# ljubobratovicrelja/tensor-truth

Measured on AMD Instinct MI355X. Metric: queries/sec (embed+top-k+rerank) over 10M x 1024 corpus, higher is better.
Workload: dtype bf16

## Files before the change

### include/tt_hip.h

```cpp
#ifndef TT_HIP_H
#define TT_HIP_H

#include <stddef.h>
#include <stdint.h>

#ifdef __cplusplus
extern "C" {
#endif

#if defined(__GNUC__) || defined(__clang__)
#pragma GCC visibility push(default)
#endif

#define TT_OK 0
#define TT_E_INVALID (-1)
#define TT_E_UNSUPPORTED (-2)
#define TT_E_WORKSPACE (-3)
#define TT_E_HIP (-4)

int tt_version(void);
const char* tt_arch(void);
const char* tt_last_error(void);
int tt_device_cu_count(void);

// ... 48 lines not shown

typedef struct tt_layer_weights {
    const void* qkv_w;
    const float* qkv_b;
    const void* o_w;
    const float* o_b;
    const float* ln1_g;
    const float* ln1_b;
    const void* ffn1_w;
    const float* ffn1_b;
    const void* ffn2_w;
    const float* ffn2_b;
    const float* ln2_g;
    const float* ln2_b;
    const void* qkv_w8;
    const float* qkv_wscale;
    const void* ffn1_w8;
    const float* ffn1_wscale;
    const void* o_w8;
    const float* o_wscale;
    const void* ffn2_w8;
    const float* ffn2_wscale;
    float ffn_act_scale;
} tt_layer_weights;

typedef struct tt_encoder_weights {
    int32_t hidden, layers, heads, ffn, vocab, max_pos, type_vocab;
    float ln_eps;
    const void* word_emb;
    const void* pos_emb;
    const void* type_emb;
    const float* emb_ln_g;
    const float* emb_ln_b;
    const tt_layer_weights* layer;
    const void* cls_dense_w;
    const float* cls_dense_b;
    const void* cls_out_w;
    const float* cls_out_b;
    float* ffn_absmax_out;
} tt_encoder_weights;

size_t tt_encoder_workspace_bytes(const tt_encoder_weights* w, int n_rows);

int tt_encoder_forward(const tt_encoder_weights* w, const int32_t* ids, const int32_t* pos,
                       const int32_t* type_ids, const int32_t* seq_start, const int32_t* seq_len,
                       int n_seq, int n_rows, int max_len, void* hidden_out,
                       void* workspace, size_t workspace_bytes, void* stream);

size_t tt_encoder_cls_workspace_bytes(const tt_encoder_weights* w, int n_rows, int n_seq);
int tt_encoder_forward_cls(const tt_encoder_weights* w, const int32_t* ids, const int32_t* pos,
                           const int32_t* type_ids, const int32_t* seq_start, const int32_t* seq_len,
                           int n_seq, int n_rows, int max_len, void* cls_out,
                           void* workspace, size_t workspace_bytes, void* stream);

int tt_embed_pool(const void* hidden_bf16, int ld, const int32_t* rows, int n_seq, int hidden,
                  float* out_f32, void* out_bf16, void* stream);

int tt_embed_pool_mean(const void* hidden_bf16, int ld, const int32_t* seq_start, const int32_t* seq_len, int n_seq, int hidden,
                       float* out_f32, void* out_bf16, void* stream);
int tt_embed_pool_mean_f32(const float* hidden_f32, int ld, const int32_t* seq_start, const int32_t* seq_len, int n_seq, int hidden,
                           float* out_f32, void* out_bf16, void* stream);

int tt_rerank_head(const tt_encoder_weights* w, const void* hidden_bf16, const int32_t* rows, int n_seq,
                   float* scores, float* logits, void* workspace, size_t workspace_bytes, void* stream);

int tt_adjacent_cosine(const float* emb_f32, int n, int hidden, float* out_dist, void* stream);

int tt_gemm_bf16(const void* a, const void* w, const float* bias, const void* residual, void* c,
                 int m, int n, int k, int epilogue , void* stream);
int tt_layernorm_bf16(const void* in, void* out, const float* gamma, const float* beta, int rows, int hidden,
                      float eps, void* stream);
int tt_attention_varlen(const void* qk, int ld_qk, int q_col0, int k_col0, const void* vt, int ldvt, void* out,
                        int ld_out, const int32_t* seq_start, const int32_t* seq_len, int n_seq, int heads,
                        int head_dim, int max_len, void* stream);
int tt_attention_cls_varlen(const void* qk, int ld_qk, int q_col0, int k_col0, const void* vt, int ldvt, void* out,
                            int ld_out, const int32_t* seq_start, const int32_t* seq_len, int n_seq, int heads,
                            int head_dim, int max_len, void* stream);

int tt_quantize_rows_fp8(const void* in_bf16, int rows, int cols, void* out_fp8, float* out_scale, void* stream);
int tt_layernorm_bf16_fp8(const void* in, void* out, const float* gamma, const float* beta, int rows, int hidden,
                          float eps, void* out_fp8, float* out_scale, void* stream);
int tt_gemm_fp8(const void* a8, const float* a_scale, const void* w8, const float* w_scale, const float* bias, void* c,
                int m, int n, int k, int epilogue , void* stream);
int tt_gemm_fp8_ex(const void* a8, const float* a_scale, const void* w8, const float* w_scale, const float* bias,
                   const void* residual, void* c_bf16, void* c_fp8, float c_fp8_inv_scale, int m, int n, int k,
                   int epilogue, void* stream);

typedef struct tt_layer_weights_f32 {
    const float* qkv_w;
    const float* qkv_b;
    const float* o_w;
    const float* o_b;
    const float* ln1_g;
    const float* ln1_b;
    const float* ffn1_w;
    const float* ffn1_b;
    const float* ffn2_w;
    const float* ffn2_b;
    const float* ln2_g;
    const float* ln2_b;
} tt_layer_weights_f32;

typedef struct tt_encoder_weights_f32 {
    int32_t hidden, layers, heads, ffn, vocab, max_pos, type_vocab;
    float ln_eps;
    const float* word_emb;
    const float* pos_emb;
    const float* type_emb;
    const float* emb_ln_g;
    const float* emb_ln_b;
    const tt_layer_weights_f32* layer;
    const float* cls_dense_w;
    const float* cls_dense_b;
    const float* cls_out_w;
    const float* cls_out_b;
} tt_encoder_weights_f32;

size_t tt_encoder_f32_workspace_bytes(const tt_encoder_weights_f32* w, int n_rows);
int tt_encoder_forward_f32(const tt_encoder_weights_f32* w, const int32_t* ids, const int32_t* pos,
                           const int32_t* type_ids, const int32_t* seq_start, const int32_t* seq_len,
                           int n_seq, int n_rows, int max_len, float* hidden_out,
                           void* workspace, size_t workspace_bytes, void* stream);
int tt_embed_pool_f32(const float* hidden_f32, int ld, const int32_t* rows, int n_seq, int hidden,
                      float* out_f32, void* out_bf16, void* stream);
int tt_rerank_head_f32(const tt_encoder_weights_f32* w, const float* hidden_f32, const int32_t* rows, int n_seq,
                       float* scores, float* logits, void* workspace, size_t workspace_bytes, void* stream);
int tt_gemm_f32(const float* a, const float* w, const float* bias, const float* residual, float* c,
                int m, int n, int k, int epilogue, void* stream);

size_t tt_encoder_workspace_bytes_f16(const tt_encoder_weights* w, int n_rows);
size_t tt_encoder_cls_workspace_bytes_f16(const tt_encoder_weights* w, int n_rows, int n_seq);
int tt_encoder_forward_f16(const tt_encoder_weights* w, const int32_t* ids, const int32_t* pos,
                           const int32_t* type_ids, const int32_t* seq_start, const int32_t* seq_len,
                           int n_seq, int n_rows, int max_len, void* hidden_out,
                           void* workspace, size_t workspace_bytes, void* stream);
int tt_encoder_forward_cls_f16(const tt_encoder_weights* w, const int32_t* ids, const int32_t* pos,
                               const int32_t* type_ids, const int32_t* seq_start, const int32_t* seq_len,
                               int n_seq, int n_rows, int max_len, void* cls_out,
                               void* workspace, size_t workspace_bytes, void* stream);
int tt_embed_pool_f16(const void* hidden_f16, int ld, const int32_t* rows, int n_seq, int hidden, float* out_f32,
                      void* out_f16, void* stream);
int tt_embed_pool_mean_f16(const void* hidden_f16, int ld, const int32_t* seq_start, const int32_t* seq_len, int n_seq, int hidden,
                           float* out_f32, void* out_f16, void* stream);
int tt_rerank_head_f16(const tt_encoder_weights* w, const void* hidden_f16, const int32_t* rows, int n_seq,
                       float* scores, float* logits, void* workspace, size_t workspace_bytes, void* stream);
int tt_gemm_f16(const void* a, const void* w, const float* bias, const void* residual, void* c,
                int m, int n, int k, int epilogue, void* stream);
int tt_layernorm_f16(const void* in, void* out, const float* gamma, const float* beta, int rows, int hidden,
                     float eps, void* stream);
int tt_attention_varlen_f16(const void* qk, int ld_qk, int q_col0, int k_col0, const void* vt, int ldvt, void* out,
                            int ld_out, const int32_t* seq_start, const int32_t* seq_len, int n_seq, int heads,
                            int head_dim, int max_len, void* stream);
int tt_attention_cls_varlen_f16(const void* qk, int ld_qk, int q_col0, int k_col0, const void* vt, int ldvt, void* out,
                                int ld_out, const int32_t* seq_start, const int32_t* seq_len, int n_seq, int heads,
                                int head_dim, int max_len, void* stream);

typedef struct tt_layer_weights_x3 {
    const void* qkv_w;
    const float* qkv_b;
    const void* o_w;
    const float* o_b;
    const float* ln1_g;
    const float* ln1_b;
    const void* ffn1_w;
    const float* ffn1_b;
    const void* ffn2_w;
    const float* ffn2_b;
    const float* ln2_g;
    const float* ln2_b;
} tt_layer_weights_x3;

typedef struct tt_encoder_weights_x3 {
    int32_t hidden, layers, heads, ffn, vocab, max_pos, type_vocab;
    float ln_eps;
    const float* word_emb;
    const float* pos_emb;
    const float* type_emb;
    const float* emb_ln_g;
    const float* emb_ln_b;
    const tt_layer_weights_x3* layer;
    const float* cls_dense_w;
    const float* cls_dense_b;
    const float* cls_out_w;
    const float* cls_out_b;
} tt_encoder_weights_x3;

size_t tt_encoder_x3_workspace_bytes(const tt_encoder_weights_x3* w, int n_rows);
int tt_encoder_forward_x3(const tt_encoder_weights_x3* w, const int32_t* ids, const int32_t* pos,
                          const int32_t* type_ids, const int32_t* seq_start, const int32_t* seq_len,
                          int n_seq, int n_rows, int max_len, float* hidden_out,
                          void* workspace, size_t workspace_bytes, void* stream);
size_t tt_encoder_x3_cls_workspace_bytes(const tt_encoder_weights_x3* w, int n_rows, int n_seq);
int tt_encoder_forward_x3_cls(const tt_encoder_weights_x3* w, const int32_t* ids, const int32_t* pos, const int32_t* type_ids,
                              const int32_t* seq_start, const int32_t* seq_len, int n_seq, int n_rows, int max_len,
                              float* cls_out, void* workspace, size_t workspace_bytes, void* stream);
int tt_rerank_head_x3(const tt_encoder_weights_x3* w, const float* hidden_f32, const int32_t* rows, int n_seq,
                      float* scores, float* logits, void* workspace, size_t workspace_bytes, void* stream);
int tt_split_planes(const float* in_f32, int64_t rows, int cols, void* out_planes, void* stream);
int tt_gemm_x3(const void* a_planes, const void* w_planes, const float* bias, const float* residual_f32, void* c_planes,
               float* c_f32, int m, int n, int k, int epilogue, void* stream);
int tt_gemm_x3_ex(const void* a_planes, const void* w_planes, const float* bias, const float* residual_f32,
                  const void* residual_planes, int ldr, int res_lo_off, void* c_planes, int ldc, int c_lo_off, float* c_f32,
                  void* vt_hi, void* vt_lo, int ldvt, int m, int n, int k, int epilogue, void* stream);
int tt_attention_x3(const void* qk_planes, int ld_qk, int q_col0, int k_col0, int lo_off, const void* vt_hi,
                    const void* vt_lo, int ldvt, void* out_planes, int ld_out, int out_lo_off,
// ... 470 lines not shown
```

### tensor-truth_amd/_lib.py

```python
from __future__ import annotations

import ctypes
import os
import threading
from ctypes import c_char_p, c_float, c_int, c_int32, c_int64, c_size_t, c_void_p

_HERE = os.path.dirname(os.path.abspath(__file__))
_LIB_NAME = "libtt_hip.so"
_lock = threading.Lock()
_lib = None


class LibraryNotBuiltError(RuntimeError):
    pass


class TTError(RuntimeError):
    """A libtt_hip.so call returned a non-zero status."""


def lib_path() -> str:
    return os.path.join(_HERE, os.environ.get("TT_LIB_NAME") or _LIB_NAME)


# ... 9 lines not shown
    if _isa_ok is None:
        import hashlib

        ok = False
        try:
            with open(lib_path() + ".isa_ok") as fh:
                want = fh.read().strip()
            h = hashlib.sha256()
            with open(lib_path(), "rb") as fh:
                for blk in iter(lambda: fh.read(1 << 20), b""):
                    h.update(blk)
            ok = h.hexdigest() == want
        except OSError:
            ok = False
        _isa_ok = ok
    return _isa_ok


_F32P = ctypes.POINTER(c_float)
_I32P = ctypes.POINTER(c_int32)

SIGNATURES = {
    "tt_version": (c_int, []),
    "tt_arch": (c_char_p, []),
    "tt_last_error": (c_char_p, []),
    "tt_device_cu_count": (c_int, []),
    "tt_scan_workspace_bytes": (c_size_t, [c_int64, c_int, c_int, c_int]),
    "tt_scan_topk": (c_int, [c_void_p, c_int64, c_int, c_void_p, c_int, c_int, c_int32, c_void_p, c_void_p,
                             c_void_p, c_size_t, c_void_p, c_void_p]),
    "tt_scan_exact_workspace_bytes": (c_size_t, [c_int64, c_int, c_int, c_int]),
    "tt_scan_topk_exact": (c_int, [c_void_p, c_int64, c_int, c_void_p, c_int, c_int, c_int32, c_void_p, c_void_p,
                                   c_void_p, c_size_t, c_void_p]),
    "tt_scan_segmented_workspace_bytes": (c_size_t, [c_int64, c_int, c_int, c_int]),
    "tt_scan_topk_segmented": (c_int, [c_void_p, c_int64, c_int, c_void_p, c_int, c_int, c_void_p, c_int, c_void_p,
                                       c_void_p, c_void_p, c_size_t, c_void_p]),
    "tt_scan_shadow_bytes": (c_size_t, [c_int64, c_int]),
    "tt_scan_shadow_build": (c_int, [c_void_p, c_int, c_int64, c_int64, c_void_p, c_int64, c_void_p]),
    "tt_scan_shadow_workspace_bytes": (c_size_t, [c_int64, c_int, c_int, c_int]),
    "tt_scan_topk_shadow": (c_int, [c_void_p, c_void_p, c_int64, c_int64, c_int, c_void_p, c_int, c_int, c_int32, c_void_p, c_void_p,
                                    c_void_p, c_size_t, c_void_p, c_void_p]),
    "tt_filter_rows_workspace_bytes": (c_size_t, [c_int64]),
    "tt_filter_rows": (c_int, [c_int, c_void_p, c_void_p, c_void_p, c_int, c_int64, c_void_p, c_int, c_void_p, c_void_p,
                               c_void_p, c_size_t, c_void_p]),
    "tt_scan_topk_rows_workspace_bytes": (c_size_t, [c_int64, c_int, c_int, c_int]),
    "tt_scan_topk_rows": (c_int, [c_void_p, c_int64, c_int, c_void_p, c_int, c_int, c_void_p, c_void_p, c_int64, c_void_p, c_int,
                                  c_int32, c_void_p, c_void_p, c_void_p, c_size_t, c_void_p, c_void_p]),
    "tt_topk_merge": (c_int, [c_void_p, c_void_p, c_int, c_int, c_int, c_void_p, c_void_p, c_void_p]),
    "tt_encoder_workspace_bytes": (c_size_t, [c_void_p, c_int]),
    "tt_encoder_forward": (c_int, [c_void_p, c_void_p, c_void_p, c_void_p, c_void_p, c_void_p, c_int, c_int, c_int,
                                   c_void_p, c_void_p, c_size_t, c_void_p]),
    "tt_encoder_cls_workspace_bytes": (c_size_t, [c_void_p, c_int, c_int]),
    "tt_encoder_forward_cls": (c_int, [c_void_p, c_void_p, c_void_p, c_void_p, c_void_p, c_void_p, c_int, c_int, c_int,
                                       c_void_p, c_void_p, c_size_t, c_void_p]),
    "tt_embed_pool": (c_int, [c_void_p, c_int, c_void_p, c_int, c_int, c_void_p, c_void_p, c_void_p]),
    "tt_embed_pool_mean": (c_int, [c_void_p, c_int, c_void_p, c_void_p, c_int, c_int, c_void_p, c_void_p, c_void_p]),
    "tt_embed_pool_mean_f32": (c_int, [c_void_p, c_int, c_void_p, c_void_p, c_int, c_int, c_void_p, c_void_p, c_void_p]),
    "tt_encoder_workspace_bytes_f16": (c_size_t, [c_void_p, c_int]),
    "tt_encoder_cls_workspace_bytes_f16": (c_size_t, [c_void_p, c_int, c_int]),
    "tt_encoder_forward_f16": (c_int, [c_void_p, c_void_p, c_void_p, c_void_p, c_void_p, c_void_p, c_int, c_int, c_int,
                                   c_void_p, c_void_p, c_size_t, c_void_p]),
    "tt_encoder_forward_cls_f16": (c_int, [c_void_p, c_void_p, c_void_p, c_void_p, c_void_p, c_void_p, c_int, c_int, c_int,
                                       c_void_p, c_void_p, c_size_t, c_void_p]),
    "tt_embed_pool_f16": (c_int, [c_void_p, c_int, c_void_p, c_int, c_int, c_void_p, c_void_p, c_void_p]),
    "tt_embed_pool_mean_f16": (c_int, [c_void_p, c_int, c_void_p, c_void_p, c_int, c_int, c_void_p, c_void_p, c_void_p]),
    "tt_rerank_head_f16": (c_int, [c_void_p, c_void_p, c_void_p, c_int, c_void_p, c_void_p, c_void_p, c_size_t, c_void_p]),
    "tt_gemm_f16": (c_int, [c_void_p, c_void_p, c_void_p, c_void_p, c_void_p, c_int, c_int, c_int, c_int, c_void_p]),
    "tt_layernorm_f16": (c_int, [c_void_p, c_void_p, c_void_p, c_void_p, c_int, c_int, c_float, c_void_p]),
    "tt_attention_varlen_f16": (c_int, [c_void_p, c_int, c_int, c_int, c_void_p, c_int, c_void_p, c_int, c_void_p,
                                    c_void_p, c_int, c_int, c_int, c_int, c_void_p]),
    "tt_attention_cls_varlen_f16": (c_int, [c_void_p, c_int, c_int, c_int, c_void_p, c_int, c_void_p, c_int, c_void_p,
                                    c_void_p, c_int, c_int, c_int, c_int, c_void_p]),
    "tt_rerank_head": (c_int, [c_void_p, c_void_p, c_void_p, c_int, c_void_p, c_void_p, c_void_p, c_size_t, c_void_p]),
    "tt_adjacent_cosine": (c_int, [c_void_p, c_int, c_int, c_void_p, c_void_p]),
    "tt_gemm_bf16": (c_int, [c_void_p, c_void_p, c_void_p, c_void_p, c_void_p, c_int, c_int, c_int, c_int, c_void_p]),
    "tt_layernorm_bf16": (c_int, [c_void_p, c_void_p, c_void_p, c_void_p, c_int, c_int, c_float, c_void_p]),
    "tt_attention_varlen": (c_int, [c_void_p, c_int, c_int, c_int, c_void_p, c_int, c_void_p, c_int, c_void_p,
                                    c_void_p, c_int, c_int, c_int, c_int, c_void_p]),
    "tt_attention_cls_varlen": (c_int, [c_void_p, c_int, c_int, c_int, c_void_p, c_int, c_void_p, c_int, c_void_p,
                                    c_void_p, c_int, c_int, c_int, c_int, c_void_p]),
    "tt_quantize_rows_fp8": (c_int, [c_void_p, c_int, c_int, c_void_p, c_void_p, c_void_p]),
    "tt_layernorm_bf16_fp8": (c_int, [c_void_p, c_void_p, c_void_p, c_void_p, c_int, c_int, c_float, c_void_p, c_void_p,
                                      c_void_p]),
    "tt_gemm_fp8": (c_int, [c_void_p, c_void_p, c_void_p, c_void_p, c_void_p, c_void_p, c_int, c_int, c_int, c_int,
                            c_void_p]),
    "tt_gemm_fp8_ex": (c_int, [c_void_p, c_void_p, c_void_p, c_void_p, c_void_p, c_void_p, c_void_p, c_void_p, c_float,
                               c_int, c_int, c_int, c_int, c_void_p]),
    "tt_encoder_f32_workspace_bytes": (c_size_t, [c_void_p, c_int]),
    "tt_encoder_forward_f32": (c_int, [c_void_p, c_void_p, c_void_p, c_void_p, c_void_p, c_void_p, c_int, c_int, c_int,
                                       c_void_p, c_void_p, c_size_t, c_void_p]),
    "tt_embed_pool_f32": (c_int, [c_void_p, c_int, c_void_p, c_int, c_int, c_void_p, c_void_p, c_void_p]),
    "tt_rerank_head_f32": (c_int, [c_void_p, c_void_p, c_void_p, c_int, c_void_p, c_void_p, c_void_p, c_size_t, c_void_p]),
    "tt_gemm_f32": (c_int, [c_void_p, c_void_p, c_void_p, c_void_p, c_void_p, c_int, c_int, c_int, c_int, c_void_p]),
    "tt_encoder_x3_workspace_bytes": (c_size_t, [c_void_p, c_int]),
    "tt_encoder_x3_cls_workspace_bytes": (c_size_t, [c_void_p, c_int, c_int]),
    "tt_encoder_forward_x3": (c_int, [c_void_p, c_void_p, c_void_p, c_void_p, c_void_p, c_void_p, c_int, c_int, c_int,
                                      c_void_p, c_void_p, c_size_t, c_void_p]),
    "tt_encoder_forward_x3_cls": (c_int, [c_void_p, c_void_p, c_void_p, c_void_p, c_void_p, c_void_p, c_int, c_int, c_int,
                                      c_void_p, c_void_p, c_size_t, c_void_p]),
    "tt_rerank_head_x3": (c_int, [c_void_p, c_void_p, c_void_p, c_int, c_void_p, c_void_p, c_void_p, c_size_t, c_void_p]),
    "tt_split_planes": (c_int, [c_void_p, c_int64, c_int, c_void_p, c_void_p]),
    "tt_gemm_x3": (c_int, [c_void_p, c_void_p, c_void_p, c_void_p, c_void_p, c_void_p, c_int, c_int, c_int, c_int, c_void_p]),
    "tt_gemm_x3_ex": (c_int, [c_void_p, c_void_p, c_void_p, c_void_p, c_void_p, c_int, c_int, c_void_p, c_int, c_int, c_void_p,
                              c_void_p, c_void_p, c_int, c_int, c_int, c_int, c_int, c_void_p]),
    "tt_attention_x3": (c_int, [c_void_p, c_int, c_int, c_int, c_int, c_void_p, c_void_p, c_int, c_void_p, c_int, c_int,
                                c_void_p, c_void_p, c_int, c_int, c_int, c_void_p]),
    "tt_attention_x3_hd": (c_int, [c_void_p, c_int, c_int, c_int, c_int, c_void_p, c_void_p, c_int, c_void_p, c_int, c_int,
# ... 117 lines not shown
                                       c_int, c_int, c_int, c_int, c_int, c_void_p, c_void_p]),
    "tt_maxsim": (c_int, [c_void_p, c_void_p, c_void_p, c_int, c_void_p, c_void_p, c_void_p, c_void_p, c_int, c_int, c_void_p,
                          c_void_p]),
    "tt_colbert_project": (c_int, [c_void_p, c_int, c_int, c_void_p, c_int, c_void_p, c_int, c_void_p, c_void_p]),
    "tt_attention_keylimit": (c_int, [c_void_p, c_int, c_int, c_int, c_void_p, c_int, c_void_p, c_int, c_void_p, c_void_p, c_void_p,
                                      c_int, c_int, c_int, c_int, c_void_p]),
    "tt_encoder_forward_keylen": (c_int, [c_void_p, c_void_p, c_void_p, c_void_p, c_void_p, c_void_p, c_void_p, c_int, c_int, c_int,
                                          c_void_p, c_void_p, c_size_t, c_void_p]),
    "tt_maxsim_f16": (c_int, [c_void_p, c_void_p, c_void_p, c_int, c_void_p, c_void_p, c_void_p, c_void_p, c_int, c_int, c_void_p,
                              c_void_p]),
    "tt_colbert_project_f16": (c_int, [c_void_p, c_int, c_int, c_void_p, c_int, c_void_p, c_int, c_void_p, c_void_p]),
    "tt_attention_keylimit_f16": (c_int, [c_void_p, c_int, c_int, c_int, c_void_p, c_int, c_void_p, c_int, c_void_p, c_void_p,
                                          c_void_p, c_int, c_int, c_int, c_int, c_void_p]),
    "tt_encoder_forward_keylen_f16": (c_int, [c_void_p, c_void_p, c_void_p, c_void_p, c_void_p, c_void_p, c_void_p, c_int, c_int,
                                              c_int, c_void_p, c_void_p, c_size_t, c_void_p]),
    "tt_lexical_weights": (c_int, [c_void_p, c_int, c_int, c_int, c_void_p, c_float, c_void_p, c_void_p, c_void_p, c_int, c_int,
                                   c_int, c_int, c_int, c_int, c_void_p, c_void_p, c_void_p, c_void_p]),
    "tt_lexical_weights_f16": (c_int, [c_void_p, c_int, c_int, c_int, c_void_p, c_float, c_void_p, c_void_p, c_void_p, c_int, c_int,
                                       c_int, c_int, c_int, c_int, c_void_p, c_void_p, c_void_p, c_void_p]),
    "tt_lexical_weights_f32": (c_int, [c_void_p, c_int, c_int, c_int, c_void_p, c_float, c_void_p, c_void_p, c_void_p, c_int, c_int,
                                       c_int, c_int, c_int, c_int, c_void_p, c_void_p, c_void_p, c_void_p]),
    "tt_lexical_score": (c_int, [c_void_p, c_void_p, c_void_p, c_void_p, c_int, c_void_p, c_void_p, c_void_p, c_void_p, c_void_p,
                                 c_int, c_void_p, c_void_p, c_int, c_float, c_float, c_void_p, c_void_p, c_void_p, c_void_p]),
    "tt_lexical_scan_workspace_bytes": (c_size_t, [c_int64, c_int]),
    "tt_lexical_scan_topk": (c_int, [c_void_p, c_void_p, c_void_p, c_void_p, c_int, c_void_p, c_void_p, c_void_p, c_void_p, c_int64,
                                     c_int, c_void_p, c_void_p, c_void_p, c_size_t, c_void_p]),
    "tt_postings_build_workspace_bytes": (c_size_t, [c_int]),
    "tt_postings_build": (c_int, [c_void_p, c_void_p, c_void_p, c_void_p, c_int64, c_int, c_void_p, c_void_p, c_int64, c_void_p,
                                  c_void_p, c_void_p, c_size_t, c_void_p]),
    "tt_lexical_topk_postings_workspace_bytes": (c_size_t, [c_int64, c_int64, c_int]),
    "tt_lexical_topk_postings": (c_int, [c_void_p, c_void_p, c_void_p, c_void_p, c_int, c_void_p, c_void_p, c_void_p, c_void_p, c_int64,
                                         c_void_p, c_int64, c_int64, c_void_p, c_void_p, c_void_p, c_int64, c_int, c_void_p, c_void_p,
                                         c_void_p, c_void_p, c_void_p, c_void_p, c_size_t, c_void_p]),
    "tt_multivec_project": (c_int, [c_void_p, c_int, c_int, c_int, c_void_p, c_void_p, c_int, c_void_p, c_int, c_void_p, c_void_p]),
    "tt_multivec_project_f16": (c_int, [c_void_p, c_int, c_int, c_int, c_void_p, c_void_p, c_int, c_void_p, c_int, c_void_p,
                                        c_void_p]),
    "tt_multivec_project_f32": (c_int, [c_void_p, c_int, c_int, c_int, c_void_p, c_void_p, c_int, c_void_p, c_int, c_void_p,
                                        c_void_p]),
    "tt_maxsim_wide": (c_int, [c_void_p, c_void_p, c_void_p, c_int, c_void_p, c_void_p, c_void_p, c_void_p, c_int, c_int, c_int,
                               c_void_p, c_void_p]),
    "tt_maxsim_wide_f16": (c_int, [c_void_p, c_void_p, c_void_p, c_int, c_void_p, c_void_p, c_void_p, c_void_p, c_int, c_int, c_int,
                                   c_void_p, c_void_p]),
    "tt_m3_mix": (c_int, [c_void_p, c_void_p, c_void_p, c_int64, c_float, c_float, c_float, c_void_p, c_void_p]),
    "tt_splade_pool": (c_int, [c_void_p, c_int, c_int, c_int, c_void_p, c_void_p, c_int, c_void_p, c_void_p, c_int, c_int, c_int,
                               c_void_p, c_int, c_void_p]),
    "tt_splade_pool_f16": (c_int, [c_void_p, c_int, c_int, c_int, c_void_p, c_void_p, c_int, c_void_p, c_void_p, c_int, c_int, c_int,
                                   c_void_p, c_int, c_void_p]),
    "tt_sparse_compact": (c_int, [c_void_p, c_int, c_int, c_int, c_int, c_void_p, c_void_p, c_void_p, c_void_p]),
    "tt_prof_enable": (c_int, [c_int]),
    "tt_prof_read": (c_int, [c_int, ctypes.POINTER(ctypes.c_double), ctypes.POINTER(c_int)]),
}


def load_library():
    global _lib
    if _lib is not None:
        return _lib
    with _lock:
        if _lib is not None:
            return _lib
        path = lib_path()
        if not os.path.exists(path):
            raise LibraryNotBuiltError(
                f"{path} not found. Build it first: `python -c 'import __graft_entry__ as g; g.build()'` "
                f"or `make -C {os.path.join(_HERE, 'csrc')}` (needs hipcc, --offload-arch=gfx950). "
                "tensor_truth_amd has no CPU fallback."
            )
        import torch

        lib = ctypes.CDLL(path)
        for name, (res, args) in SIGNATURES.items():
            fn = getattr(lib, name)
            fn.restype = res
            fn.argtypes = args
        _lib = lib
        return _lib


def check(status: int, what: str) -> None:
    if status != 0:
        msg = load_library().tt_last_error().decode("utf-8", "replace")
        raise TTError(f"{what} failed with status {status}: {msg}")
```

### tensor-truth_amd/csrc/attention.hip

```cpp
#include "common.h"
#include "encoder.h"
#include "f16c.h"

namespace {

#ifndef TT_ATT_RESIDENT_DEFAULT
#define TT_ATT_RESIDENT_DEFAULT 0
#endif
#ifndef TT_ATT_RESIDENT_MIN_LEN
#define TT_ATT_RESIDENT_MIN_LEN 1
#endif
constexpr int kKTile = 64;
constexpr int kWaves = 4;

typedef unsigned int u32x4 __attribute__((ext_vector_type(4)));
template <int OFF>
__device__ __forceinline__ u32x4 lds_read128_async(uint32_t addr) {
    u32x4 r;
    asm volatile("ds_read_b128 %0, %1 offset:%2" : "=v"(r) : "v"(addr), "n"(OFF));
    return r;
}
template <int N>
__device__ __forceinline__ void lds_wait4n(u32x4& a, u32x4& b, u32x4& c, u32x4& d) {
    asm volatile("s_waitcnt lgkmcnt(%4)" : "+v"(a), "+v"(b), "+v"(c), "+v"(d) : "n"(N));
}
template <int N>
__device__ __forceinline__ void lds_wait2n(u32x4& a, u32x4& b) {
    asm volatile("s_waitcnt lgkmcnt(%2)" : "+v"(a), "+v"(b) : "n"(N));
}
typedef unsigned int u32x2 __attribute__((ext_vector_type(2)));
__device__ __forceinline__ void lds_write64_async(uint32_t addr, uint2 v) {
    const u32x2 d = u32x2{v.x, v.y};
    asm volatile("ds_write_b64 %0, %1" :: "v"(addr), "v"(d) : "memory");
}

constexpr int kIoLineStores = 1, kIoShapeStores = 4, kIoShapeQ = 8;

template <int DH, bool STAMP = false, int ABL = 0, int NW = kWaves, int IO = kIoLineStores>
__global__ __launch_bounds__(64 * NW, 4) void attention_kernel(AttnParams p) {
    constexpr int RB = DH * 2;
    constexpr int CH = RB / 16;
    constexpr int RPB = 256 / RB;
    constexpr int KS = DH / 16;
    constexpr int DT = DH / 32;
    constexpr int NPK = kKTile * RB / 1024;
    constexpr int NPV = 8 * DH * 16 / 1024;
    constexpr bool kEvenPieces = NPK % NW == 0 && NPV % NW == 0;
    constexpr int KPW = kEvenPieces ? NPK / NW : 1, VPW = kEvenPieces ? NPV / NW : 1;
    static_assert(kEvenPieces || (DH == 64 && NPK == 8 && NPV == 8), "the uneven piece map is written for head_dim 64");
    constexpr int BUF = (NPK + NPV) * 1024;
    __shared__ __attribute__((aligned(1024))) char lds[2 * BUF];

    int st_i = 0;
    auto stamp = [&]() {
        if constexpr (STAMP) {
            if (p.dbg && blockIdx.x == gridDim.x / 2 && (threadIdx.x & 63) == 0 && st_i < 60) {
                __builtin_amdgcn_sched_barrier(0);
                p.dbg[(threadIdx.x >> 6) * 64 + st_i] = __builtin_amdgcn_s_memtime();
                __builtin_amdgcn_sched_barrier(0);
            }
            ++st_i;
        }
    };
    stamp();
    const int nqt = p.n_qt > 0 ? p.n_qt : -p.n_qt;
    const int L = blockIdx.x, t = L >> 3;
    const int qt = p.n_qt > 0 ? t % nqt : L % nqt;
    const int pair = p.n_qt > 0 ? (t / nqt) * 8 + (L & 7) : L / nqt;
    if (pair >= p.heads * p.n_seq) return;
    const int head = pair % p.heads, seq = pair / p.heads;
    const int len = p.seq_len[seq];
    if (qt * 32 * NW >= len) return;
    const int t0 = p.seq_start[seq];
    const int t0a = t0 & ~7, off = t0 - t0a, alen = off + len;
    const int tid = threadIdx.x, lane = tid & 63;
    const int wave = __builtin_amdgcn_readfirstlane(tid >> 6);
    const int ql = lane & 31, hh = lane >> 5;
    const uint32_t lds0 = (uint32_t)(uintptr_t)(__attribute__((address_space(3))) char*)lds;

    int wslot = wave;
    if (p.rotate && NW == kWaves) {
        const int left = len - qt * 32 * kWaves;
        const int n_live = left >= 32 * kWaves ? kWaves : (left + 31) >> 5;
        if (n_live < kWaves) wslot = (wave + ((pair * n_live) & (kWaves - 1))) & (kWaves - 1);
    }
    const int q_row = (qt * NW + wslot) * 32 + ql;
    const int q_row_c = q_row < len ? q_row : len - 1;
    const uint16_t* qp = p.qk + (size_t)(t0 + q_row_c) * p.ld_qk + p.q_col0 + head * DH + hh * 8;
    ex8 qf[KS];
    if constexpr ((IO & kIoShapeQ) != 0) {
#pragma unroll
        for (int s = 0; s < KS; ++s) {
            const int r = (qt * NW + wslot) * 32 + s * (64 / CH) + lane / CH;
            const int rc = r < len ? r : len - 1;
            qf[s] = *reinterpret_cast<const ex8*>(p.qk + (size_t)(t0 + rc) * p.ld_qk + p.q_col0 + head * DH + (lane % CH) * 8);
        }
    } else {
#pragma unroll
        for (int s = 0; s < KS; ++s) qf[s] = *reinterpret_cast<const ex8*>(qp + s * 16);
    }

    const int n_kt = (alen + kKTile - 1) / kKTile;
    const int n_g8 = (alen + 7) >> 3;
    const int t0kv = (ABL == 4) ? (p.seq_start[0] & ~7) : t0a;
    const uint16_t* kbase = p.qk + (size_t)t0kv * p.ld_qk + p.k_col0 + head * DH;
    const uint16_t* vbase = p.vt + (size_t)(t0kv >> 3) * p.ldvt + (size_t)head * DH * 8;
    constexpr int kRowsPerPiece = 64 / CH, kGroupsPerPiece = 64 / DH > 0 ? 64 / DH : 1;
    static_assert(KPW == 1 || CH == 8, "piece-to-piece swizzle step is written for 128-byte K rows");
    static_assert(VPW == 1 || DH == 64, "one token group per V piece");
    const uint32_t lds_base = (uint32_t)(uintptr_t)(__attribute__((address_space(3))) char*)lds;
    uint32_t kvoff0, vvoff0;
    {
        const int e = (kEvenPieces ? wave * KPW * 64 : 0) + lane, r = e / CH, pos = e % CH;
        kvoff0 = ((uint32_t)r * (uint32_t)p.ld_qk + (uint32_t)((pos ^ ((r / RPB) & (CH - 1))) << 3)) * 2u;
        const int ev = (kEvenPieces ? wave * VPW * 64 : 0) + lane;
        vvoff0 = ((uint32_t)(ev / DH) * (uint32_t)p.ldvt + (uint32_t)((ev % DH) * 8)) * 2u;
    }
    auto sbase = [](const void* ptr) {
        const unsigned long long b = reinterpret_cast<unsigned long long>(ptr);
        const unsigned lo = __builtin_amdgcn_readfirstlane((unsigned)b), hi = __builtin_amdgcn_readfirstlane((unsigned)(b >> 32));
        return reinterpret_cast<const char*>(((unsigned long long)hi << 32) | lo);
    };
    auto glds16 = [](const char* base, uint32_t voff, uint32_t lds_addr) {
        asm volatile("s_mov_b32 m0, %2\n\ts_nop 0\n\tglobal_load_lds_dwordx4 %0, %1" ::"v"(voff), "s"(base), "s"(lds_addr) : "memory", "m0");
    };
    auto issue_tile = [&](int kt) {
        const uint32_t buf = lds_base + (uint32_t)(kt & 1) * BUF;
        const bool clamp = (kt + 1) * kKTile > alen || (kt == 0 && off != 0);
        if (!clamp) {
            if constexpr (kEvenPieces) {
#pragma unroll
                for (int i = 0; i < KPW; ++i)
                    glds16(sbase(kbase + ((size_t)kt * kKTile + i * kRowsPerPiece) * p.ld_qk), (i & 1) ? (kvoff0 ^ 64u) : kvoff0,
                           buf + (uint32_t)(wave * KPW + i) * 1024u);
#pragma unroll
                for (int i = 0; i < VPW; ++i)
                    glds16(sbase(vbase + ((size_t)kt * 8 + i * kGroupsPerPiece) * p.ldvt), vvoff0, buf + (uint32_t)(NPK + wave * VPW + i) * 1024u);
            } else {
                for (int j = wave; j < NPK + NPV; j += NW) {
                    if (j < NPK)
                        glds16(sbase(kbase + ((size_t)kt * kKTile + j * kRowsPerPiece) * p.ld_qk), (j & 1) ? (kvoff0 ^ 64u) : kvoff0,
                               buf + (uint32_t)j * 1024u);
                    else
                        glds16(sbase(vbase + ((size_t)kt * 8 + (j - NPK) * kGroupsPerPiece) * p.ldvt), vvoff0, buf + (uint32_t)j * 1024u);
                }
            }
            return;
        }
        const char* kb = sbase(kbase);
        const char* vb = sbase(vbase);
        int lane_c = lane;
        asm volatile("" : "+v"(lane_c));
        auto clamped_k = [&](int piece) {
            const int e = piece * 64 + lane_c, r = e / CH, pos = e % CH;
            int row = kt * kKTile + r;
            row = row < off ? off : (row < alen ? row : alen - 1);
            glds16(kb, ((uint32_t)row * (uint32_t)p.ld_qk + (uint32_t)((pos ^ ((r / RPB) & (CH - 1))) << 3)) * 2u,
                   buf + (uint32_t)piece * 1024u);
// ... 246 lines not shown
            __builtin_amdgcn_sched_barrier(0);
            if (!wave_active) return;
            const uint32_t slice = lds0 + (uint32_t)wave * (32 * RB);
            const uint32_t wbase = slice + ql * RB + (((ql / RPL) & (CH - 1)) << 4) + 8 * hh;
#pragma unroll
            for (int d = 0; d < DT; ++d)
#pragma unroll
                for (int g = 0; g < 4; ++g) {
                    uint2 o;
                    o.x = pack_e2(acc_o[d][4 * g + 0] * inv, acc_o[d][4 * g + 1] * inv);
                    o.y = pack_e2(acc_o[d][4 * g + 2] * inv, acc_o[d][4 * g + 3] * inv);
                    lds_write64_async(wbase ^ (uint32_t)((4 * d + g) << 4), o);
                }
            asm volatile("s_waitcnt lgkmcnt(0)" ::: "memory");
            const int r0 = lane / CH;
            const uint32_t raddr = slice + r0 * RB + (((lane % CH) ^ ((r0 / RPL) & (CH - 1))) << 4);
            t[0] = lds_read128_async<0>(raddr);
            t[1] = lds_read128_async<RPI * RB>(raddr);
            if constexpr (NI == 4) {
                t[2] = lds_read128_async<2 * RPI * RB>(raddr);
                t[3] = lds_read128_async<3 * RPI * RB>(raddr);
                lds_wait4n<0>(t[0], t[1], t[2], t[3]);
            } else {
                lds_wait2n<0>(t[0], t[1]);
            }
        }
        const int row0 = (qt * NW + wslot) * 32 + lane / CH;
        uint16_t* op = p.out + (size_t)(t0 + row0) * p.ld_out + head * DH + (lane % CH) * 8;
#pragma unroll
        for (int i = 0; i < NI; ++i)
            if (row0 + i * RPI < len) *reinterpret_cast<u32x4*>(op + (size_t)(i * RPI) * p.ld_out) = t[i];
    }
}


#if TT_DIAG
constexpr int kResMaxTiles = 5;

template <int DH, bool PIPE = false, bool EARLY = false>
__global__ __launch_bounds__(64 * kWaves, 2) void attention_resident_kernel(AttnParams p) {
    constexpr int RB = DH * 2, CH = RB / 16, RPB = 256 / RB, KS = DH / 16, DT = DH / 32;
    constexpr int NPK = kKTile * RB / 1024, NPV = 8 * DH * 16 / 1024, NW = kWaves;
    constexpr int KPW = NPK / NW, VPW = NPV / NW;
    static_assert(DH == 64 && NPK % NW == 0 && NPV % NW == 0, "written for head_dim 64");
    constexpr int BUF = (NPK + NPV) * 1024;
    extern __shared__ __attribute__((aligned(1024))) char lds_dyn[];

    const int pair = blockIdx.x;
    if (pair >= p.heads * p.n_seq) return;
    const int head = pair % p.heads, seq = pair / p.heads;
    const int len = p.seq_len[seq];
    if (len <= 0) return;
    const int t0 = p.seq_start[seq];
    const int t0a = t0 & ~7, off = t0 - t0a, alen = off + len;
    const int tid = threadIdx.x, lane = tid & 63;
    const int wave = __builtin_amdgcn_readfirstlane(tid >> 6);
    const int ql = lane & 31, hh = lane >> 5;
    const uint32_t lds0 = (uint32_t)(uintptr_t)(__attribute__((address_space(3))) char*)lds_dyn;
    const int n_kt = (alen + kKTile - 1) / kKTile;
    const int n_g8 = (alen + 7) >> 3;
    const int n_blk = (len + 31) >> 5;
    const int rot = (int)((blockIdx.x >> 8) * 2 + (blockIdx.x & 1)) & 3;
    const int first = (wave - rot) & 3;

    auto q_ptr = [&](int b) {
        const int q_row = b * 32 + ql;
        const int q_row_c = q_row < len ? q_row : len - 1;
        return p.qk + (size_t)(t0 + q_row_c) * p.ld_qk + p.q_col0 + head * DH + hh * 8;
    };
    const int abl = p.rotate;
    ex8 qf[KS] = {};
    if (first < n_blk && !(abl & 2)) {
        const uint16_t* qp = q_ptr(first);
#pragma unroll
        for (int s = 0; s < KS; ++s) qf[s] = *reinterpret_cast<const ex8*>(qp + s * 16);
    }

    const uint16_t* kbase = p.qk + (size_t)t0a * p.ld_qk + p.k_col0 + head * DH;
    const uint16_t* vbase = p.vt + (size_t)(t0a >> 3) * p.ldvt + (size_t)head * DH * 8;
    constexpr int kRowsPerPiece = 64 / CH, kGroupsPerPiece = 1;
    uint32_t kvoff0, vvoff0;
    {
        const int e = wave * KPW * 64 + lane, r = e / CH, pos = e % CH;
        kvoff0 = ((uint32_t)r * (uint32_t)p.ld_qk + (uint32_t)((pos ^ ((r / RPB) & (CH - 1))) << 3)) * 2u;
        const int ev = wave * VPW * 64 + lane;
        vvoff0 = ((uint32_t)(ev / DH) * (uint32_t)p.ldvt + (uint32_t)((ev % DH) * 8)) * 2u;
    }
    auto sbase = [](const void* ptr) {
        const unsigned long long b = reinterpret_cast<unsigned long long>(ptr);
        const unsigned lo = __builtin_amdgcn_readfirstlane((unsigned)b), hi = __builtin_amdgcn_readfirstlane((unsigned)(b >> 32));
        return reinterpret_cast<const char*>(((unsigned long long)hi << 32) | lo);
    };
    auto glds16 = [](const char* base, uint32_t voff, uint32_t lds_addr) {
        asm volatile("s_mov_b32 m0, %2\n\ts_nop 0\n\tglobal_load_lds_dwordx4 %0, %1" ::"v"(voff), "s"(base), "s"(lds_addr) : "memory", "m0");
    };
    for (int kt = 0; kt < ((abl & 4) ? 0 : n_kt); ++kt) {
        const uint32_t buf = lds0 + (uint32_t)kt * BUF;
        const bool clamp = (kt + 1) * kKTile > alen || (kt == 0 && off != 0);
        if (!clamp) {
#pragma unroll
            for (int i = 0; i < KPW; ++i)
                glds16(sbase(kbase + ((size_t)kt * kKTile + i * kRowsPerPiece) * p.ld_qk), (i & 1) ? (kvoff0 ^ 64u) : kvoff0,
                       buf + (uint32_t)(wave * KPW + i) * 1024u);
#pragma unroll
            for (int i = 0; i < VPW; ++i)
                glds16(sbase(vbase + ((size_t)kt * 8 + i * kGroupsPerPiece) * p.ldvt), vvoff0, buf + (uint32_t)(NPK + wave * VPW + i) * 1024u);
        } else {
            const char* kb = sbase(kbase);
            const char* vb = sbase(vbase);
#pragma unroll
            for (int i = 0; i < KPW; ++i) {
                const int piece = wave * KPW + i;
                const int e = piece * 64 + lane, r = e / CH, pos = e % CH;
                int row = kt * kKTile + r;
                row = row < off ? off : (row < alen ? row : alen - 1);
                glds16(kb, ((uint32_t)row * (uint32_t)p.ld_qk + (uint32_t)((pos ^ ((r / RPB) & (CH - 1))) << 3)) * 2u, buf + (uint32_t)piece * 1024u);
            }
#pragma unroll
            for (int i = 0; i < VPW; ++i) {
                const int piece = wave * VPW + i;
                const int e = piece * 64 + lane;
                int g8 = kt * 8 + e / DH;
                g8 = g8 < n_g8 ? g8 : n_g8 - 1;
                glds16(vb, ((uint32_t)g8 * (uint32_t)p.ldvt + (uint32_t)((e % DH) * 8)) * 2u, buf + (uint32_t)(NPK + piece) * 1024u);
            }
        }
    }
    if constexpr (!EARLY) {
        __builtin_amdgcn_s_waitcnt(0x0F70);
        asm volatile("" ::: "memory");
        __builtin_amdgcn_sched_barrier(0);
// ... 284 lines not shown
                    vf[1][1] = lds_read128_async<6 * DH * 16 + 512>(vaddr);
                }
#pragma unroll
                for (int s2 = 0; s2 < 2; ++s2) {
                    uint4 pb;
                    pb.x = pack_e2_inrange(acc_s[j][8 * s2 + 0], acc_s[j][8 * s2 + 1]);
                    pb.y = pack_e2_inrange(acc_s[j][8 * s2 + 2], acc_s[j][8 * s2 + 3]);
                    pb.z = pack_e2_inrange(acc_s[j][8 * s2 + 4], acc_s[j][8 * s2 + 5]);
                    pb.w = pack_e2_inrange(acc_s[j][8 * s2 + 6], acc_s[j][8 * s2 + 7]);
                    const ex8 pf = __builtin_bit_cast(ex8, pb);
#pragma unroll
                    for (int d = 0; d < DT; ++d)
                        acc_o[d] = TT_MFMA_32x32x16(va[s2][d], pf, acc_o[d]);
                }
            }
        }
        const float l_tot = l_run + __shfl_xor(l_run, 32, 64);
        const float inv = 1.0f / l_tot;
        const int q_row = b * 32 + ql;
        if (q_row < len && !(abl & 1)) {
            uint16_t* op = p.out + (size_t)(t0 + q_row) * p.ld_out + head * DH;
#pragma unroll
            for (int d = 0; d < DT; ++d)
#pragma unroll
                for (int g = 0; g < 4; ++g) {
                    uint2 o;
                    o.x = pack_e2(acc_o[d][4 * g + 0] * inv, acc_o[d][4 * g + 1] * inv);
                    o.y = pack_e2(acc_o[d][4 * g + 2] * inv, acc_o[d][4 * g + 3] * inv);
                    *reinterpret_cast<uint2*>(op + 32 * d + 8 * g + 4 * hh) = o;
                }
        }
        if (EARLY && first_walk) {
            first_walk = false;
            if (more && !(abl & 2)) {
                const uint16_t* qp = q_ptr(b + NW);
#pragma unroll
                for (int s = 0; s < KS; ++s) qn[s] = *reinterpret_cast<const ex8*>(qp + s * 16);
            }
        }
        if (more) {
#pragma unroll
            for (int s = 0; s < KS; ++s) qf[s] = qn[s];
        }
    }
}


#endif
template <int DH>
__global__ __launch_bounds__(64) void attention_cls_kernel(AttnParams p) {
    extern __shared__ __attribute__((aligned(16))) float probs[];
    const int seq = blockIdx.x, head = blockIdx.y, lane = threadIdx.x;
    const int len = p.seq_len[seq], t0 = p.seq_start[seq];
    const int t0a = t0 & ~7, off = t0 - t0a, alen = off + len;
    float q[DH];
    {
        const uint16_t* qp = p.q_rows ? p.q_rows + (size_t)seq * p.ld_q_rows + head * DH : p.qk + (size_t)t0 * p.ld_qk + p.q_col0 + head * DH;
#pragma unroll
        for (int c = 0; c < DH / 8; ++c) {
            const uint4 u = *reinterpret_cast<const uint4*>(qp + c * 8);
            q[c * 8 + 0] = elo(u.x); q[c * 8 + 1] = ehi(u.x);
            q[c * 8 + 2] = elo(u.y); q[c * 8 + 3] = ehi(u.y);
            q[c * 8 + 4] = elo(u.z); q[c * 8 + 5] = ehi(u.z);
            q[c * 8 + 6] = elo(u.w); q[c * 8 + 7] = ehi(u.w);
            if (p.qk_lo_off) {
                const uint4 l = *reinterpret_cast<const uint4*>(qp + p.qk_lo_off + c * 8);
                q[c * 8 + 0] += elo(l.x); q[c * 8 + 1] += ehi(l.x);
                q[c * 8 + 2] += elo(l.y); q[c * 8 + 3] += ehi(l.y);
                q[c * 8 + 4] += elo(l.z); q[c * 8 + 5] += ehi(l.z);
                q[c * 8 + 6] += elo(l.w); q[c * 8 + 7] += ehi(l.w);
            }
        }
    }
    const float sc = p.scale * 1.4426950408889634f;
    float mx = -__builtin_inff();
    for (int j = off + lane; j < alen; j += 64) {
        const uint16_t* kp = p.qk + (size_t)(t0a + j) * p.ld_qk + p.k_col0 + head * DH;
        float acc = 0.f;
#pragma unroll
        for (int c = 0; c < DH / 8; ++c) {
            const uint4 u = *reinterpret_cast<const uint4*>(kp + c * 8);
            float kf[8] = {elo(u.x), ehi(u.x), elo(u.y), ehi(u.y), elo(u.z), ehi(u.z), elo(u.w), ehi(u.w)};
            if (p.qk_lo_off) {
                const uint4 l = *reinterpret_cast<const uint4*>(kp + p.qk_lo_off + c * 8);
                kf[0] += elo(l.x); kf[1] += ehi(l.x); kf[2] += elo(l.y); kf[3] += ehi(l.y);
                kf[4] += elo(l.z); kf[5] += ehi(l.z); kf[6] += elo(l.w); kf[7] += ehi(l.w);
            }
#pragma unroll
            for (int i = 0; i < 8; ++i) acc = fmaf(q[c * 8 + i], kf[i], acc);
        }
        acc *= sc;
        probs[j] = acc;
        mx = fmaxf(mx, acc);
    }
#pragma unroll
    for (int off = 32; off > 0; off >>= 1) mx = fmaxf(mx, __shfl_xor(mx, off, 64));
    float sum = 0.f;
    const int len8 = (alen + 7) & ~7;
    for (int j = lane; j < len8; j += 64) {
        float e = 0.f;
        if (j >= off && j < alen) e = __builtin_amdgcn_exp2f(probs[j] - mx);
        probs[j] = e;
        sum += e;
    }
#pragma unroll
    for (int off = 32; off > 0; off >>= 1) sum += __shfl_xor(sum, off, 64);
    __syncthreads();
    constexpr int PARTS = 64 / DH;
    const int d = lane % DH, part = lane / DH;
    float o = 0.f;
    for (int g8 = part; g8 * 8 < alen; g8 += PARTS) {
        const uint4 u = *reinterpret_cast<const uint4*>(p.vt + (size_t)(t0a / 8 + g8) * p.ldvt + (size_t)(head * DH + d) * 8);
        const float4 pa = *reinterpret_cast<const float4*>(probs + g8 * 8);
        const float4 pb = *reinterpret_cast<const float4*>(probs + g8 * 8 + 4);
        o = fmaf(pa.x, elo(u.x), o); o = fmaf(pa.y, ehi(u.x), o);
        o = fmaf(pa.z, elo(u.y), o); o = fmaf(pa.w, ehi(u.y), o);
        o = fmaf(pb.x, elo(u.z), o); o = fmaf(pb.y, ehi(u.z), o);
        o = fmaf(pb.z, elo(u.w), o); o = fmaf(pb.w, ehi(u.w), o);
    }
    if constexpr (PARTS == 2) o += __shfl_xor(o, 32, 64);
    if (p.out_scales) {
        float y = o / sum;
        asm("" : "+v"(y));
        float amax = fabsf(y);
#pragma unroll
        for (int off = 16; off > 0; off >>= 1) amax = fmaxf(amax, __shfl_xor(amax, off, 64));
        int sbyte, sh;
        xc_block_scale(amax, sbyte, sh);
        if (part == 0) {
            const int W = p.out_width, col = head * DH + d;
// ... 140 lines not shown
```

### tensor-truth_amd/csrc/encoder.h

```cpp
#pragma once
#include "common.h"
#include "gemm_plan.h"

struct GemmParams {
    const uint16_t* A;
    const uint16_t* W;
    const float* bias;
    const uint16_t* residual;
    uint16_t* C;
    uint16_t* vt;
    int M, N, K, lda, ldc, ldr, ldvt, vt_col0;
    const float* a_scale;
    const float* w_scale;
    int fp8;
    uint8_t* C8;
    float c8_inv_scale;
    int nt_store;
    int sn;
    int scan_wave_lists;
    int32_t* scan_cnt;
    float* scan_scores;
    int32_t* scan_idx;
    int scan_cap;
    int32_t scan_idx_base;
    float* scan_dense;
    int scan_dense_stride;
    int scan_tile_stride;
    int scan_rows;
    int x3;
    int ldw;
    int c_lo_off;
    float* C32;
    const float* res32;
    const uint16_t* res_planes;
    int res_lo_off;
    uint16_t* vt_lo;
    int x3_zero_lo;
    int xc;
    const uint8_t* a_scales;
    const uint8_t* w_scales;
    uint8_t* c_scales;
};
int tt_scan_gemm_launch(const uint16_t* corpus, int64_t rows, int dim, const uint16_t* queries256, const float* thr256,
                        int32_t* cnt, float* cand_scores, int32_t* cand_idx, int cap, int32_t idx_base, hipStream_t st);
int tt_scan_gemm_sample_launch(const uint16_t* corpus, int tiles, int tile_stride, int dim, const uint16_t* queries256, const float* thr256,
                               float* dense, int dense_stride, hipStream_t st);
int tt_gemm_launch(const GemmParams& p, int epilogue, hipStream_t st);
bool tt_gemm_skinny_enabled();

struct AttnParams {
    const uint16_t* qk;
    const uint16_t* vt;
    uint16_t* out;
    const int32_t* seq_start;
    const int32_t* seq_len;
    int n_seq, heads, head_dim, max_len;
    int total_rows;
    int ld_qk, q_col0, k_col0, ldvt, ld_out;
    float scale;
    float lazy;
    int n_qt;
    int rotate;
    unsigned long long* dbg;
    const uint16_t* q_rows;
    int ld_q_rows;
    uint8_t* out_scales;
    int out_width;
    int qk_lo_off;
};
int tt_attention_launch(const AttnParams& p, hipStream_t st);
int tt_attention_keylimit_launch(const AttnParams& p, const int32_t* key_len, hipStream_t st);
int tt_attention_cls_launch(const AttnParams& p, hipStream_t st);

struct EmbedParams {
    const int32_t* ids;
    const int32_t* pos;
    const int32_t* type;
    const uint16_t* word;
    const uint16_t* posemb;
    const uint16_t* typeemb;
    const float* gamma;
    const float* beta;
    uint16_t* out;
    int T, H, vocab, max_pos, type_vocab;
    float eps;
    uint8_t* q8;
    float* q8_scale;
};
int tt_embed_ln_launch(const EmbedParams& p, hipStream_t st);

int tt_layernorm_launch(const uint16_t* in, uint16_t* out, const float* gamma, const float* beta, int rows, int H,
                        float eps, hipStream_t st, uint8_t* q8 = nullptr, float* q8_scale = nullptr);
int tt_absmax_launch(const uint16_t* x, size_t n, float* out, hipStream_t st);
int tt_quantize_rows_launch(const uint16_t* in, int ld, int rows, int cols, uint8_t* q8, float* scale, hipStream_t st);

int tt_cls_pool_l2norm_launch(const uint16_t* hidden, int ld, const int32_t* rows, int n, int H, float* out_f32,
                              uint16_t* out_bf16, hipStream_t st);

int tt_mean_pool_l2norm_launch(const void* hidden, int is_f32, int ld, const int32_t* seq_start, const int32_t* seq_len, int n, int H,
                               float* out_f32, uint16_t* out_bf16, hipStream_t st);
int tt_gather_rows_launch(const uint16_t* src, int ld, const int32_t* rows, int n, int n_pad, int H, uint16_t* dst,
                          hipStream_t st);

int tt_head_out_sigmoid_launch(const uint16_t* t, int ld, const uint16_t* w, const float* bias, int n, int H,
                               float* scores, float* logits, hipStream_t st);

int tt_adjacent_cosine_launch(const float* e, int n, int H, float* dist, hipStream_t st);

int tt_gather_rows_f32_launch(const float* src, const int32_t* rows, int n, int n_pad, int H, float* dst, hipStream_t st);

struct WsPlanner {
    size_t off = 0;
    size_t take(size_t bytes) { const size_t o = off; off += tt_align_up(bytes, 256); return o; }
};

inline int tt_check_workspace(const char* what, const void* workspace, size_t workspace_bytes, size_t need) {
    if (!workspace || workspace_bytes < need) {
        tt_set_error("%s: workspace %zu < required %zu bytes", what, workspace_bytes, need);
        return TT_E_WORKSPACE;
    }
    TT_CHECK_ARG(((uintptr_t)workspace % 256) == 0, "workspace must be 256-byte aligned");
    return TT_OK;
}

inline int pooled_rows_pad(int n_seq, bool skinny_allowed) {
    return (n_seq <= 256 && skinny_allowed) ? (n_seq + 63) / 64 * 64 : (n_seq + 255) / 256 * 256;
}

template <class Weights>
inline tt_encoder_weights_f32 head_weights_f32(const Weights* w) {
    tt_encoder_weights_f32 h{};
    h.hidden = w->hidden; h.layers = 0; h.heads = w->heads; h.ffn = w->ffn; h.vocab = w->vocab; h.max_pos = w->max_pos;
    h.type_vocab = w->type_vocab; h.ln_eps = w->ln_eps;
    h.word_emb = w->word_emb; h.pos_emb = w->pos_emb; h.type_emb = w->type_emb; h.emb_ln_g = w->emb_ln_g; h.emb_ln_b = w->emb_ln_b;
    h.cls_dense_w = w->cls_dense_w; h.cls_dense_b = w->cls_dense_b; h.cls_out_w = w->cls_out_w; h.cls_out_b = w->cls_out_b;
    return h;
}

inline GemmParams gemm_16(const uint16_t* a, const void* w, const float* bias, int M, int N, int K) {
    GemmParams g{};
// ... 4 lines not shown
```

### tensor-truth_amd/csrc/encoder_api.hip

```cpp
#include "common.h"
#include "encoder.h"

namespace {

struct EncWs {
    size_t off_xa, off_xb, off_y, off_qk, off_vt, off_ctx, off_ffn, total;
    size_t off_cctx, off_cx, off_cy, off_cx1, off_cffn, off_rows;
    int n_cls_pad;
    size_t off_q8, off_q8s, off_q8c;
    bool fp8;
};

bool fp8_ready(const tt_encoder_weights* w, int n_rows) {
    if constexpr (kF16) return false;
    if (w->layers <= 0 || w->hidden % 256 || w->ffn % 256 || n_rows % 256) return false;
    for (int l = 0; l < w->layers; ++l) {
        const tt_layer_weights& lw = w->layer[l];
        if (!lw.qkv_w8 || !lw.qkv_wscale || !lw.ffn1_w8 || !lw.ffn1_wscale) return false;
    }
    return true;
}

EncWs enc_plan(const tt_encoder_weights* w, int n_rows, int n_seq = 0) {
    EncWs e{};
    const size_t H = (size_t)w->hidden, F = (size_t)w->ffn, T = ((size_t)n_rows + 255) / 256 * 256;
    WsPlanner ws;
    e.off_xa = ws.take(T * H * 2);
    e.off_xb = ws.take(T * H * 2);
    e.off_y = ws.take(T * H * 2);
    e.off_qk = ws.take(T * 2 * H * 2);
    e.off_vt = ws.take(H * T * 2);
    e.off_ctx = ws.take(T * H * 2);
    e.off_ffn = ws.take(T * F * 2);
    e.n_cls_pad = pooled_rows_pad(n_seq, tt_gemm_skinny_enabled());
    if (n_seq > 0) {
        const size_t B = (size_t)e.n_cls_pad;
        e.off_cctx = ws.take(B * H * 2);
        e.off_cx = ws.take(B * H * 2);
        e.off_cy = ws.take(B * H * 2);
        e.off_cx1 = ws.take(B * H * 2);
        e.off_cffn = ws.take(B * F * 2);
    }
    e.fp8 = fp8_ready(w, n_rows);
    if (e.fp8) {
        e.off_q8 = ws.take(T * H);
        e.off_q8s = ws.take(T * 4);
        e.off_q8c = ws.take(T * 4);
    }
    e.total = ws.off;
    return e;
}

int check_weights(const tt_encoder_weights* w) {
    TT_CHECK_ARG(w != nullptr, "null weights");
    TT_CHECK_ARG(w->hidden > 0 && w->hidden % 128 == 0 && w->hidden <= 1024, "hidden=%d unsupported", w->hidden);
    TT_CHECK_ARG(w->heads > 0 && w->hidden % w->heads == 0, "heads=%d", w->heads);
    const int dh = w->hidden / w->heads;
    TT_CHECK_ARG(dh == 64 || dh == 32, "head_dim=%d not in {32,64}", dh);
    TT_CHECK_ARG(w->ffn > 0 && w->ffn % 128 == 0, "ffn=%d must be a multiple of 128", w->ffn);
    TT_CHECK_ARG(w->layers >= 0 && (w->layers == 0 || w->layer != nullptr), "layer array missing");
    TT_CHECK_ARG(w->word_emb && w->pos_emb && w->type_emb && w->emb_ln_g && w->emb_ln_b, "embedding tables missing");
    return TT_OK;
}

}

extern "C" {

size_t tt_encoder_workspace_bytes(const tt_encoder_weights* w, int n_rows) {
    if (!w || n_rows <= 0) return 0;
    return enc_plan(w, n_rows).total;
}

static int forward_impl(const tt_encoder_weights* w, const int32_t* ids, const int32_t* pos,
                        const int32_t* type_ids, const int32_t* seq_start, const int32_t* seq_len, int n_seq,
                        int n_rows, int max_len, void* hidden_out, void* cls_out, void* workspace,
                        size_t workspace_bytes, void* stream, const int32_t* key_len = nullptr) {
    if (int rc = check_weights(w)) return rc;
    TT_CHECK_ARG(key_len == nullptr || cls_out == nullptr, "key_len: the full forward only");
    TT_CHECK_ARG(n_rows > 0 && (n_rows % 128 == 0 || (n_rows < 256 && n_rows % 64 == 0)),
                 "n_rows=%d must be a positive multiple of 128 (or 64 / 192)", n_rows);
    TT_CHECK_ARG(n_seq > 0 && max_len > 0, "n_seq=%d max_len=%d", n_seq, max_len);
    TT_CHECK_ARG(ids && pos && seq_start && seq_len && (hidden_out || cls_out), "null pointer");
    const bool cls_tail = cls_out != nullptr && w->layers > 0;
    const EncWs e = enc_plan(w, n_rows, cls_tail ? n_seq : 0);
    if (int rc = tt_check_workspace("tt_encoder_forward", workspace, workspace_bytes, e.total)) return rc;
    hipStream_t st = (hipStream_t)stream;
    char* ws = (char*)workspace;
    const int H = w->hidden, F = w->ffn, T = n_rows;
    uint16_t* xa = (uint16_t*)(ws + e.off_xa);
    uint16_t* xb = (uint16_t*)(ws + e.off_xb);
    uint16_t* y = (uint16_t*)(ws + e.off_y);
    uint16_t* qk = (uint16_t*)(ws + e.off_qk);
    uint16_t* vt = (uint16_t*)(ws + e.off_vt);
    uint16_t* ctx = (uint16_t*)(ws + e.off_ctx);
    uint16_t* ffn = (uint16_t*)(ws + e.off_ffn);
    TT_CHECK_HIP(hipMemsetAsync(ctx, 0, (size_t)T * H * 2, st));

    EmbedParams ep{};
    ep.ids = ids; ep.pos = pos; ep.type = type_ids;
    ep.word = (const uint16_t*)w->word_emb; ep.posemb = (const uint16_t*)w->pos_emb;
    ep.typeemb = (const uint16_t*)w->type_emb;
    ep.gamma = w->emb_ln_g; ep.beta = w->emb_ln_b;
    ep.T = T; ep.H = H; ep.vocab = w->vocab; ep.max_pos = w->max_pos; ep.type_vocab = w->type_vocab;
    ep.eps = w->ln_eps;
    uint16_t* x = (w->layers == 0 && hidden_out) ? (uint16_t*)hidden_out : xa;
    ep.out = x;
    uint8_t* q8 = e.fp8 ? (uint8_t*)(ws + e.off_q8) : nullptr;
    float* q8s = e.fp8 ? (float*)(ws + e.off_q8s) : nullptr;
    ep.q8 = q8; ep.q8_scale = q8s;
    {
        TtProfScope prof(TT_K_ROWOPS, st);
        if (int rc = tt_embed_ln_launch(ep, st)) return rc;
    }

    const int dh = H / w->heads;
    const int f8mask_all = TT_DIAG_ENV_INT("TT_FP8_MASK", 0xF), f8first = TT_DIAG_ENV_INT("TT_FP8_SKIP_FIRST", 0),
              f8last = TT_DIAG_ENV_INT("TT_FP8_SKIP_LAST", 0);
    struct Fp8Ops {
        uint8_t* q8;
        float* q8s;
        float* q8c;
        int mask;
        float* absmax;
    };
    auto half_layer = [&](const tt_layer_weights& lw, int M, uint16_t* c, const uint16_t* res, uint16_t* y, uint16_t* x1, uint16_t* f,
                          uint16_t* out, const Fp8Ops& f8) -> int {
        GemmParams go = gemm_16(c, lw.o_w, lw.o_b, M, H, H);
        go.residual = res; go.ldr = H; go.C = y; go.ldc = H;
        if ((f8.mask & 2) && lw.o_w8 && lw.o_wscale) {
            {
                TtProfScope prof(TT_K_ROWOPS, st);
                if (int rc = tt_quantize_rows_launch(c, H, M, H, f8.q8, f8.q8s, st)) return rc;
            }
            go.A = (const uint16_t*)f8.q8; go.W = (const uint16_t*)lw.o_w8; go.a_scale = f8.q8s; go.w_scale = lw.o_wscale; go.fp8 = 1;
        }
        if (int rc = tt_gemm_launch(go, TT_EPI_RESIDUAL, st)) return rc;
        {
            TtProfScope prof(TT_K_ROWOPS, st);
            if (int rc = tt_layernorm_launch(y, x1, lw.ln1_g, lw.ln1_b, M, H, w->ln_eps, st, f8.q8, f8.q8s)) return rc;
        }
        GemmParams g1 = gemm_16(x1, lw.ffn1_w, lw.ffn1_b, M, F, H);
        g1.C = f; g1.ldc = F;
        const bool f8down = (f8.mask & 12) == 12 && lw.ffn2_w8 && lw.ffn2_wscale && lw.ffn_act_scale > 0.f;
        if (f8.mask & 4) {
            g1.A = (const uint16_t*)f8.q8; g1.W = (const uint16_t*)lw.ffn1_w8; g1.a_scale = f8.q8s; g1.w_scale = lw.ffn1_wscale; g1.fp8 = 1;
            if (f8down) {
                g1.C8 = (uint8_t*)f; g1.c8_inv_scale = 1.0f / lw.ffn_act_scale;
            }
        }
        if (int rc = tt_gemm_launch(g1, TT_EPI_GELU, st)) return rc;
        if (f8.absmax && !f8down) {
            TtProfScope prof(TT_K_ROWOPS, st);
            if (int rc = tt_absmax_launch(f, (size_t)M * F, f8.absmax, st)) return rc;
        }
        GemmParams g2 = gemm_16(f, lw.ffn2_w, lw.ffn2_b, M, H, F);
        g2.residual = x1; g2.ldr = H; g2.C = y; g2.ldc = H;
        if (f8down) {
            const unsigned bits = __builtin_bit_cast(unsigned, lw.ffn_act_scale);
            TT_CHECK_HIP(hipMemsetD32Async(f8.q8c, (int)bits, (size_t)M, st));
            g2.W = (const uint16_t*)lw.ffn2_w8; g2.a_scale = f8.q8c; g2.w_scale = lw.ffn2_wscale; g2.fp8 = 1;
        }
        if (int rc = tt_gemm_launch(g2, TT_EPI_RESIDUAL, st)) return rc;
        TtProfScope prof(TT_K_ROWOPS, st);
        return tt_layernorm_launch(y, out, lw.ln2_g, lw.ln2_b, M, H, w->ln_eps, st, f8.q8, f8.q8s);
    };
    for (int l = 0; l < w->layers; ++l) {
        const tt_layer_weights& lw = w->layer[l];
        TT_CHECK_ARG(lw.qkv_w && lw.qkv_b && lw.o_w && lw.o_b && lw.ln1_g && lw.ln1_b && lw.ffn1_w && lw.ffn1_b &&
                         lw.ffn2_w && lw.ffn2_b && lw.ln2_g && lw.ln2_b,
                     "layer %d has a null weight pointer", l);
        GemmParams g = gemm_16(x, lw.qkv_w, lw.qkv_b, T, 3 * H, H);
        g.C = qk; g.ldc = 2 * H; g.vt = vt; g.ldvt = 8 * H; g.vt_col0 = 2 * H;
        const int f8mask = (!e.fp8 || l < f8first || l >= w->layers - f8last) ? 0 : f8mask_all;
        if (f8mask & 1) {
            g.A = (const uint16_t*)q8; g.W = (const uint16_t*)lw.qkv_w8; g.a_scale = q8s; g.w_scale = lw.qkv_wscale; g.fp8 = 1;
        }
        static const bool kv_only_on = TT_DIAG_ENV_INT("TT_CLS_KV_ONLY", 1) != 0;
        const bool kv_only = cls_tail && l == w->layers - 1 && !g.fp8 && kv_only_on;
        if (kv_only) {
            g.W = (const uint16_t*)lw.qkv_w + (size_t)H * H; g.bias = lw.qkv_b + H;
            g.C = qk + H; g.N = 2 * H; g.vt_col0 = H;
        }
        if (int rc = tt_gemm_launch(g, TT_EPI_QKV, st)) return rc;
        AttnParams a{};
        a.qk = qk; a.ld_qk = 2 * H; a.q_col0 = 0; a.k_col0 = H; a.vt = vt; a.ldvt = 8 * H;
        a.ld_out = H; a.seq_start = seq_start; a.seq_len = seq_len;
        a.n_seq = n_seq; a.heads = w->heads; a.head_dim = dh; a.max_len = max_len;
        a.scale = 1.0f / sqrtf((float)dh);
        if (cls_tail && l == w->layers - 1) {
            const int Bp = e.n_cls_pad;
            uint16_t* cctx = (uint16_t*)(ws + e.off_cctx);
            uint16_t* cx = (uint16_t*)(ws + e.off_cx);
            uint16_t* cy = (uint16_t*)(ws + e.off_cy);
            uint16_t* cx1 = (uint16_t*)(ws + e.off_cx1);
            uint16_t* cffn = (uint16_t*)(ws + e.off_cffn);
            TT_CHECK_HIP(hipMemsetAsync(cctx, 0, (size_t)Bp * H * 2, st));
            {
                TtProfScope prof(TT_K_ROWOPS, st);
                if (int rc = tt_gather_rows_launch(x, H, seq_start, n_seq, Bp, H, cx, st)) return rc;
            }
            if (kv_only) {
                GemmParams gq = gemm_16(cx, lw.qkv_w, lw.qkv_b, Bp, H, H);
                gq.C = cy; gq.ldc = H;
                if (int rc = tt_gemm_launch(gq, TT_EPI_BIAS, st)) return rc;
                a.q_rows = cy; a.ld_q_rows = H;
            }
            a.out = cctx;
            if (int rc = tt_attention_cls_launch(a, st)) return rc;
            return half_layer(lw, Bp, cctx, cx, cy, cx1, cffn, (uint16_t*)cls_out, Fp8Ops{});
        }
        a.out = ctx; a.total_rows = n_rows;
        if (int rc = key_len ? tt_attention_keylimit_launch(a, key_len, st) : tt_attention_launch(a, st)) return rc;
        uint16_t* x1 = (x == xa) ? xb : xa;
        uint16_t* dst = (l == w->layers - 1) ? (uint16_t*)hidden_out : x;
        const Fp8Ops f8{q8, q8s, e.fp8 ? (float*)(ws + e.off_q8c) : nullptr, f8mask, w->ffn_absmax_out ? w->ffn_absmax_out + l : nullptr};
        if (int rc = half_layer(lw, T, ctx, x, y, x1, ffn, dst, f8)) return rc;
        x = dst;
    }
    return TT_OK;
}

int tt_encoder_forward(const tt_encoder_weights* w, const int32_t* ids, const int32_t* pos,
                       const int32_t* type_ids, const int32_t* seq_start, const int32_t* seq_len, int n_seq,
                       int n_rows, int max_len, void* hidden_out, void* workspace, size_t workspace_bytes,
                       void* stream) {
    TT_CHECK_ARG(hidden_out != nullptr, "null hidden_out");
    return forward_impl(w, ids, pos, type_ids, seq_start, seq_len, n_seq, n_rows, max_len, hidden_out, nullptr, workspace,
                        workspace_bytes, stream);
}

int tt_encoder_forward_keylen(const tt_encoder_weights* w, const int32_t* ids, const int32_t* pos, const int32_t* type_ids,
                              const int32_t* seq_start, const int32_t* seq_len, const int32_t* key_len, int n_seq, int n_rows,
                              int max_len, void* hidden_out, void* workspace, size_t workspace_bytes, void* stream) {
    TT_CHECK_ARG(hidden_out != nullptr, "null hidden_out");
    TT_CHECK_ARG(key_len != nullptr, "null key_len");
    return forward_impl(w, ids, pos, type_ids, seq_start, seq_len, n_seq, n_rows, max_len, hidden_out, nullptr, workspace,
                        workspace_bytes, stream, key_len);
}

size_t tt_encoder_cls_workspace_bytes(const tt_encoder_weights* w, int n_rows, int n_seq) {
    if (!w || n_rows <= 0 || n_seq <= 0) return 0;
    return enc_plan(w, n_rows, n_seq).total;
}

int tt_encoder_forward_cls(const tt_encoder_weights* w, const int32_t* ids, const int32_t* pos,
                           const int32_t* type_ids, const int32_t* seq_start, const int32_t* seq_len, int n_seq,
                           int n_rows, int max_len, void* cls_out, void* workspace, size_t workspace_bytes,
                           void* stream) {
    TT_CHECK_ARG(cls_out != nullptr, "null cls_out");
    TT_CHECK_ARG(w && w->layers > 0, "tt_encoder_forward_cls needs at least one layer");
    return forward_impl(w, ids, pos, type_ids, seq_start, seq_len, n_seq, n_rows, max_len, nullptr, cls_out, workspace,
                        workspace_bytes, stream);
}

int tt_embed_pool(const void* hidden_bf16, int ld, const int32_t* rows, int n_seq, int hidden, float* out_f32,
                  void* out_bf16, void* stream) {
    TT_CHECK_ARG(n_seq >= 0, "n_seq=%d", n_seq);
    if (n_seq == 0) return TT_OK;
    TT_CHECK_ARG(hidden_bf16 && rows && out_f32 && ld >= hidden && ld % 8 == 0, "bad argument");
    TtProfScope prof(TT_K_ROWOPS, (hipStream_t)stream);
    return tt_cls_pool_l2norm_launch((const uint16_t*)hidden_bf16, ld, rows, n_seq, hidden, out_f32,
                                     (uint16_t*)out_bf16, (hipStream_t)stream);
}

int tt_embed_pool_mean(const void* hidden_bf16, int ld, const int32_t* seq_start, const int32_t* seq_len, int n_seq, int hidden,
                       float* out_f32, void* out_bf16, void* stream) {
    TT_CHECK_ARG(n_seq >= 0, "n_seq=%d", n_seq);
    if (n_seq == 0) return TT_OK;
    TT_CHECK_ARG(hidden_bf16 && seq_start && seq_len && out_f32 && ld >= hidden && ld % 8 == 0, "bad argument");
    TtProfScope prof(TT_K_ROWOPS, (hipStream_t)stream);
    return tt_mean_pool_l2norm_launch(hidden_bf16, 0, ld, seq_start, seq_len, n_seq, hidden, out_f32, (uint16_t*)out_bf16,
                                      (hipStream_t)stream);
}

#if !TT_F16
int tt_embed_pool_mean_f32(const float* hidden_f32, int ld, const int32_t* seq_start, const int32_t* seq_len, int n_seq, int hidden,
                           float* out_f32, void* out_bf16, void* stream) {
    TT_CHECK_ARG(n_seq >= 0, "n_seq=%d", n_seq);
    if (n_seq == 0) return TT_OK;
    TT_CHECK_ARG(hidden_f32 && seq_start && seq_len && out_f32 && ld >= hidden && ld % 4 == 0, "bad argument");
    TtProfScope prof(TT_K_ROWOPS, (hipStream_t)stream);
    return tt_mean_pool_l2norm_launch(hidden_f32, 1, ld, seq_start, seq_len, n_seq, hidden, out_f32, (uint16_t*)out_bf16,
                                      (hipStream_t)stream);
}

#endif
int tt_rerank_head(const tt_encoder_weights* w, const void* hidden_bf16, const int32_t* rows, int n_seq,
                   float* scores, float* logits, void* workspace, size_t workspace_bytes, void* stream) {
    if (int rc = check_weights(w)) return rc;
    TT_CHECK_ARG(w->cls_dense_w && w->cls_dense_b && w->cls_out_w && w->cls_out_b, "weights carry no classification head");
    TT_CHECK_ARG(n_seq >= 0, "n_seq=%d", n_seq);
    if (n_seq == 0) return TT_OK;
    TT_CHECK_ARG(hidden_bf16 && rows && scores, "null pointer");
    const int H = w->hidden;
    const int n_pad = (n_seq + 127) / 128 * 128;
    const size_t need = 2 * tt_align_up((size_t)n_pad * H * 2, 256);
    if (!workspace || workspace_bytes < need) {
        tt_set_error("tt_rerank_head: workspace %zu < required %zu bytes", workspace_bytes, need);
        return TT_E_WORKSPACE;
    }
    hipStream_t st = (hipStream_t)stream;
    uint16_t* cls = (uint16_t*)workspace;
    uint16_t* t = (uint16_t*)((char*)workspace + tt_align_up((size_t)n_pad * H * 2, 256));
    {
        TtProfScope prof(TT_K_ROWOPS, st);
        if (int rc = tt_gather_rows_launch((const uint16_t*)hidden_bf16, H, rows, n_seq, n_pad, H, cls, st)) return rc;
    }
// ... 46 lines not shown
    g.A = (const uint16_t*)a8; g.lda = k; g.W = (const uint16_t*)w8; g.bias = bias; g.C = (uint16_t*)c; g.ldc = n;
    g.M = m; g.N = n; g.K = k; g.a_scale = a_scale; g.w_scale = w_scale; g.fp8 = 1;
    return tt_gemm_launch(g, epilogue, (hipStream_t)stream);
}

int tt_gemm_fp8_ex(const void* a8, const float* a_scale, const void* w8, const float* w_scale, const float* bias,
                   const void* residual, void* c_bf16, void* c_fp8, float c_fp8_inv_scale, int m, int n, int k,
                   int epilogue, void* stream) {
    TT_CHECK_ARG(epilogue == TT_EPI_BIAS || epilogue == TT_EPI_GELU || epilogue == TT_EPI_RESIDUAL, "epilogue %d", epilogue);
    TT_CHECK_ARG(a8 && a_scale && w8 && w_scale && bias && (c_bf16 || c_fp8), "null pointer");
    TT_CHECK_ARG(epilogue != TT_EPI_RESIDUAL || (residual && c_bf16 && !c_fp8), "residual epilogue: bf16 result only");
    GemmParams g{};
    g.A = (const uint16_t*)a8; g.lda = k; g.W = (const uint16_t*)w8; g.bias = bias; g.ldc = n;
    g.C = c_bf16 ? (uint16_t*)c_bf16 : (uint16_t*)c_fp8;
    g.residual = (const uint16_t*)residual; g.ldr = n;
    g.M = m; g.N = n; g.K = k; g.a_scale = a_scale; g.w_scale = w_scale; g.fp8 = 1;
    if (c_fp8) { g.C8 = (uint8_t*)c_fp8; g.c8_inv_scale = c_fp8_inv_scale; }
    return tt_gemm_launch(g, epilogue, (hipStream_t)stream);
}

#endif
#if !TT_F16 && TT_DIAG
__attribute__((visibility("default"))) int tt_attention_debug_stamps(const void* qk, int ld_qk, int q_col0, int k_col0, const void* vt, int ldvt, void* out,
                              int ld_out, const int32_t* seq_start, const int32_t* seq_len, int n_seq, int heads,
                              int head_dim, int max_len, void* stamps, void* stream) {
    AttnParams a{};
    a.qk = (const uint16_t*)qk; a.ld_qk = ld_qk; a.q_col0 = q_col0; a.k_col0 = k_col0;
    a.vt = (const uint16_t*)vt; a.ldvt = ldvt; a.out = (uint16_t*)out; a.ld_out = ld_out;
    a.seq_start = seq_start; a.seq_len = seq_len; a.n_seq = n_seq; a.heads = heads; a.head_dim = head_dim;
    a.max_len = max_len; a.scale = 1.0f / sqrtf((float)head_dim);
    a.dbg = (unsigned long long*)stamps;
    return tt_attention_launch(a, (hipStream_t)stream);
}

#endif
int tt_layernorm_bf16(const void* in, void* out, const float* gamma, const float* beta, int rows, int hidden,
                      float eps, void* stream) {
    TT_CHECK_ARG(in && out && gamma && beta, "null pointer");
    return tt_layernorm_launch((const uint16_t*)in, (uint16_t*)out, gamma, beta, rows, hidden, eps, (hipStream_t)stream);
}

int tt_attention_varlen(const void* qk, int ld_qk, int q_col0, int k_col0, const void* vt, int ldvt, void* out,
                        int ld_out, const int32_t* seq_start, const int32_t* seq_len, int n_seq, int heads,
                        int head_dim, int max_len, void* stream) {
    TT_CHECK_ARG(qk && vt && out && seq_start && seq_len, "null pointer");
    AttnParams a{};
    a.qk = (const uint16_t*)qk; a.ld_qk = ld_qk; a.q_col0 = q_col0; a.k_col0 = k_col0;
    a.vt = (const uint16_t*)vt; a.ldvt = ldvt; a.out = (uint16_t*)out; a.ld_out = ld_out;
    a.seq_start = seq_start; a.seq_len = seq_len; a.n_seq = n_seq; a.heads = heads; a.head_dim = head_dim;
    a.max_len = max_len; a.scale = 1.0f / sqrtf((float)head_dim);
    return tt_attention_launch(a, (hipStream_t)stream);
}

int tt_attention_cls_varlen(const void* qk, int ld_qk, int q_col0, int k_col0, const void* vt, int ldvt, void* out,
                            int ld_out, const int32_t* seq_start, const int32_t* seq_len, int n_seq, int heads,
                            int head_dim, int max_len, void* stream) {
    TT_CHECK_ARG(qk && vt && out && seq_start && seq_len, "null pointer");
    TT_CHECK_ARG(head_dim == 64 || head_dim == 32, "head_dim=%d: the attention takes 64- or 32-wide heads", head_dim);
    AttnParams a{};
    a.qk = (const uint16_t*)qk; a.ld_qk = ld_qk; a.q_col0 = q_col0; a.k_col0 = k_col0;
    a.vt = (const uint16_t*)vt; a.ldvt = ldvt; a.out = (uint16_t*)out; a.ld_out = ld_out;
    a.seq_start = seq_start; a.seq_len = seq_len; a.n_seq = n_seq; a.heads = heads; a.head_dim = head_dim;
    a.max_len = max_len; a.scale = 1.0f / sqrtf((float)head_dim);
    return tt_attention_cls_launch(a, (hipStream_t)stream);
}

}
```

### tensor-truth_amd/csrc/f16_names.h

```cpp
#pragma once
#define tt_gemm_launch tt_gemm_launch_f16
#define tt_scan_gemm_launch tt_scan_gemm_launch_f16
#define tt_scan_gemm_sample_launch tt_scan_gemm_sample_launch_f16
#define tt_gemm_skinny_enabled tt_gemm_skinny_enabled_f16
#define tt_attention_launch tt_attention_launch_f16
#define tt_attention_cls_launch tt_attention_cls_launch_f16
#define tt_attention_keylimit_launch tt_attention_keylimit_launch_f16
#define tt_absmax_launch tt_absmax_launch_f16
#define tt_embed_ln_launch tt_embed_ln_launch_f16
#define tt_layernorm_launch tt_layernorm_launch_f16
#define tt_gather_rows_launch tt_gather_rows_launch_f16
#define tt_quantize_rows_launch tt_quantize_rows_launch_f16
#define tt_adjacent_cosine_launch tt_adjacent_cosine_launch_f16
#define tt_cls_pool_l2norm_launch tt_cls_pool_l2norm_launch_f16
#define tt_head_out_sigmoid_launch tt_head_out_sigmoid_launch_f16
#define tt_mean_pool_l2norm_launch tt_mean_pool_l2norm_launch_f16
#define tt_encoder_workspace_bytes tt_encoder_workspace_bytes_f16
#define tt_encoder_cls_workspace_bytes tt_encoder_cls_workspace_bytes_f16
#define tt_encoder_forward tt_encoder_forward_f16
#define tt_encoder_forward_cls tt_encoder_forward_cls_f16
#define tt_encoder_forward_keylen tt_encoder_forward_keylen_f16
#define tt_embed_pool tt_embed_pool_f16
#define tt_embed_pool_mean tt_embed_pool_mean_f16
#define tt_rerank_head tt_rerank_head_f16
#define tt_gemm_bf16 tt_gemm_f16
#define tt_layernorm_bf16 tt_layernorm_f16
#define tt_attention_varlen tt_attention_varlen_f16
#define tt_encoder_x3_workspace_bytes tt_encoder_x3_workspace_bytes_f16
#define tt_encoder_x3_cls_workspace_bytes tt_encoder_x3_cls_workspace_bytes_f16
#define tt_encoder_forward_x3 tt_encoder_forward_x3_f16
#define tt_encoder_forward_x3_cls tt_encoder_forward_x3_cls_f16
#define tt_rerank_head_x3 tt_rerank_head_x3_f16
#define tt_split_planes tt_split_planes_f16
#define tt_gemm_x3 tt_gemm_x3_f16
#define tt_gemm_x3_ex tt_gemm_x3_ex_f16
#define tt_attention_x3 tt_attention_x3_f16
#define tt_attention_x3_hd tt_attention_x3_hd_f16
#define tt_attention_cls_varlen tt_attention_cls_varlen_f16
#define tt_decoder_workspace_bytes tt_decoder_workspace_bytes_f16
#define tt_decoder_forward tt_decoder_forward_f16
#define tt_decoder_rows_workspace_bytes tt_decoder_rows_workspace_bytes_f16
#define tt_decoder_forward_rows tt_decoder_forward_rows_f16
#define tt_decoder_score tt_decoder_score_f16
#define tt_embed_pool_last tt_embed_pool_last_f16
#define tt_attention_causal_gqa tt_attention_causal_gqa_f16
#define tt_qk_norm_rope tt_qk_norm_rope_f16
#define tt_modernbert_workspace_bytes tt_modernbert_workspace_bytes_f16
#define tt_modernbert_forward tt_modernbert_forward_f16
#define tt_modernbert_head tt_modernbert_head_f16
#define tt_rope_v8 tt_rope_v8_f16
#define tt_attention_window tt_attention_window_f16
#define tt_mpnet_workspace_bytes tt_mpnet_workspace_bytes_f16
#define tt_mpnet_forward tt_mpnet_forward_f16
#define tt_attention_relbias tt_attention_relbias_f16
#define tt_deberta_workspace_bytes tt_deberta_workspace_bytes_f16
#define tt_deberta_forward tt_deberta_forward_f16
#define tt_deberta_head tt_deberta_head_f16
#define tt_attention_disentangled tt_attention_disentangled_f16
#define tt_ropebert_workspace_bytes tt_ropebert_workspace_bytes_f16
#define tt_ropebert_forward tt_ropebert_forward_f16
#define tt_jinabert_workspace_bytes tt_jinabert_workspace_bytes_f16
#define tt_jinabert_forward tt_jinabert_forward_f16
#define tt_attention_alibi tt_attention_alibi_f16
#define tt_maxsim tt_maxsim_f16
#define tt_colbert_project tt_colbert_project_f16
#define tt_attention_keylimit tt_attention_keylimit_f16
#define tt_lexical_weights tt_lexical_weights_f16
#define tt_multivec_project tt_multivec_project_f16
#define tt_maxsim_wide tt_maxsim_wide_f16
#define tt_splade_pool tt_splade_pool_f16
```

### tensor-truth_amd/csrc/gemm.hip

```cpp
#include "common.h"
#include <type_traits>

#include "encoder.h"
#include "gemm_plan.h"
#include "f16c.h"

namespace {

constexpr int BM = 128, BN = 128, BK = 64;
constexpr int kGemmThreads = 256;
constexpr int kTileBytes = BM * BK * 2;
constexpr int kStageBytes = 2 * kTileBytes;
constexpr int kGemmLds = 2 * kStageBytes;

__device__ __forceinline__ f32x2 gelu_erf2(f32x2 x) {
    const f32x2 u = f32x2{fabsf(x.x), fabsf(x.y)};
    f32x2 q = u * -9.697845371e-07f + 4.016999810e-05f;
    q = q * u + -7.211678312e-04f;
    q = q * u + 7.490924560e-03f;
    q = q * u + -5.142170191e-02f;
    q = q * u + -4.614778757e-01f;
    q = q * u + -1.149914980e+00f;
    q = q * u + -1.000091195e+00f;
    const f32x2 e = f32x2{__builtin_amdgcn_exp2f(q.x), __builtin_amdgcn_exp2f(q.y)};
// ... 70 lines not shown
                    const int n = nw + i * 16 + g * 4;
                    const int m = mw + j * 16 + (lane & 15);
                    const float4 b4 = *reinterpret_cast<const float4*>(p.bias + n);
                    uint16_t* vt = p.vt + (size_t)(m >> 3) * p.ldvt + (size_t)(n - p.vt_col0) * 8 + (m & 7);
                    vt[0] = f32_to_ebits(acc[i][j][0] + b4.x);
                    vt[8] = f32_to_ebits(acc[i][j][1] + b4.y);
                    vt[16] = f32_to_ebits(acc[i][j][2] + b4.z);
                    vt[24] = f32_to_ebits(acc[i][j][3] + b4.w);
                }
                continue;
            }
        }
        const int n = nw + i * 16 + (g & ~1) * 4;
        const float4 ba = *reinterpret_cast<const float4*>(p.bias + n);
        const float4 bb = *reinterpret_cast<const float4*>(p.bias + n + 4);
        const float bias8[8] = {ba.x, ba.y, ba.z, ba.w, bb.x, bb.y, bb.z, bb.w};
#pragma unroll
        for (int j = 0; j < MT; j += 2) {
            float v[8];
#pragma unroll
            for (int k = 0; k < 4; ++k) {
                const auto r = __builtin_amdgcn_permlane16_swap(__float_as_uint(acc[i][j][k]),
                                                                __float_as_uint(acc[i][j + 1][k]), false, false);
                v[k] = __uint_as_float(r[0]);
                v[4 + k] = __uint_as_float(r[1]);
            }
            const int m = mw + (odd ? j + 1 : j) * 16 + (lane & 15);
#pragma unroll
            for (int k = 0; k < 8; ++k) v[k] += bias8[k];
            if constexpr (EPI == TT_EPI_GELU) {
#pragma unroll
                for (int k = 0; k < 8; ++k) v[k] = gelu_erf(v[k]);
            } else if constexpr (EPI == TT_EPI_TANH) {
#pragma unroll
                for (int k = 0; k < 8; ++k) v[k] = tanhf(v[k]);
            } else if constexpr (EPI == TT_EPI_RELU) {
#pragma unroll
                for (int k = 0; k < 8; ++k) v[k] = fmaxf(v[k], 0.f);
            } else if constexpr (EPI == TT_EPI_RESIDUAL) {
                const uint4 r = *reinterpret_cast<const uint4*>(p.residual + (size_t)m * p.ldr + n);
                v[0] += elo(r.x); v[1] += ehi(r.x);
                v[2] += elo(r.y); v[3] += ehi(r.y);
                v[4] += elo(r.z); v[5] += ehi(r.z);
                v[6] += elo(r.w); v[7] += ehi(r.w);
            }
            uint4 o;
            o.x = pack_e2(v[0], v[1]); o.y = pack_e2(v[2], v[3]);
            o.z = pack_e2(v[4], v[5]); o.w = pack_e2(v[6], v[7]);
            *reinterpret_cast<uint4*>(p.C + (size_t)m * p.ldc + n) = o;
        }
    }
}

template <int NT, int MT, bool FP8 = false, bool X3 = false>
__device__ __forceinline__ void gemm_epilogue_vt(const GemmParams& p, f32x4 (&acc)[NT][MT], int mw, int nw, int lane) {
    static_assert(NT % 2 == 0, "n-tiles are processed in pairs");
    const int g = lane >> 4;
    const bool odd = (g & 1) != 0;
#pragma unroll
    for (int i = 0; i < NT; i += 2) {
        const int n = nw + (odd ? i + 1 : i) * 16 + (lane & 15);
        const float b = p.bias[n];
        float sw = 1.f;
        if constexpr (FP8) sw = p.w_scale[n];
        uint16_t* col = p.vt + (size_t)(n - p.vt_col0) * 8;
#pragma unroll
        for (int j = 0; j < MT; ++j) {
            float v[8];
            const int m = mw + j * 16 + (g & ~1) * 4;
#pragma unroll
            for (int k = 0; k < 4; ++k) {
                const auto r = __builtin_amdgcn_permlane16_swap(__float_as_uint(acc[i][j][k]),
                                                                __float_as_uint(acc[i + 1][j][k]), false, false);
                v[k] = __uint_as_float(r[0]);
                v[4 + k] = __uint_as_float(r[1]);
            }
            if constexpr (FP8) {
                const float4 a0 = *reinterpret_cast<const float4*>(p.a_scale + m);
                const float4 a1 = *reinterpret_cast<const float4*>(p.a_scale + m + 4);
                v[0] *= a0.x * sw; v[1] *= a0.y * sw; v[2] *= a0.z * sw; v[3] *= a0.w * sw;
                v[4] *= a1.x * sw; v[5] *= a1.y * sw; v[6] *= a1.z * sw; v[7] *= a1.w * sw;
            }
#pragma unroll
            for (int k = 0; k < 8; ++k) v[k] += b;
            uint4 o;
            o.x = pack_sel<X3>(v[0], v[1]); o.y = pack_sel<X3>(v[2], v[3]);
            o.z = pack_sel<X3>(v[4], v[5]); o.w = pack_sel<X3>(v[6], v[7]);
            *reinterpret_cast<uint4*>(col + (size_t)(m >> 3) * p.ldvt) = o;
            if constexpr (X3) {
                uint4 l;
                l.x = pack_e2(v[0] - elo(o.x), v[1] - ehi(o.x));
                l.y = pack_e2(v[2] - elo(o.y), v[3] - ehi(o.y));
                l.z = pack_e2(v[4] - elo(o.z), v[5] - ehi(o.z));
                l.w = pack_e2(v[6] - elo(o.w), v[7] - ehi(o.w));
                if (p.x3_zero_lo) l = uint4{0u, 0u, 0u, 0u};
                *reinterpret_cast<uint4*>(p.vt_lo + (size_t)(n - p.vt_col0) * 8 + (size_t)(m >> 3) * p.ldvt) = l;
            }
        }
    }
}

__device__ __forceinline__ void stage_tile(const GemmParams& p, char* stage, int wave, int lane, int m0, int n0, int k0) {
    const int lrow = lane >> 3;
    const int slot = lane & 7;
#pragma unroll
    for (int j = 0; j < 4; ++j) {
        const int row = 32 * wave + 8 * j + lrow;
        const int chunk = slot ^ ((row >> 1) & 7);
        const uint16_t* src = p.A + (size_t)(m0 + row) * p.lda + k0 + chunk * 8;
        __builtin_amdgcn_global_load_lds((const __attribute__((address_space(1))) void*)src,
                                         (__attribute__((address_space(3))) void*)(stage + (32 * wave + 8 * j) * 128),
                                         16, 0, 0);
    }
#pragma unroll
    for (int j = 0; j < 4; ++j) {
        const int row = 32 * wave + 8 * j + lrow;
        const int chunk = slot ^ ((row >> 1) & 7);
        const uint16_t* src = p.W + (size_t)(n0 + row) * p.K + k0 + chunk * 8;
        __builtin_amdgcn_global_load_lds((const __attribute__((address_space(1))) void*)src,
                                         (__attribute__((address_space(3))) void*)(stage + kTileBytes + (32 * wave + 8 * j) * 128),
                                         16, 0, 0);
    }
}

template <int EPI>
__global__ __launch_bounds__(kGemmThreads, 2) void gemm_kernel(GemmParams p) {
    extern __shared__ __attribute__((aligned(16))) char smem[];
    const int tid = threadIdx.x;
    const int lane = tid & 63;
    const int wave = __builtin_amdgcn_readfirstlane(tid >> 6);
    const int wm = wave >> 1, wn = wave & 1;

    const int mt_n = p.M / BM, nt_n = p.N / BN;
    int L = blockIdx.x;
    {
        const int nwg = gridDim.x;
        if ((nwg & 7) == 0) L = (L & 7) * (nwg >> 3) + (L >> 3);
    }
    const int SN = nt_n < 8 ? nt_n : 8;
    const int SM = 8;
// ... 634 lines not shown
#pragma unroll
            for (int qm = 0; qm < 2; ++qm)
#pragma unroll
                for (int half = 0; half < 2; ++half) {
                    const f32x4 a = acc[qm][qn][nt][2 * half], b = acc[qm][qn][nt][2 * half + 1];
                    float m[4];
#pragma unroll
                    for (int r = 0; r < 4; ++r) m[r] = dpp_max16(fmaxf(a[r], b[r]));
                    if (l15 == 0) {
                        const int grp = tile * 8 + qm * 4 + wm * 2 + half;
#pragma unroll
                        for (int r = 0; r < 4; ++r) p.scan_dense[(size_t)(q0 + r) * p.scan_dense_stride + grp] = m[r];
                    }
                }
        }
}

#define TT_SLOT_END()                                         \
    do {                                                      \
        __builtin_amdgcn_sched_barrier(0);                    \
        __builtin_amdgcn_s_barrier();                         \
        __builtin_amdgcn_sched_barrier(0);                    \
    } while (0)

typedef int v8i __attribute__((ext_vector_type(8)));
struct Frag2 { ex8 lo, hi; };
__device__ __forceinline__ f32x4 mfma_fp8(const ex8& a0, const ex8& a1, const ex8& b0, const ex8& b1, f32x4 c) {
    const v8i a = __builtin_bit_cast(v8i, Frag2{a0, a1});
    const v8i b = __builtin_bit_cast(v8i, Frag2{b0, b1});
    return __builtin_amdgcn_mfma_scale_f32_16x16x128_f8f6f4(a, b, c, 0, 0, 0, 0x7F7F7F7F, 0, 0x7F7F7F7F);
}

constexpr int kXcScaleOff = kLds3;
constexpr int kLdsXc = kLds3 + 2 * 8192;
__device__ __forceinline__ void glds4(const void* base, uint32_t voff, uint32_t lds_addr) {
    asm volatile("s_mov_b32 m0, %2\n\ts_nop 0\n\tglobal_load_lds_dword %0, %1"
                 :: "v"(voff), "s"(base), "s"(lds_addr) : "memory", "m0");
}
template <int OA, int OB>
__device__ __forceinline__ f32x4 mfma_fp8_scaled(const ex8& a0, const ex8& a1, const ex8& b0, const ex8& b1, f32x4 c, uint32_t scale_a,
                                                 uint32_t scale_b) {
    const v8i a = __builtin_bit_cast(v8i, Frag2{a0, a1});
    const v8i b = __builtin_bit_cast(v8i, Frag2{b0, b1});
    return __builtin_amdgcn_mfma_scale_f32_16x16x128_f8f6f4(a, b, c, 0, 0, OA, (int)scale_a, OB, (int)scale_b);
}
template <int N, class F>
__device__ __forceinline__ void static_for(F&& f) {
    if constexpr (N > 0) {
        static_for<N - 1>(f);
        f(std::integral_constant<int, N - 1>{});
    }
}

template <int EPI, bool FP8 = false, bool X3 = false, bool XC = false, bool RP = false>
__global__ __launch_bounds__(kThreads3, 2) void gemm_kernel_v3(GemmParams p) {
    static_assert(!(FP8 && X3), "split-bf16 operands are bf16");
    static_assert(!XC || (!FP8 && !X3 && kF16), "f16c operands: the fp16 instantiation, no other operand mode");
    constexpr int ES = FP8 ? 1 : 2;
    extern __shared__ __attribute__((aligned(16))) char smem[];
    const int tid = threadIdx.x;
    const int lane = tid & 63;
    const int wave = __builtin_amdgcn_readfirstlane(tid >> 6);
    const int wm = wave >> 2, wn = wave & 3;

    const int mt_n = p.M / BM3, nt_n = (p.N + BN3 - 1) / BN3;
    int L = blockIdx.x;
    {
        const int nwg = gridDim.x;
        if ((nwg & 7) == 0) L = (L & 7) * (nwg >> 3) + (L >> 3);
    }
    const int SN = p.sn > 0 ? p.sn : (nt_n < 4 ? nt_n : 4);
    const int SM = 32 / SN > 0 ? 32 / SN : 1;
    const int per_super = SM * SN;
    const int supers_n = (nt_n + SN - 1) / SN;
    const int sidx = L / per_super, widx = L % per_super;
    const int tm = (sidx / supers_n) * SM + widx / SN;
    const int tn = (sidx % supers_n) * SN + widx % SN;
    if (tm >= mt_n || tn >= nt_n) return;
    int m0_nominal = tm * BM3;
    if constexpr (EPI == TT_EPI_SCAN) {
        if (p.scan_tile_stride > 1) m0_nominal *= p.scan_tile_stride;
        if (p.scan_rows && m0_nominal + BM3 > p.scan_rows) m0_nominal = p.scan_rows - BM3;
    }
    const int m0 = m0_nominal, n0 = tn * BN3;
    const int nk1 = p.K * ES / 128;
    constexpr int TB = X3 ? 64 : 128;
    const int nk = X3 ? 2 * nk1 : (XC ? 2 * nk1 : nk1);
    auto tile_a = [&](int t) { return t; };
    auto tile_w = [&](int t) { return t; };

    f32x4 acc[2][2][2][4];
#pragma unroll
    for (int a = 0; a < 2; ++a)
#pragma unroll
        for (int b = 0; b < 2; ++b)
#pragma unroll
            for (int c = 0; c < 2; ++c)
#pragma unroll
                for (int d = 0; d < 4; ++d) acc[a][b][c][d] = f32x4{0.f, 0.f, 0.f, 0.f};

    const int frow = lane & 15, fchk = lane >> 4, sw = (frow >> 1) & 7;
    const int off0 = frow * 128 + ((fchk ^ sw) << 4);
    const int off1 = frow * 128 + (((4 + fchk) ^ sw) << 4);
    const int a_row0 = wm * 64 * 128;
    const int w_row0 = wn * 32 * 128;

    uint32_t voffA[2], voffW[2];
#pragma unroll
    for (int j = 0; j < 2; ++j) {
// ... 187 lines not shown
            mma8(acc[0][0], wf0, sa_reg[0], sw_reg, std::integral_constant<int, 0>{});
            mma8(acc[0][1], wf1, sa_reg[0], sw_reg, std::integral_constant<int, 1>{});
        } else {
            mma(acc[0][0], wf0);
            mma(acc[0][1], wf1);
        }
        TT_SLOT_END();
        if (more2) {
            stage_half<0, ES, true>(p, smem, 0, B, tile_a(t + 2), wave, voffA, m0, n0, TB);
            stage_half<1, ES>(p, smem, 0, B, tile_w(t + 2), wave, voffW, m0, n0, TB);
            if (sc_lb) stage_scales(t + 2);
        } else if (kResLds) {
            stage_res(B == 0 ? 0 : 2);
        }
        read_a(smem + slot_off(0, 1, B));
        if constexpr (F8T) sa_reg[1] = *reinterpret_cast<const uint32_t*>(sbuf + 512 + sa_off);
        wait_n((t + 2 < nk || kResLds) ? 6 + sc_lb : 0);
        if constexpr (F8T) {
            mma8(acc[1][1], wf1, sa_reg[1], sw_reg, std::integral_constant<int, 1>{});
            mma8(acc[1][0], wf0, sa_reg[1], sw_reg, std::integral_constant<int, 0>{});
        } else {
            mma(acc[1][1], wf1);
            mma(acc[1][0], wf0);
        }
        TT_SLOT_END();
    };

    if constexpr (XC) {
        for (int t = 0; t < nk1; t += 2) {
            tile4(t, std::integral_constant<int, 0>{}, std::false_type{});
            tile4(t + 1, std::integral_constant<int, 1>{}, std::false_type{});
        }
        for (int t = nk1; t < nk; t += 2) {
            tile4(t, std::integral_constant<int, 0>{}, std::true_type{});
            tile4(t + 1, std::integral_constant<int, 1>{}, std::true_type{});
        }
    } else {
        for (int t = 0; t < nk; t += 2) {
            tile4(t, std::integral_constant<int, 0>{}, std::false_type{});
            if (t + 1 < nk) tile4(t + 1, std::integral_constant<int, 1>{}, std::false_type{});
        }
    }
    if (!late) TT_SLOT_END();
    stage_res(3);

    if constexpr (X3) {
        if (n0 + wn * 64 >= p.N) return;
    }
    if constexpr (vblk) {
#pragma unroll
        for (int qm = 0; qm < 2; ++qm)
#pragma unroll
            for (int qn = 0; qn < 2; ++qn)
                gemm_epilogue_vt<2, 4, FP8, X3>(p, acc[qm][qn], m0 + qm * 128 + wm * 64, n0 + wn * 64 + qn * 32, lane);
    } else if constexpr (X3) {
        epilogue_x3<EPI, RP>(p, acc, smem, kBiasOff, m0, n0, wm, wn, lane);
    } else if constexpr (XC && EPI == TT_EPI_RESIDUAL) {
        epilogue_x3<EPI>(p, acc, smem, kBiasOff, m0, n0, wm, wn, lane);
    } else if constexpr (XC && EPI == TT_EPI_GELU) {
        epilogue_xc<EPI>(p, acc, smem, kBiasOff, m0, n0, wm, wn, lane);
    } else if constexpr (XC && EPI == TT_EPI_BIAS) {
        if (p.c_lo_off) epilogue_h2(p, acc, smem, kBiasOff, m0, n0, wm, wn, lane);
        else epilogue_all<EPI, true, false>(p, acc, smem, kBiasOff, kScaleOff, m0, n0, wm, wn, wave, lane, false, NoNext{});
    } else if constexpr (EPI == TT_EPI_QKV) {
#pragma unroll
        for (int qm = 0; qm < 2; ++qm)
#pragma unroll
            for (int qn = 0; qn < 2; ++qn)
                gemm_epilogue_wide<EPI, 2, 4>(p, acc[qm][qn], m0 + qm * 128 + wm * 64, n0 + wn * 64 + qn * 32, lane);
    } else if constexpr (EPI == TT_EPI_SCAN) {
        if (p.scan_dense) scan_sample_epilogue(p, acc, tm, wm, wn, lane);
        else if (p.scan_wave_lists) scan_filter_epilogue<2>(p, acc, smem, kBiasOff, m0, wm, wn, lane);
        else scan_filter_epilogue<1>(p, acc, smem, kBiasOff, m0, wm, wn, lane);
    } else {
        epilogue_all<EPI, true, FP8>(p, acc, smem, kBiasOff, kScaleOff, m0, n0, wm, wn, wave, lane, false, NoNext{});
    }
}

template <int EPI, bool FP8 = false>
__global__ __launch_bounds__(kThreads3, 2) void gemm_kernel_p(GemmParams p, int nwg) {
    constexpr int ES = FP8 ? 1 : 2;
    extern __shared__ __attribute__((aligned(16))) char smem[];
    const int tid = threadIdx.x;
    const int lane = tid & 63;
    const int wave = __builtin_amdgcn_readfirstlane(tid >> 6);
    const int wm = wave >> 2, wn = wave & 3;

    const int mt_n = p.M / BM3, nt_n = p.N / BN3;
    const int SN = p.sn > 0 ? p.sn : (nt_n < 4 ? nt_n : 4);
    const int SM = 32 / SN > 0 ? 32 / SN : 1;
    const int per_super = SM * SN;
    const int supers_n = (nt_n + SN - 1) / SN;
    const int nk = p.K * ES / 128;
    auto decode = [&](int v, int& m0, int& n0) {
        const int L = (v & 7) * (nwg >> 3) + (v >> 3);
        const int sidx = L / per_super, widx = L % per_super;
        const int tm = (sidx / supers_n) * SM + widx / SN;
        const int tn = (sidx % supers_n) * SN + widx % SN;
        int mm = tm * BM3;
        if constexpr (EPI == TT_EPI_SCAN) {
            if (p.scan_rows && mm + BM3 > p.scan_rows) mm = p.scan_rows - BM3;
        }
        m0 = __builtin_amdgcn_readfirstlane(mm);
        n0 = __builtin_amdgcn_readfirstlane(tn * BN3);
        return tm < mt_n && tn < nt_n;
    };
    auto next_valid = [&](int v, int& m0, int& n0) {
// ... 607 lines not shown
        const int ldw = p.ldw ? p.ldw : 2 * p.K;
        if (p.M % v3::BM3 || p.N % v3::BN3 || p.K % 256 || p.K < 256 || p.lda < 2 * p.K || ldw < 2 * p.K || p.lda % 8 || ldw % 8 || !p.A ||
            !p.W || !p.bias || !p.a_scales || !p.w_scales) {
            tt_set_error("gemm f16c: M=%d N=%d K=%d lda=%d ldw=%d: M, N, K multiples of 256, c-planes [.][>= 2K uint16] with tiled scales",
                         p.M, p.N, p.K, p.lda, ldw);
            return TT_E_UNSUPPORTED;
        }
        if constexpr (EPI == TT_EPI_RESIDUAL) {
            if (!p.C32 || !p.res32 || p.ldc % 4 || p.ldr % 4) { tt_set_error("gemm f16c: residual epilogue needs fp32 C32 / res32"); return TT_E_INVALID; }
        } else if constexpr (EPI == TT_EPI_VT) {
            if (!p.vt || p.ldvt % 8) { tt_set_error("gemm f16c: V^T epilogue needs vt"); return TT_E_INVALID; }
        } else if constexpr (EPI == TT_EPI_GELU) {
            if (!p.C || !p.c_scales || p.ldc != 2 * p.N) { tt_set_error("gemm f16c: c-planes output needs C, c_scales, ldc = 2 N"); return TT_E_INVALID; }
        } else {
            if (!p.C || p.ldc % 8 || p.c_lo_off % 8 || (p.c_lo_off && p.c_lo_off < p.N)) {
                tt_set_error("gemm f16c: fp16 output needs C, ldc %% 8 == 0 (two planes: c_lo_off >= N, a multiple of 8)");
                return TT_E_INVALID;
            }
        }
        const GemmPlan pl = plan_of(GemmForm::Xc, EPI, p);
        GemmParams q = p;
        q.sn = pl.grid.sn;
        q.ldw = ldw;
        q.nt_store = 1;
        return run_kernel<v3::gemm_kernel_v3<EPI, false, false, true>>(TT_K_GEMM, dim3(pl.gx), v3::kThreads3, v3::kLdsXc, st, q);
    } else {
        tt_set_error("gemm f16c: epilogue %d has no f16c form (fp16 instantiation: bias, GELU, residual, V^T)", EPI);
        return TT_E_UNSUPPORTED;
    }
}

template <int EPI>
int launch_16(const GemmParams& p, const GemmPlan& pl, hipStream_t st) {
    if constexpr (!kF16) if (p.fp8) return launch_fp8<EPI>(p, st);
    const GemmSwitches& sw = gemm_switches();
    GemmParams q = p;
    if constexpr (EPI != TT_EPI_VT) {
        if (pl.kernel == GemmKernel::Skinny) return run_kernel<gemm_skinny_kernel<EPI, false>>(TT_K_GEMM, dim3(pl.gx, pl.gy), 64, 0, st, q);
    }
    if (sw.trace) fprintf(stderr, "gemm launch<%d> M=%d N=%d K=%d lda=%d ldc=%d ldr=%d\n", EPI, p.M, p.N, p.K, p.lda, p.ldc, p.ldr);
    const bool tile128 = pl.kernel == GemmKernel::Staged128 || pl.kernel == GemmKernel::TwoStage128;
    if (EPI == TT_EPI_VT && tile128) {
        tt_set_error("gemm: internal V^T epilogue needs the 256x256 kernel");
        return TT_E_UNSUPPORTED;
    }
    if (!tile128) q.sn = pl.grid.sn;
    switch (pl.kernel) {
        case GemmKernel::Persistent256:
            if constexpr (EPI == TT_EPI_GELU)
                return run_kernel<v3::gemm_kernel_p<EPI>>(TT_K_GEMM, dim3(pl.gx), v3::kThreads3, v3::kLds3, st, q, pl.grid.blocks);
            break;
        case GemmKernel::OneTile256:
            q.nt_store = sw.nt_store;
            return run_kernel<v3::gemm_kernel_v3<EPI>>(TT_K_GEMM, dim3(pl.gx), v3::kThreads3, v3::kLds3, st, q);
        case GemmKernel::Staged128:
            if constexpr (EPI != TT_EPI_VT) return run_kernel<gemm_staged_kernel<EPI, false>>(TT_K_GEMM, dim3(pl.gx), kStagedThreads, kStagedLds, st, q);
            break;
        case GemmKernel::TwoStage128:
            if constexpr (EPI != TT_EPI_VT) return run_kernel<gemm_kernel<EPI>>(TT_K_GEMM, dim3(pl.gx), kGemmThreads, kGemmLds, st, q);
            break;
        default: break;
    }
    tt_set_error("gemm: internal: the plan names kernel %d, which epilogue %d of 16-bit operands has not", (int)pl.kernel, EPI);
    return TT_E_UNSUPPORTED;
}

}

bool tt_gemm_skinny_enabled() { return gemm_switches().skinny; }

int tt_gemm_launch(const GemmParams& p, int epilogue, hipStream_t st) {
    if (p.M <= 0 || p.N <= 0) return TT_OK;
    if constexpr (kF16) {
        if (p.fp8) { tt_set_error("gemm (fp16 build): fp8 operands belong to the bf16 instantiation"); return TT_E_UNSUPPORTED; }
        if (p.xc) {
            switch (epilogue) {
                case TT_EPI_BIAS: return launch_xc<TT_EPI_BIAS>(p, st);
                case TT_EPI_GELU: return launch_xc<TT_EPI_GELU>(p, st);
                case TT_EPI_RESIDUAL: return launch_xc<TT_EPI_RESIDUAL>(p, st);
                case TT_EPI_VT: return launch_xc<TT_EPI_VT>(p, st);
                default: tt_set_error("gemm f16c: epilogue %d has no f16c form", epilogue); return TT_E_UNSUPPORTED;
            }
        }
    } else if (p.xc) {
        tt_set_error("gemm (bf16 build): f16c operands belong to the fp16 instantiation");
        return TT_E_UNSUPPORTED;
    }
    if (p.x3) {
        switch (epilogue) {
            case TT_EPI_BIAS: return launch_x3<TT_EPI_BIAS>(p, st);
            case TT_EPI_GELU: return launch_x3<TT_EPI_GELU>(p, st);
            case TT_EPI_RESIDUAL: return launch_x3<TT_EPI_RESIDUAL>(p, st);
            case TT_EPI_VT: return launch_x3<TT_EPI_VT>(p, st);
            default: tt_set_error("gemm x3: epilogue %d has no split-bf16 form", epilogue); return TT_E_UNSUPPORTED;
        }
    }
    if constexpr (!kF16) if (p.fp8 && epilogue == TT_EPI_QKV) {
        if (!p.vt || p.vt_col0 % v3::BN3 || (p.N - p.vt_col0) % v3::BN3 || p.ldvt % 8) {
            tt_set_error("gemm fp8: bad qkv split");
            return TT_E_INVALID;
        }
        GemmParams a = p;
        a.N = p.vt_col0;
        if (int rc = launch_fp8<TT_EPI_BIAS>(a, st)) return rc;
        GemmParams b = p;
        b.W = reinterpret_cast<const uint16_t*>(reinterpret_cast<const char*>(p.W) + (size_t)p.vt_col0 * p.K);
        b.bias = p.bias + p.vt_col0;
        b.w_scale = p.w_scale + p.vt_col0;
        b.N = p.N - p.vt_col0;
        b.vt_col0 = 0;
        return launch_fp8<TT_EPI_VT>(b, st);
    }
    if ((p.lda % 8) || (p.ldc % 4) || !p.A || !p.W || !p.C || !p.bias) {
        tt_set_error("gemm: bad leading dimension / null pointer");
        return TT_E_INVALID;
    }
    const GemmPlan pl = plan_of(p.fp8 ? GemmForm::Fp8 : GemmForm::Bits16, epilogue, p);
    const bool skinny = pl.kernel == GemmKernel::Skinny;
    if (!skinny && (p.M % BM || p.N % BN || p.K % BK || p.K <= 0)) {
        tt_set_error("gemm: M=%d N=%d K=%d must be multiples of %d/%d/%d (or M a multiple of 64 up to 256)", p.M, p.N, p.K, BM, BN, BK);
        return TT_E_UNSUPPORTED;
    }
    switch (epilogue) {
        case TT_EPI_BIAS: return launch_16<TT_EPI_BIAS>(p, pl, st);
        case TT_EPI_GELU: return launch_16<TT_EPI_GELU>(p, pl, st);
        case TT_EPI_RESIDUAL:
            if (!p.residual || (skinny && p.ldr % 4)) { tt_set_error("gemm: residual epilogue without residual"); return TT_E_INVALID; }
            return launch_16<TT_EPI_RESIDUAL>(p, pl, st);
        case TT_EPI_TANH: return launch_16<TT_EPI_TANH>(p, pl, st);
        case TT_EPI_RELU: return launch_16<TT_EPI_RELU>(p, pl, st);
        case TT_EPI_QKV: {
            if (!p.vt || (skinny && p.vt_col0 % 16)) { tt_set_error("gemm: qkv epilogue without vt"); return TT_E_INVALID; }
            if (!skinny && gemm_qkv_splits(p.M, p.N, p.vt_col0, p.ldc, p.ldvt, gemm_switches())) {
                GemmParams a = p;
                a.N = p.vt_col0;
                if (int rc = launch_16<TT_EPI_BIAS>(a, plan_of(GemmForm::Bits16, TT_EPI_BIAS, a), st)) return rc;
                GemmParams b = p;
                b.W = p.W + (size_t)p.vt_col0 * p.K;
                b.bias = p.bias + p.vt_col0;
                b.N = p.N - p.vt_col0;
                b.vt_col0 = 0;
                return launch_16<TT_EPI_VT>(b, plan_of(GemmForm::Bits16, TT_EPI_VT, b), st);
            }
            return launch_16<TT_EPI_QKV>(p, pl, st);
        }
        default: tt_set_error("gemm: unknown epilogue %d", epilogue); return TT_E_INVALID;
    }
}

constexpr int kLdsScanOne = v3::kLdsScan > v3::kLdsScanW ? v3::kLdsScan : v3::kLdsScanW;
#ifndef TT_SCAN_PERSIST_DEFAULT
#define TT_SCAN_PERSIST_DEFAULT 1
#endif
int tt_scan_gemm_sample_launch(const uint16_t* corpus, int tiles, int tile_stride, int dim, const uint16_t* queries256, const float* thr256,
                               float* dense, int dense_stride, hipStream_t st) {
    if (tiles <= 0) return TT_OK;
    if constexpr (kF16) { tt_set_error("scan gemm: the corpus is bf16 (bf16 instantiation only)"); return TT_E_UNSUPPORTED; }
    else
    if (dim % 128 || dim <= 0 || tile_stride < 1 || !dense || dense_stride < tiles * 8 || (int64_t)tiles * tile_stride * v3::BM3 > INT32_MAX) {
        tt_set_error("scan gemm sample: tiles=%d stride=%d dim=%d dense_stride=%d", tiles, tile_stride, dim, dense_stride);
        return TT_E_UNSUPPORTED;
    }
    GemmParams p{};
    p.A = corpus;
    p.W = queries256;
    p.bias = thr256;
    p.M = tiles * v3::BM3;
    p.N = v3::BN3;
    p.K = dim;
    p.lda = dim;
    p.ldc = 8;
    p.scan_dense = dense;
    p.scan_dense_stride = dense_stride;
    p.scan_tile_stride = tile_stride;
    p.sn = 1;
    const int blocks = tile_grid_256(tiles, 1, 0).blocks;
    return run_kernel<v3::gemm_kernel_v3<TT_EPI_SCAN>>(TT_K_SCAN_SAMPLE, dim3(blocks), v3::kThreads3, kLdsScanOne, st, p);
}

int tt_scan_gemm_launch(const uint16_t* corpus, int64_t rows, int dim, const uint16_t* queries256, const float* thr256,
                        int32_t* cnt, float* cand_scores, int32_t* cand_idx, int cap, int32_t idx_base, hipStream_t st) {
    if (rows <= 0) return TT_OK;
    if constexpr (kF16) { tt_set_error("scan gemm: the corpus is bf16 (bf16 instantiation only)"); return TT_E_UNSUPPORTED; }
// ... 30 lines not shown
```

### tensor-truth_amd/csrc/rowops.hip

```cpp
#include "common.h"
#include "encoder.h"

namespace {

constexpr int kRowThreads = 256;
constexpr int kMaxChunks = 2;

__device__ __forceinline__ void unpack8(const uint4& u, float (&f)[8]) {
    f[0] = elo(u.x); f[1] = ehi(u.x);
    f[2] = elo(u.y); f[3] = ehi(u.y);
    f[4] = elo(u.z); f[5] = ehi(u.z);
    f[6] = elo(u.w); f[7] = ehi(u.w);
}

__device__ __forceinline__ uint4 pack8(const float (&f)[8]) {
    uint4 u;
    u.x = pack_e2(f[0], f[1]); u.y = pack_e2(f[2], f[3]);
    u.z = pack_e2(f[4], f[5]); u.w = pack_e2(f[6], f[7]);
    return u;
}

__device__ __forceinline__ float wave_max(float v) {
#pragma unroll
    for (int off = 32; off > 0; off >>= 1) v = fmaxf(v, __shfl_xor(v, off, 64));
// ... 74 lines not shown
            const int ch = lane + 64 * c;
            if (ch < nchunk_total) {
                float q[8];
#pragma unroll
                for (int i = 0; i < 8; ++i) q[i] = x[c][i] * inv;
                *reinterpret_cast<uint2*>(q8_row + ch * 8) = pack_fp8x8(q);
            }
        }
    }
}

template <int NT>
__global__ __launch_bounds__(kRowThreads) void layernorm_kernel(const uint16_t* in, uint16_t* out, const float* gamma,
                                                               const float* beta, int rows, int H, float eps, uint8_t* q8,
                                                               float* q8_scale) {
    constexpr int RPW = (NT & 2) ? 2 : 1;
    const int lane = threadIdx.x & 63;
    const int row0 = (blockIdx.x * (kRowThreads / 64) + (threadIdx.x >> 6)) * RPW;
    if (row0 >= rows) return;
    const int nch = H / 8;
    float x[RPW][kMaxChunks][8];
#pragma unroll
    for (int r = 0; r < RPW; ++r) {
        const int row = row0 + r < rows ? row0 + r : rows - 1;
#pragma unroll
        for (int c = 0; c < kMaxChunks; ++c) {
            const int ch = lane + 64 * c;
            if (ch < nch) {
                uint4 u;
                if constexpr (NT & 1) {
                    typedef unsigned int u4v __attribute__((ext_vector_type(4)));
                    const u4v t = __builtin_nontemporal_load(reinterpret_cast<const u4v*>(in + (size_t)row * H + ch * 8));
                    u = make_uint4(t.x, t.y, t.z, t.w);
                } else {
                    u = *reinterpret_cast<const uint4*>(in + (size_t)row * H + ch * 8);
                }
                unpack8(u, x[r][c]);
            }
        }
    }
#pragma unroll
    for (int r = 0; r < RPW; ++r) {
        const int row = row0 + r;
        if (row < rows)
            ln_finish<(NT & 4) != 0>(x[r], nch, lane, H, eps, gamma, beta, out + (size_t)row * H,
                                     q8 ? q8 + (size_t)row * H : nullptr, q8 ? q8_scale + row : nullptr);
    }
}

__global__ __launch_bounds__(kRowThreads) void embed_ln_kernel(EmbedParams p) {
    const int lane = threadIdx.x & 63;
    const int row = blockIdx.x * (kRowThreads / 64) + (threadIdx.x >> 6);
    if (row >= p.T) return;
    int id = p.ids[row], ps = p.pos[row], ty = p.type ? p.type[row] : 0;
    id = id < 0 ? 0 : (id >= p.vocab ? p.vocab - 1 : id);
    ps = ps < 0 ? 0 : (ps >= p.max_pos ? p.max_pos - 1 : ps);
    ty = ty < 0 ? 0 : (ty >= p.type_vocab ? p.type_vocab - 1 : ty);
    const int nch = p.H / 8;
    float x[kMaxChunks][8];
#pragma unroll
    for (int c = 0; c < kMaxChunks; ++c) {
        const int ch = lane + 64 * c;
        if (ch < nch) {
            float a[8], b[8], t[8];
            unpack8(*reinterpret_cast<const uint4*>(p.word + (size_t)id * p.H + ch * 8), a);
            unpack8(*reinterpret_cast<const uint4*>(p.posemb + (size_t)ps * p.H + ch * 8), b);
            unpack8(*reinterpret_cast<const uint4*>(p.typeemb + (size_t)ty * p.H + ch * 8), t);
#pragma unroll
            for (int i = 0; i < 8; ++i) x[c][i] = a[i] + b[i] + t[i];
        }
    }
    ln_finish(x, nch, lane, p.H, p.eps, p.gamma, p.beta, p.out + (size_t)row * p.H, p.q8 ? p.q8 + (size_t)row * p.H : nullptr,
              p.q8 ? p.q8_scale + row : nullptr);
}

__global__ __launch_bounds__(kRowThreads) void cls_pool_kernel(const uint16_t* hidden, int ld, const int32_t* rows, int n,
                                                              int H, float* out_f32, uint16_t* out_bf16) {
    const int lane = threadIdx.x & 63;
    const int b = blockIdx.x * (kRowThreads / 64) + (threadIdx.x >> 6);
    if (b >= n) return;
    const int nch = H / 8;
    const uint16_t* src = hidden + (size_t)rows[b] * ld;
    float x[kMaxChunks][8];
    float ss = 0.f;
#pragma unroll
    for (int c = 0; c < kMaxChunks; ++c) {
        const int ch = lane + 64 * c;
        if (ch < nch) {
            unpack8(*reinterpret_cast<const uint4*>(src + ch * 8), x[c]);
#pragma unroll
            for (int i = 0; i < 8; ++i) ss = mul_then_add(x[c][i], x[c][i], ss);
        }
    }
    const float nrm = fmaxf(sqrtf(wave_sum(ss)), 1e-12f);
    const float inv = 1.0f / nrm;
#pragma unroll
    for (int c = 0; c < kMaxChunks; ++c) {
        const int ch = lane + 64 * c;
        if (ch < nch) {
            float y[8];
#pragma unroll
            for (int i = 0; i < 8; ++i) y[i] = x[c][i] * inv;
            float* o = out_f32 + (size_t)b * H + ch * 8;
            *reinterpret_cast<float4*>(o) = make_float4(y[0], y[1], y[2], y[3]);
            *reinterpret_cast<float4*>(o + 4) = make_float4(y[4], y[5], y[6], y[7]);
            if (out_bf16) *reinterpret_cast<uint4*>(out_bf16 + (size_t)b * H + ch * 8) = pack8(y);
        }
// ... 258 lines not shown
```

### tensor-truth_amd/encoder.py

```python
from __future__ import annotations

import ctypes
import dataclasses
import itertools
import os
import threading
from ctypes import POINTER, Structure, c_float, c_int32, c_void_p
from dataclasses import dataclass
from typing import Dict, Iterable, List, Optional, Sequence, Tuple

import numpy as np
import torch

from . import _lib


@dataclass(frozen=True)
class EncoderConfig:

    arch: str = "xlmr"
    vocab_size: int = 250002
    hidden: int = 1024
    layers: int = 24
    heads: int = 16
# ... 22 lines not shown
    "BAAI/bge-m3": BGE_M3,
    "BAAI/bge-reranker-v2-m3": BGE_RERANKER_V2_M3,
    "BAAI/bge-small-en-v1.5": BGE_SMALL_EN_V15,
    "BAAI/bge-reranker-base": BGE_RERANKER_BASE,
    "cross-encoder/ms-marco-MiniLM-L-6-v2": MS_MARCO_MINILM_L6_V2,
}


_LAYER_FIELDS = ("qkv_w", "qkv_b", "o_w", "o_b", "ln1_g", "ln1_b", "ffn1_w", "ffn1_b", "ffn2_w", "ffn2_b", "ln2_g", "ln2_b")


class _LayerW(Structure):
    _fields_ = [(n, c_void_p) for n in _LAYER_FIELDS + ("qkv_w8", "qkv_wscale", "ffn1_w8", "ffn1_wscale",
                                                         "o_w8", "o_wscale", "ffn2_w8", "ffn2_wscale")] + [("ffn_act_scale", c_float)]


class _PlainLayerW(Structure):
    _fields_ = [(n, c_void_p) for n in _LAYER_FIELDS]


def _weights_struct(name: str, layer: type, *extra) -> type:
    fields = ([(n, c_int32) for n in ("hidden", "layers", "heads", "ffn", "vocab", "max_pos", "type_vocab")] + [("ln_eps", c_float)]
              + [(n, c_void_p) for n in ("word_emb", "pos_emb", "type_emb", "emb_ln_g", "emb_ln_b")] + [("layer", POINTER(layer))]
              + [(n, c_void_p) for n in ("cls_dense_w", "cls_dense_b", "cls_out_w", "cls_out_b")] + list(extra))
    return type(name, (Structure,), {"_fields_": fields, "layer_type": layer})


_EncW = _weights_struct("_EncW", _LayerW, ("ffn_absmax_out", c_void_p))


@dataclass(frozen=True, kw_only=True)
class EncoderPath:

    forward: str
    workspace: str
    cls_forward: Optional[str]
    cls_workspace: Optional[str]
    pool: str
    pool_mean: str
    head: Optional[str]
    scratch: str
    head_scratch: str
    hidden: torch.dtype
    row_tile: int = 0
    skinny: bool = False
    pool_writes_bf16: bool = True
    no_fp8: Optional[str] = None
    pool_last: Optional[str] = None
    rows_forward: Optional[str] = None
    rows_workspace: Optional[str] = None
    score: Optional[str] = None
    pooled_head: Optional[str] = None
    pool_dense: Optional[str] = None


BF16_PATH = EncoderPath(forward="tt_encoder_forward", workspace="tt_encoder_workspace_bytes",
                        cls_forward="tt_encoder_forward_cls", cls_workspace="tt_encoder_cls_workspace_bytes",
                        pool="tt_embed_pool", pool_mean="tt_embed_pool_mean", head="tt_rerank_head",
                        scratch="enc", head_scratch="head", hidden=torch.bfloat16)
FP16_PATH = EncoderPath(forward="tt_encoder_forward_f16", workspace="tt_encoder_workspace_bytes_f16",
                        cls_forward="tt_encoder_forward_cls_f16", cls_workspace="tt_encoder_cls_workspace_bytes_f16",
                        pool="tt_embed_pool_f16", pool_mean="tt_embed_pool_mean_f16", head="tt_rerank_head_f16",
                        scratch="enc", head_scratch="head", hidden=torch.float16, pool_writes_bf16=False)
DECODER_BF16_PATH = EncoderPath(forward="tt_decoder_forward", workspace="tt_decoder_workspace_bytes", cls_forward=None,
                                cls_workspace=None, pool="tt_embed_pool", pool_mean="tt_embed_pool_mean", head=None,
                                scratch="enc", head_scratch="head", hidden=torch.bfloat16, pool_last="tt_embed_pool_last",
                                rows_forward="tt_decoder_forward_rows", rows_workspace="tt_decoder_rows_workspace_bytes",
                                score="tt_decoder_score", no_fp8="the decoder embedder has no fp8 projections")
DECODER_FP16_PATH = EncoderPath(forward="tt_decoder_forward_f16", workspace="tt_decoder_workspace_bytes_f16", cls_forward=None,
                                cls_workspace=None, pool="tt_embed_pool_f16", pool_mean="tt_embed_pool_mean_f16", head=None,
                                scratch="enc", head_scratch="head", hidden=torch.float16, pool_writes_bf16=False,
                                pool_last="tt_embed_pool_last_f16", rows_forward="tt_decoder_forward_rows_f16",
                                rows_workspace="tt_decoder_rows_workspace_bytes_f16", score="tt_decoder_score_f16",
                                no_fp8="the decoder embedder has no fp8 projections")
MODERNBERT_BF16_PATH = EncoderPath(forward="tt_modernbert_forward", workspace="tt_modernbert_workspace_bytes", cls_forward=None,
                                   cls_workspace=None, pool="tt_embed_pool", pool_mean="tt_embed_pool_mean", head=None,
                                   scratch="enc", head_scratch="head", hidden=torch.bfloat16, pooled_head="tt_modernbert_head",
                                   no_fp8="the ModernBERT path has no fp8 projections")
MODERNBERT_FP16_PATH = EncoderPath(forward="tt_modernbert_forward_f16", workspace="tt_modernbert_workspace_bytes_f16",
                                   cls_forward=None, cls_workspace=None, pool="tt_embed_pool_f16",
                                   pool_mean="tt_embed_pool_mean_f16", head=None, scratch="enc", head_scratch="head",
                                   hidden=torch.float16, pool_writes_bf16=False, pooled_head="tt_modernbert_head_f16",
                                   no_fp8="the ModernBERT path has no fp8 projections")
GEMMA_BF16_PATH = EncoderPath(forward="tt_gemma_forward", workspace="tt_gemma_workspace_bytes", cls_forward=None, cls_workspace=None,
                              pool="tt_embed_pool", pool_mean="tt_embed_pool_mean", head=None, scratch="enc", head_scratch="head",
                              hidden=torch.bfloat16, pool_dense="tt_gemma_pool_dense",
                              no_fp8="the EmbeddingGemma path has no fp8 projections")
MPNET_BF16_PATH = EncoderPath(forward="tt_mpnet_forward", workspace="tt_mpnet_workspace_bytes", cls_forward=None, cls_workspace=None,
                              pool="tt_embed_pool", pool_mean="tt_embed_pool_mean", head=None, scratch="enc", head_scratch="head",
                              hidden=torch.bfloat16, no_fp8="the MPNet path has no fp8 projections")
MPNET_FP16_PATH = EncoderPath(forward="tt_mpnet_forward_f16", workspace="tt_mpnet_workspace_bytes_f16", cls_forward=None,
                              cls_workspace=None, pool="tt_embed_pool_f16", pool_mean="tt_embed_pool_mean_f16", head=None,
                              scratch="enc", head_scratch="head", hidden=torch.float16, pool_writes_bf16=False,
                              no_fp8="the MPNet path has no fp8 projections")

DEBERTA_BF16_PATH = EncoderPath(forward="tt_deberta_forward", workspace="tt_deberta_workspace_bytes", cls_forward=None,
                                cls_workspace=None, pool="tt_embed_pool", pool_mean="tt_embed_pool_mean", head=None, scratch="enc",
                                head_scratch="head", hidden=torch.bfloat16, pooled_head="tt_deberta_head",
                                no_fp8="the DeBERTa path has no fp8 projections")
DEBERTA_FP16_PATH = EncoderPath(forward="tt_deberta_forward_f16", workspace="tt_deberta_workspace_bytes_f16", cls_forward=None,
                                cls_workspace=None, pool="tt_embed_pool_f16", pool_mean="tt_embed_pool_mean_f16", head=None,
                                scratch="enc", head_scratch="head", hidden=torch.float16, pool_writes_bf16=False,
                                pooled_head="tt_deberta_head_f16", no_fp8="the DeBERTa path has no fp8 projections")

ROPEBERT_BF16_PATH = EncoderPath(forward="tt_ropebert_forward", workspace="tt_ropebert_workspace_bytes", cls_forward=None,
                                 cls_workspace=None, pool="tt_embed_pool", pool_mean="tt_embed_pool_mean", head=None, scratch="enc",
                                 head_scratch="head", hidden=torch.bfloat16, no_fp8="the NomicBERT / Jina-v3 path has no fp8 projections")
ROPEBERT_FP16_PATH = EncoderPath(forward="tt_ropebert_forward_f16", workspace="tt_ropebert_workspace_bytes_f16", cls_forward=None,
                                 cls_workspace=None, pool="tt_embed_pool_f16", pool_mean="tt_embed_pool_mean_f16", head=None,
                                 scratch="enc", head_scratch="head", hidden=torch.float16, pool_writes_bf16=False,
                                 no_fp8="the NomicBERT / Jina-v3 path has no fp8 projections")

JINABERT_BF16_PATH = EncoderPath(forward="tt_jinabert_forward", workspace="tt_jinabert_workspace_bytes", cls_forward=None,
                                 cls_workspace=None, pool="tt_embed_pool", pool_mean="tt_embed_pool_mean", head=None, scratch="enc",
                                 head_scratch="head", hidden=torch.bfloat16, no_fp8="the JinaBERT path has no fp8 projections")
JINABERT_FP16_PATH = EncoderPath(forward="tt_jinabert_forward_f16", workspace="tt_jinabert_workspace_bytes_f16", cls_forward=None,
# ... 225 lines not shown
        W[p + "attention.output.LayerNorm.bias"] = n(H, std=0.05)
        W[p + "intermediate.dense.weight"] = n(F, H)
        W[p + "intermediate.dense.bias"] = n(F)
        W[p + "output.dense.weight"] = n(H, F)
        W[p + "output.dense.bias"] = n(H)
        W[p + "output.LayerNorm.weight"] = 1.0 + n(H, std=0.1)
        W[p + "output.LayerNorm.bias"] = n(H, std=0.05)
    if cfg.num_labels:
        W["classifier.dense.weight"] = n(H, H)
        W["classifier.dense.bias"] = n(H)
        W["classifier.out_proj.weight"] = n(cfg.num_labels, H, std=0.2)
        W["classifier.out_proj.bias"] = n(cfg.num_labels)
    return W


def synthetic_state_device(cfg: EncoderConfig, device: torch.device, seed: int = 0,
                           dtype: torch.dtype = torch.bfloat16) -> Dict[str, torch.Tensor]:
    g = torch.Generator(device=device).manual_seed(seed)
    n = lambda *s, std=0.02: (torch.randn(*s, generator=g, device=device) * std).to(dtype)
    H, F = cfg.hidden, cfg.ffn
    W = {
        "embeddings.word_embeddings.weight": n(cfg.vocab_size, H),
        "embeddings.position_embeddings.weight": n(cfg.max_pos, H),
        "embeddings.token_type_embeddings.weight": n(cfg.type_vocab, H),
        "embeddings.LayerNorm.weight": 1.0 + n(H, std=0.1).float(),
        "embeddings.LayerNorm.bias": n(H, std=0.05).float(),
    }
    for i in range(cfg.layers):
        p = f"encoder.layer.{i}."
        for nm in ("query", "key", "value"):
            W[p + f"attention.self.{nm}.weight"] = n(H, H)
            W[p + f"attention.self.{nm}.bias"] = n(H).float()
        W[p + "attention.output.dense.weight"] = n(H, H)
        W[p + "attention.output.dense.bias"] = n(H).float()
        W[p + "attention.output.LayerNorm.weight"] = 1.0 + n(H, std=0.1).float()
        W[p + "attention.output.LayerNorm.bias"] = n(H, std=0.05).float()
        W[p + "intermediate.dense.weight"] = n(F, H)
        W[p + "intermediate.dense.bias"] = n(F).float()
        W[p + "output.dense.weight"] = n(H, F)
        W[p + "output.dense.bias"] = n(H).float()
        W[p + "output.LayerNorm.weight"] = 1.0 + n(H, std=0.1).float()
        W[p + "output.LayerNorm.bias"] = n(H, std=0.05).float()
    if cfg.num_labels:
        W["classifier.dense.weight"] = n(H, H)
        W["classifier.dense.bias"] = n(H).float()
        W["classifier.out_proj.weight"] = n(cfg.num_labels, H, std=0.2)
        W["classifier.out_proj.bias"] = n(cfg.num_labels).float()
    return W


_PACK_ALIGN = max(1, int(os.environ.get("TT_PACK_ALIGN", "8")))


@dataclass
class PackedBatch:

    ids: np.ndarray
    pos: np.ndarray
    types: Optional[np.ndarray]
    seq_start: np.ndarray
    seq_len: np.ndarray
    n_rows: int
    max_len: int
    n_tokens: int


def _round_rows(used: int) -> int:
    if used <= 256 and not (_lib.is_diag() and os.environ.get("TT_GEMM_SKINNY", "1") == "0"):
        return max(64, (used + 63) // 64 * 64)
    return (used + 255) // 256 * 256


def pack_tokens(seqs: Sequence[Sequence[int]], cfg: EncoderConfig,
                type_ids: Optional[Sequence[Sequence[int]]] = None, max_len: Optional[int] = None) -> PackedBatch:
    limit = cfg.max_seq_len if max_len is None else min(max_len, cfg.max_seq_len)
    n_seq = len(seqs)
    lens = np.fromiter((min(len(s), limit) for s in seqs), dtype=np.int64, count=n_seq)
    if n_seq == 0 or (lens <= 0).any():
        raise ValueError("empty token sequence")
    aligned = (lens + _PACK_ALIGN - 1) // _PACK_ALIGN * _PACK_ALIGN
    starts = np.zeros(n_seq, dtype=np.int64)
    np.cumsum(aligned[:-1], out=starts[1:])
    n_rows = _round_rows(int(aligned.sum()))
    total = int(lens.sum())

    def flat_of(rows) -> np.ndarray:
        if all(isinstance(r, np.ndarray) for r in rows):
            return np.concatenate([np.asarray(r[:n], dtype=np.int32) for r, n in zip(rows, lens)]) if n_seq > 1 else \
                np.asarray(rows[0][: lens[0]], dtype=np.int32)
        return np.fromiter(itertools.chain.from_iterable(r if len(r) == n else r[:n] for r, n in zip(rows, lens)),
                           dtype=np.int32, count=total)

    first = np.zeros(n_seq, dtype=np.int64)
    np.cumsum(lens[:-1], out=first[1:])
    within = np.arange(total, dtype=np.int64) - np.repeat(first, lens)
    dest = np.repeat(starts, lens) + within
    flat = flat_of(seqs)
    if flat.min() < 0 or flat.max() >= cfg.vocab_size:
        raise ValueError("token id outside the vocabulary")
    ids = np.full(n_rows, cfg.pad_id, dtype=np.int32)
    pos = np.zeros(n_rows, dtype=np.int32)
    pos_off = cfg.pad_id + 1 if cfg.arch in ("xlmr", "mpnet") else 0
    ids[dest] = flat
    pos[dest] = within + pos_off
    types = None
    if type_ids is not None:
# ... 9 lines not shown
    sel = np.asarray(sel, dtype=np.int64)
    n_seq = len(sel)
    ln = np.minimum(lens[sel].astype(np.int64), limit)
    if n_seq == 0 or (ln <= 0).any():
        raise ValueError("empty token sequence")
    aligned = (ln + _PACK_ALIGN - 1) // _PACK_ALIGN * _PACK_ALIGN
    starts = np.zeros(n_seq, dtype=np.int64)
    np.cumsum(aligned[:-1], out=starts[1:])
    n_rows = _round_rows(int(aligned.sum()))
    total = int(ln.sum())
    local_first = np.zeros(n_seq, dtype=np.int64)
    np.cumsum(ln[:-1], out=local_first[1:])
    within = np.arange(total, dtype=np.int64) - np.repeat(local_first, ln)
    src = np.repeat(first[sel].astype(np.int64), ln) + within
    dest = np.repeat(starts, ln) + within
    vals = flat[src]
    if vals.min() < 0 or vals.max() >= cfg.vocab_size:
        raise ValueError("token id outside the vocabulary")
    ids = np.full(n_rows, cfg.pad_id, dtype=np.int32)
    pos = np.zeros(n_rows, dtype=np.int32)
    pos_off = cfg.pad_id + 1 if cfg.arch in ("xlmr", "mpnet") else 0
    ids[dest] = vals
    pos[dest] = within + pos_off
    return PackedBatch(ids, pos, None, starts.astype(np.int32), ln.astype(np.int32), int(n_rows), int(ln.max()), total)


def pack_token_matrix(ids2d: np.ndarray, cfg: EncoderConfig, type_ids2d: Optional[np.ndarray] = None) -> PackedBatch:
    ids2d = np.ascontiguousarray(ids2d, dtype=np.int32)
    n, length = ids2d.shape
    if n == 0 or length == 0:
        raise ValueError("empty token matrix")
    if length > cfg.max_seq_len:
        ids2d = ids2d[:, : cfg.max_seq_len]
        length = cfg.max_seq_len
    stride = (length + _PACK_ALIGN - 1) // _PACK_ALIGN * _PACK_ALIGN
    n_rows = _round_rows(n * stride)
    ids = np.full(n_rows, cfg.pad_id, dtype=np.int32)
    pos = np.zeros(n_rows, dtype=np.int32)
    pos_off = cfg.pad_id + 1 if cfg.arch in ("xlmr", "mpnet") else 0
    view = ids[: n * stride].reshape(n, stride)
    view[:, :length] = ids2d
    pos[: n * stride].reshape(n, stride)[:, :length] = np.arange(length, dtype=np.int32) + pos_off
    types = None
    if type_ids2d is not None:
        types = np.zeros(n_rows, dtype=np.int32)
        types[: n * stride].reshape(n, stride)[:, :length] = np.asarray(type_ids2d, dtype=np.int32)[:, :length]
    if ids2d.min() < 0 or ids2d.max() >= cfg.vocab_size:
        raise ValueError("token id outside the vocabulary")
    starts = (np.arange(n, dtype=np.int64) * stride).astype(np.int32)
    lens = np.full(n, length, dtype=np.int32)
    return PackedBatch(ids, pos, types, starts, lens, int(n_rows), int(length), int(n * length))


def pooled_rows(batch: PackedBatch, pad_token_id: Optional[int] = None) -> np.ndarray:
    starts, lens = batch.seq_start.astype(np.int64), batch.seq_len.astype(np.int64)
    if pad_token_id is None:
        return (starts + lens - 1).astype(np.int32)
    first = np.zeros(len(lens), dtype=np.int64)
    np.cumsum(lens[:-1], out=first[1:])
    within = np.arange(int(lens.sum()), dtype=np.int64) - np.repeat(first, lens)
    keep = batch.ids[np.repeat(starts, lens) + within] != pad_token_id
    return (starts + np.maximum.reduceat(np.where(keep, within, 0), first)).astype(np.int32)


class _Scratch:

    def __init__(self):
        self.bufs = {}
        self.lock = threading.Lock()

    def get(self, key, device, nbytes):
        stream = torch.cuda.current_stream(device).cuda_stream
        k = (key, device.type, device.index, stream)
        with self.lock:
            buf = self.bufs.get(k)
            if buf is None or buf.numel() < nbytes + 256:
                buf = torch.empty(nbytes + 256, dtype=torch.uint8, device=device)
                self.bufs[k] = buf
        base = (buf.data_ptr() + 255) // 256 * 256
        return buf, base


_scratch = _Scratch()
_ENQUEUE_LOCKS: Dict[Tuple[str, Optional[int]], threading.Lock] = {}


class _Stager:

    SLOTS = 8

    def __init__(self):
        self.slots = []
        self.cursor = 0
        self.lock = threading.Lock()

    def acquire(self, nbytes: int):
        with self.lock:
            if len(self.slots) < self.SLOTS:
                self.slots.append({"buf": None, "ev": None, "lock": threading.Lock()})
                slot = self.slots[-1]
            else:
                slot = self.slots[self.cursor % self.SLOTS]
            self.cursor += 1
        slot["lock"].acquire()
        if slot["ev"] is not None:
            slot["ev"].synchronize()
            slot["ev"] = None
        if slot["buf"] is None or slot["buf"].numel() < nbytes:
            slot["buf"] = torch.empty(max(nbytes, 4 << 20), dtype=torch.uint8, pin_memory=True)
        return slot


_stager = _Stager()


def _pad_rows(batch: PackedBatch, multiple: int, skinny: bool) -> PackedBatch:
    if skinny and batch.n_rows <= 256 and batch.n_rows % 64 == 0:
        return batch
    n = (batch.n_rows + multiple - 1) // multiple * multiple
    if n == batch.n_rows:
        return batch

    def pad(a, fill):
        if a is None:
            return None
        out = np.full(n, fill, dtype=a.dtype)
        out[: a.size] = a
        return out

    return dataclasses.replace(batch, ids=pad(batch.ids, batch.ids[-1] if batch.ids.size else 0), pos=pad(batch.pos, 0),
                               types=pad(batch.types, 0), n_rows=n)


class Encoder:

    def __init__(self, weights: _CheckpointWeights):
        self.w = weights
        self.cfg = weights.cfg
        self.device = weights.device
        self.path = weights.path
        self.lib = _lib.load_library()
        self._enqueue_lock = _ENQUEUE_LOCKS.setdefault((self.device.type, self.device.index), threading.Lock())

    def _upload(self, batch: PackedBatch, *more: np.ndarray):
        parts = [batch.ids, batch.pos, batch.types, batch.seq_start, batch.seq_len, *more]
        offs, total = [], 0
        for a in parts:
            offs.append(total)
            if a is not None:
                total += (a.size + 63) // 64 * 64
        slot = _stager.acquire(total * 4)
        try:
            host = slot["buf"][: total * 4].view(torch.int32)
            hn = host.numpy()
            for a, o in zip(parts, offs):
                if a is not None:
                    hn[o:o + a.size] = a
            with torch.cuda.device(self.device):
                devbuf = torch.empty(total, dtype=torch.int32, device=self.device)
                devbuf.copy_(host, non_blocking=True)
                slot["ev"] = torch.cuda.Event()
                slot["ev"].record(torch.cuda.current_stream(self.device))
        finally:
            slot["lock"].release()
        return tuple(devbuf[o:o + a.size] if a is not None else None for a, o in zip(parts, offs))

    def _padded(self, batch: PackedBatch) -> PackedBatch:
        return _pad_rows(batch, self.path.row_tile, self.path.skinny) if self.path.row_tile else batch

    def _run(self, name: str, workspace: str, batch: PackedBatch, out_rows: int, *ws_args):
        dev, w = self.device, ctypes.byref(self.w.struct)
        ids, pos, types, starts, lens = self._upload(batch)
        out = torch.empty((out_rows, self.cfg.hidden), dtype=self.path.hidden, device=dev)
        need = getattr(self.lib, workspace)(w, batch.n_rows, *ws_args)
        with self._enqueue_lock, torch.cuda.device(dev):
            ws, base = _scratch.get(self.path.scratch, dev, need)
            rc = getattr(self.lib, name)(w, ids.data_ptr(), pos.data_ptr(), types.data_ptr() if types is not None else None,
                                         starts.data_ptr(), lens.data_ptr(), len(batch.seq_len), batch.n_rows, batch.max_len,
                                         out.data_ptr(), base, need, torch.cuda.current_stream(dev).cuda_stream)
        _lib.check(rc, name)
        return out, starts, lens

    def forward_packed(self, batch: PackedBatch, want_lens: bool = False):
        batch = self._padded(batch)
        hidden, starts, lens = self._run(self.path.forward, self.path.workspace, batch, batch.n_rows)
        return (hidden, starts, lens) if want_lens else (hidden, starts)

    def calibrate_fp8(self, batch: PackedBatch, margin: float = 2.0) -> List[float]:
        if self.path.no_fp8:
            raise RuntimeError(self.path.no_fp8)
        w = self.w
        prev = w.gemm_dtype
        w.set_gemm_dtype("bf16")
        absmax = torch.zeros(max(self.cfg.layers, 1), dtype=torch.float32, device=self.device)
        w.struct.ffn_absmax_out = absmax.data_ptr()
        try:
            self.forward_packed(batch)
            vals = absmax.cpu().tolist()
        finally:
            w.struct.ffn_absmax_out = None
        w.ffn_act_scales = [max(v, 1e-6) * margin / 448.0 for v in vals[: self.cfg.layers]]
        w.set_gemm_dtype(prev)
        return w.ffn_act_scales

    def cls_hidden_packed(self, batch: PackedBatch) -> Tuple[torch.Tensor, torch.Tensor]:
        p = self.path
        if p.cls_forward is None or self.cfg.layers == 0:
            return self.forward_packed(batch)
        B = len(batch.seq_len)
        b_pad = (B + 63) // 64 * 64 if p.skinny and B <= 256 else (B + 255) // 256 * 256
        cls, _, _ = self._run(p.cls_forward, p.cls_workspace, self._padded(batch), b_pad, B)
        return cls, torch.arange(B, dtype=torch.int32, device=self.device)

    def rows_hidden_packed(self, batch: PackedBatch, rows: np.ndarray) -> torch.Tensor:
        p, dev, w = self.path, self.device, ctypes.byref(self.w.struct)
        if p.rows_forward is None:
            raise RuntimeError("this path has no one-row-per-sequence forward")
        B = len(batch.seq_len)
        rows = np.ascontiguousarray(rows, dtype=np.int32)
        if rows.shape != (B,) or (rows < batch.seq_start).any() or (rows >= batch.seq_start + batch.seq_len).any():
            raise ValueError("pooled rows: one row inside each sequence is needed")
        batch = self._padded(batch)
        ids, pos, types, starts, lens, pool = self._upload(batch, rows)
        if types is not None:
            raise ValueError("a decoder has no token types")
        out = torch.empty((_round_rows(B), self.cfg.hidden), dtype=p.hidden, device=dev)
        need = getattr(self.lib, p.rows_workspace)(w, batch.n_rows, B)
        with self._enqueue_lock, torch.cuda.device(dev):
            ws, base = _scratch.get(p.scratch, dev, need)
            rc = getattr(self.lib, p.rows_forward)(w, ids.data_ptr(), pos.data_ptr(), None, starts.data_ptr(), lens.data_ptr(), B,
                                                   batch.n_rows, batch.max_len, pool.data_ptr(), out.data_ptr(), base, need,
                                                   torch.cuda.current_stream(dev).cuda_stream)
        _lib.check(rc, p.rows_forward)
        return out

    def _compact_rows(self, n: int) -> Tuple[torch.Tensor, torch.Tensor]:
        have = getattr(self, "_compact", None)
        if have is None or have[0].numel() < n:
            cap = max(1024, 1 << (n - 1).bit_length())
            have = (torch.arange(cap, dtype=torch.int32, device=self.device), torch.ones(cap, dtype=torch.int32, device=self.device))
            torch.cuda.current_stream(self.device).synchronize()
            self._compact = have
        return have[0][:n], have[1][:n]

    def embed_packed(self, batch: PackedBatch, pooling: str = "cls", skip: int = 0) -> Tuple[torch.Tensor, torch.Tensor]:
        p, dev = self.path, self.device
        B, H = len(batch.seq_len), self.cfg.hidden
        if skip and self.cfg.arch != "t5":
            raise ValueError("a prompt is left out of the mean on the T5 path only")
        if p.pool_dense is not None:
            if pooling != "mean":
                if self.cfg.arch == "t5":
                    raise ValueError(f"pooling '{pooling}': a T5 encoder checkpoint pools the mean (its Dense module follows it)")
                raise ValueError(f"pooling '{pooling}': an EmbeddingGemma checkpoint pools the mean (its Dense modules follow it)")
            ranges = None
            if skip:
                from .t5 import pooled_ranges

                ranges = pooled_ranges(batch.seq_start, batch.seq_len, skip)
            hidden, starts, lens = self.forward_packed(batch, want_lens=True)
            if ranges is not None:
                both = torch.from_numpy(np.concatenate(ranges)).to(dev)
                starts, lens = both[:B], both[B:]
            out = torch.empty((B, self.w.out_dim), dtype=torch.float32, device=dev)
            out16 = torch.empty((B, self.w.out_dim), dtype=torch.bfloat16, device=dev)
            with torch.cuda.device(dev):
                rc = getattr(self.lib, p.pool_dense)(ctypes.byref(self.w.struct), hidden.data_ptr(), H, starts.data_ptr(),
                                                     lens.data_ptr(), B, out.data_ptr(), out16.data_ptr(),
                                                     torch.cuda.current_stream(dev).cuda_stream)
            _lib.check(rc, p.pool_dense)
            return out, out16
        out = torch.empty((B, H), dtype=torch.float32, device=dev)
        out16 = torch.empty((B, H), dtype=torch.bfloat16, device=dev) if p.pool_writes_bf16 else None
        if pooling == "mean":
            hidden, starts, lens = self.forward_packed(batch, want_lens=True)
            name, rows = p.pool_mean, (starts.data_ptr(), lens.data_ptr())
        elif pooling == "last":
            if p.pool_last is None:
                raise ValueError("last-token pooling needs a decoder path")
            hidden = self.rows_hidden_packed(batch, pooled_rows(batch))
            starts, lens = self._compact_rows(B)
            name, rows = p.pool_last, (starts.data_ptr(), lens.data_ptr())
        elif pooling == "cls":
            hidden, cls_rows = self.cls_hidden_packed(batch)
            name, rows = p.pool, (cls_rows.data_ptr(),)
        else:
            raise ValueError(f"pooling '{pooling}' (supported: 'cls', 'mean', 'last')")
        with torch.cuda.device(dev):
            rc = getattr(self.lib, name)(hidden.data_ptr(), H, *rows, B, H, out.data_ptr(),
                                         out16.data_ptr() if out16 is not None else None, torch.cuda.current_stream(dev).cuda_stream)
        _lib.check(rc, name)
        return out, (out16 if out16 is not None else out.to(torch.bfloat16))

    def rerank_packed(self, batch: PackedBatch, want_logits: bool = False):
        if not self.cfg.num_labels:
            raise RuntimeError("these weights carry no classification head")
        p, dev = self.path, self.device
        B, H = len(batch.seq_len), self.cfg.hidden
        scores = torch.empty(B, dtype=torch.float32, device=dev)
        logits = torch.empty(B, dtype=torch.float32, device=dev) if want_logits else None
        if p.score is not None:
            hidden = self.rows_hidden_packed(batch, pooled_rows(batch, self.cfg.pad_token_id))
            with torch.cuda.device(dev):
                rc = getattr(self.lib, p.score)(hidden.data_ptr(), H, self.w.score_w.data_ptr(), B, H, scores.data_ptr(),
                                                logits.data_ptr() if want_logits else None, torch.cuda.current_stream(dev).cuda_stream)
            _lib.check(rc, p.score)
            return (scores, logits) if want_logits else scores
        if p.pooled_head is not None:
            hidden, starts, lens = self.forward_packed(batch, want_lens=True)
            with torch.cuda.device(dev):
                rc = getattr(self.lib, p.pooled_head)(ctypes.byref(self.w.struct), hidden.data_ptr(), H, starts.data_ptr(),
                                                      lens.data_ptr(), B, 1 if getattr(self.cfg, "classifier_pooling", "cls") == "mean" else 0,
                                                      scores.data_ptr(), logits.data_ptr() if want_logits else None,
                                                      torch.cuda.current_stream(dev).cuda_stream)
            _lib.check(rc, p.pooled_head)
            return (scores, logits) if want_logits else scores
        hidden, cls_rows = self.cls_hidden_packed(batch)
        n_pad = (B + 127) // 128 * 128
        need = 2 * ((n_pad * H * hidden.element_size() + 255) // 256 * 256)
        with self._enqueue_lock, torch.cuda.device(dev):
            ws, base = _scratch.get(p.head_scratch, dev, need)
            rc = getattr(self.lib, p.head)(ctypes.byref(self.w.struct), hidden.data_ptr(), cls_rows.data_ptr(), B,
                                           scores.data_ptr(), logits.data_ptr() if want_logits else None, base, need,
                                           torch.cuda.current_stream(dev).cuda_stream)
        _lib.check(rc, p.head)
        return (scores, logits) if want_logits else scores

    def embed(self, seqs, type_ids=None, max_len=None):
        return self.embed_packed(pack_tokens(seqs, self.cfg, type_ids, max_len))

    def rerank(self, seqs, max_len: Optional[int] = 512, want_logits: bool = False):
        return self.rerank_packed(pack_tokens(seqs, self.cfg, None, max_len), want_logits)
```

Before: 116.2.

## Run reranker CLS forward on compacted rows without per-sequence alignment padding

Adds a compact CLS encoder forward for batches whose sequences share one length. Rows are packed densely (n_seq*len) for the GEMMs and layernorms, while V^T is written into an aligned frame layout by a new V^T GEMM epilogue. Attention kernels gain a frame_start offset so they can address packed K rows against the framed V^T. The aim is to stop spending GEMM and FFN work on the alignment padding rows between sequences. In exchange it splits the QKV GEMM into two launches, adds a prologue kernel, and disables the fp8 path when this mode is used.

```diff
diff --git a/include/tt_hip.h b/include/tt_hip.h
--- a/include/tt_hip.h
+++ b/include/tt_hip.h
@@ -124,6 +124,16 @@
                            const int32_t* type_ids, const int32_t* seq_start, const int32_t* seq_len,
                            int n_seq, int n_rows, int max_len, void* cls_out,
                            void* workspace, size_t workspace_bytes, void* stream);
+
+size_t tt_encoder_cls_compact_workspace_bytes(const tt_encoder_weights* w, int n_seq, int len, int stride, int64_t* layout);
+int tt_encoder_forward_cls_compact(const tt_encoder_weights* w, const int32_t* ids, const int32_t* pos, const int32_t* type_ids,
+                                   int n_seq, int len, int stride, int n_rows, void* cls_out,
+                                   void* workspace, size_t workspace_bytes, void* stream);
+int tt_attention_varlen_framed(const void* qk, int ld_qk, int q_col0, int k_col0, const void* vt, int ldvt, void* out, int ld_out,
+                               const int32_t* seq_start, const int32_t* frame_start, const int32_t* seq_len, int n_seq,
+                               int heads, int head_dim, int max_len, void* stream);
+int tt_gemm_vt(const void* a, const void* w, const float* bias, void* vt, int m, int n, int k, int rows, int len, int stride,
+               void* stream);
 
 int tt_embed_pool(const void* hidden_bf16, int ld, const int32_t* rows, int n_seq, int hidden,
                   float* out_f32, void* out_bf16, void* stream);
@@ -223,6 +233,15 @@
 int tt_attention_varlen_f16(const void* qk, int ld_qk, int q_col0, int k_col0, const void* vt, int ldvt, void* out,
                             int ld_out, const int32_t* seq_start, const int32_t* seq_len, int n_seq, int heads,
                             int head_dim, int max_len, void* stream);
+size_t tt_encoder_cls_compact_workspace_bytes_f16(const tt_encoder_weights* w, int n_seq, int len, int stride, int64_t* layout);
+int tt_encoder_forward_cls_compact_f16(const tt_encoder_weights* w, const int32_t* ids, const int32_t* pos, const int32_t* type_ids,
+                                       int n_seq, int len, int stride, int n_rows, void* cls_out,
+                                       void* workspace, size_t workspace_bytes, void* stream);
+int tt_attention_varlen_framed_f16(const void* qk, int ld_qk, int q_col0, int k_col0, const void* vt, int ldvt, void* out, int ld_out,
+                                   const int32_t* seq_start, const int32_t* frame_start, const int32_t* seq_len, int n_seq,
+                                   int heads, int head_dim, int max_len, void* stream);
+int tt_gemm_vt_f16(const void* a, const void* w, const float* bias, void* vt, int m, int n, int k, int rows, int len, int stride,
+                   void* stream);
 int tt_attention_cls_varlen_f16(const void* qk, int ld_qk, int q_col0, int k_col0, const void* vt, int ldvt, void* out,
                                 int ld_out, const int32_t* seq_start, const int32_t* seq_len, int n_seq, int heads,
                                 int head_dim, int max_len, void* stream);
diff --git a/tensor-truth_amd/_lib.py b/tensor-truth_amd/_lib.py
--- a/tensor-truth_amd/_lib.py
+++ b/tensor-truth_amd/_lib.py
@@ -85,6 +85,18 @@
     "tt_encoder_cls_workspace_bytes": (c_size_t, [c_void_p, c_int, c_int]),
     "tt_encoder_forward_cls": (c_int, [c_void_p, c_void_p, c_void_p, c_void_p, c_void_p, c_void_p, c_int, c_int, c_int,
                                        c_void_p, c_void_p, c_size_t, c_void_p]),
+    "tt_encoder_cls_compact_workspace_bytes": (c_size_t, [c_void_p, c_int, c_int, c_int, c_void_p]),
+    "tt_encoder_forward_cls_compact": (c_int, [c_void_p, c_void_p, c_void_p, c_void_p, c_int, c_int, c_int, c_int, c_void_p,
+                                               c_void_p, c_size_t, c_void_p]),
+    "tt_attention_varlen_framed": (c_int, [c_void_p, c_int, c_int, c_int, c_void_p, c_int, c_void_p, c_int, c_void_p, c_void_p,
+                                           c_void_p, c_int, c_int, c_int, c_int, c_void_p]),
+    "tt_gemm_vt": (c_int, [c_void_p, c_void_p, c_void_p, c_void_p, c_int, c_int, c_int, c_int, c_int, c_int, c_void_p]),
+    "tt_encoder_cls_compact_workspace_bytes_f16": (c_size_t, [c_void_p, c_int, c_int, c_int, c_void_p]),
+    "tt_encoder_forward_cls_compact_f16": (c_int, [c_void_p, c_void_p, c_void_p, c_void_p, c_int, c_int, c_int, c_int, c_void_p,
+                                                   c_void_p, c_size_t, c_void_p]),
+    "tt_attention_varlen_framed_f16": (c_int, [c_void_p, c_int, c_int, c_int, c_void_p, c_int, c_void_p, c_int, c_void_p, c_void_p,
+                                               c_void_p, c_int, c_int, c_int, c_int, c_void_p]),
+    "tt_gemm_vt_f16": (c_int, [c_void_p, c_void_p, c_void_p, c_void_p, c_int, c_int, c_int, c_int, c_int, c_int, c_void_p]),
     "tt_embed_pool": (c_int, [c_void_p, c_int, c_void_p, c_int, c_int, c_void_p, c_void_p, c_void_p]),
     "tt_embed_pool_mean": (c_int, [c_void_p, c_int, c_void_p, c_void_p, c_int, c_int, c_void_p, c_void_p, c_void_p]),
     "tt_embed_pool_mean_f32": (c_int, [c_void_p, c_int, c_void_p, c_void_p, c_int, c_int, c_void_p, c_void_p, c_void_p]),
@@ -308,6 +320,14 @@
 }
 
 
+OPTIONAL = frozenset(n + t for n in ("tt_encoder_cls_compact_workspace_bytes", "tt_encoder_forward_cls_compact",
+                                     "tt_attention_varlen_framed", "tt_gemm_vt") for t in ("", "_f16"))
+
+
+def has(name: str) -> bool:
+    return hasattr(load_library(), name)
+
+
 def load_library():
     global _lib
     if _lib is not None:
@@ -326,6 +346,8 @@
 
         lib = ctypes.CDLL(path)
         for name, (res, args) in SIGNATURES.items():
+            if name in OPTIONAL and os.environ.get("TT_LIB_NAME") and not hasattr(lib, name):
+                continue
             fn = getattr(lib, name)
             fn.restype = res
             fn.argtypes = args
diff --git a/tensor-truth_amd/csrc/attention.hip b/tensor-truth_amd/csrc/attention.hip
--- a/tensor-truth_amd/csrc/attention.hip
+++ b/tensor-truth_amd/csrc/attention.hip
@@ -72,7 +72,8 @@
     const int len = p.seq_len[seq];
     if (qt * 32 * NW >= len) return;
     const int t0 = p.seq_start[seq];
-    const int t0a = t0 & ~7, off = t0 - t0a, alen = off + len;
+    const int tf = p.frame_start ? p.frame_start[seq] : t0;
+    const int t0a = tf & ~7, off = tf - t0a, alen = off + len;
     const int tid = threadIdx.x, lane = tid & 63;
     const int wave = __builtin_amdgcn_readfirstlane(tid >> 6);
     const int ql = lane & 31, hh = lane >> 5;
@@ -103,7 +104,7 @@
     const int n_kt = (alen + kKTile - 1) / kKTile;
     const int n_g8 = (alen + 7) >> 3;
     const int t0kv = (ABL == 4) ? (p.seq_start[0] & ~7) : t0a;
-    const uint16_t* kbase = p.qk + (size_t)t0kv * p.ld_qk + p.k_col0 + head * DH;
+    const uint16_t* kbase = p.qk + (ptrdiff_t)((ABL == 4) ? t0kv : t0 - off) * p.ld_qk + p.k_col0 + head * DH;
     const uint16_t* vbase = p.vt + (size_t)(t0kv >> 3) * p.ldvt + (size_t)head * DH * 8;
     constexpr int kRowsPerPiece = 64 / CH, kGroupsPerPiece = 64 / DH > 0 ? 64 / DH : 1;
     static_assert(KPW == 1 || CH == 8, "piece-to-piece swizzle step is written for 128-byte K rows");
@@ -456,7 +457,8 @@
     const int len = p.seq_len[seq];
     if (len <= 0) return;
     const int t0 = p.seq_start[seq];
-    const int t0a = t0 & ~7, off = t0 - t0a, alen = off + len;
+    const int tf = p.frame_start ? p.frame_start[seq] : t0;
+    const int t0a = tf & ~7, off = tf - t0a, alen = off + len;
     const int tid = threadIdx.x, lane = tid & 63;
     const int wave = __builtin_amdgcn_readfirstlane(tid >> 6);
     const int ql = lane & 31, hh = lane >> 5;
@@ -480,7 +482,7 @@
         for (int s = 0; s < KS; ++s) qf[s] = *reinterpret_cast<const ex8*>(qp + s * 16);
     }
 
-    const uint16_t* kbase = p.qk + (size_t)t0a * p.ld_qk + p.k_col0 + head * DH;
+    const uint16_t* kbase = p.qk + (ptrdiff_t)(t0 - off) * p.ld_qk + p.k_col0 + head * DH;
     const uint16_t* vbase = p.vt + (size_t)(t0a >> 3) * p.ldvt + (size_t)head * DH * 8;
     constexpr int kRowsPerPiece = 64 / CH, kGroupsPerPiece = 1;
     uint32_t kvoff0, vvoff0;
@@ -871,7 +873,8 @@
     extern __shared__ __attribute__((aligned(16))) float probs[];
     const int seq = blockIdx.x, head = blockIdx.y, lane = threadIdx.x;
     const int len = p.seq_len[seq], t0 = p.seq_start[seq];
-    const int t0a = t0 & ~7, off = t0 - t0a, alen = off + len;
+    const int tf = p.frame_start ? p.frame_start[seq] : t0;
+    const int t0a = tf & ~7, off = tf - t0a, alen = off + len;
     float q[DH];
     {
         const uint16_t* qp = p.q_rows ? p.q_rows + (size_t)seq * p.ld_q_rows + head * DH : p.qk + (size_t)t0 * p.ld_qk + p.q_col0 + head * DH;
@@ -894,7 +897,7 @@
     const float sc = p.scale * 1.4426950408889634f;
     float mx = -__builtin_inff();
     for (int j = off + lane; j < alen; j += 64) {
-        const uint16_t* kp = p.qk + (size_t)(t0a + j) * p.ld_qk + p.k_col0 + head * DH;
+        const uint16_t* kp = p.qk + (size_t)(t0 - off + j) * p.ld_qk + p.k_col0 + head * DH;
         float acc = 0.f;
 #pragma unroll
         for (int c = 0; c < DH / 8; ++c) {
diff --git a/tensor-truth_amd/csrc/encoder.h b/tensor-truth_amd/csrc/encoder.h
--- a/tensor-truth_amd/csrc/encoder.h
+++ b/tensor-truth_amd/csrc/encoder.h
@@ -40,6 +40,7 @@
     const uint8_t* a_scales;
     const uint8_t* w_scales;
     uint8_t* c_scales;
+    int vt_len, vt_stride, vt_rows;
 };
 int tt_scan_gemm_launch(const uint16_t* corpus, int64_t rows, int dim, const uint16_t* queries256, const float* thr256,
                         int32_t* cnt, float* cand_scores, int32_t* cand_idx, int cap, int32_t idx_base, hipStream_t st);
@@ -47,6 +48,7 @@
                                float* dense, int dense_stride, hipStream_t st);
 int tt_gemm_launch(const GemmParams& p, int epilogue, hipStream_t st);
 bool tt_gemm_skinny_enabled();
+bool tt_gemm_qkv_splits(int M, int N, int vt_col0, int ldc, int ldvt);
 
 struct AttnParams {
     const uint16_t* qk;
@@ -67,6 +69,7 @@
     uint8_t* out_scales;
     int out_width;
     int qk_lo_off;
+    const int32_t* frame_start;
 };
 int tt_attention_launch(const AttnParams& p, hipStream_t st);
 int tt_attention_keylimit_launch(const AttnParams& p, const int32_t* key_len, hipStream_t st);
@@ -86,6 +89,7 @@
     float eps;
     uint8_t* q8;
     float* q8_scale;
+    int src_len, src_stride, src_rows;
 };
 int tt_embed_ln_launch(const EmbedParams& p, hipStream_t st);
 
diff --git a/tensor-truth_amd/csrc/encoder_api.hip b/tensor-truth_amd/csrc/encoder_api.hip
--- a/tensor-truth_amd/csrc/encoder_api.hip
+++ b/tensor-truth_amd/csrc/encoder_api.hip
@@ -9,7 +9,10 @@
     int n_cls_pad;
     size_t off_q8, off_q8s, off_q8c;
     bool fp8;
+    size_t off_cstart, off_fstart, off_clen;
 };
+
+struct CompactRows { int len, stride, src_rows; };
 
 bool fp8_ready(const tt_encoder_weights* w, int n_rows) {
     if constexpr (kF16) return false;
@@ -21,7 +24,7 @@
     return true;
 }
 
-EncWs enc_plan(const tt_encoder_weights* w, int n_rows, int n_seq = 0) {
+EncWs enc_plan(const tt_encoder_weights* w, int n_rows, int n_seq = 0, size_t frame_rows = 0) {
     EncWs e{};
     const size_t H = (size_t)w->hidden, F = (size_t)w->ffn, T = ((size_t)n_rows + 255) / 256 * 256;
     WsPlanner ws;
@@ -29,7 +32,7 @@
     e.off_xb = ws.take(T * H * 2);
     e.off_y = ws.take(T * H * 2);
     e.off_qk = ws.take(T * 2 * H * 2);
-    e.off_vt = ws.take(H * T * 2);
+    e.off_vt = ws.take(H * (frame_rows ? frame_rows : T) * 2);
     e.off_ctx = ws.take(T * H * 2);
     e.off_ffn = ws.take(T * F * 2);
     e.n_cls_pad = pooled_rows_pad(n_seq, tt_gemm_skinny_enabled());
@@ -41,7 +44,12 @@
         e.off_cx1 = ws.take(B * H * 2);
         e.off_cffn = ws.take(B * F * 2);
     }
-    e.fp8 = fp8_ready(w, n_rows);
+    if (frame_rows) {
+        e.off_cstart = ws.take((size_t)n_seq * 4);
+        e.off_fstart = ws.take((size_t)n_seq * 4);
+        e.off_clen = ws.take((size_t)n_seq * 4);
+    }
+    e.fp8 = !frame_rows && fp8_ready(w, n_rows);
     if (e.fp8) {
         e.off_q8 = ws.take(T * H);
         e.off_q8s = ws.take(T * 4);
@@ -63,6 +71,29 @@
     return TT_OK;
 }
 
+int compact_rows(const tt_encoder_weights* w, int n_seq, int len, int stride) {
+    if (!w || w->layers <= 0 || !w->layer || n_seq <= 0 || len <= 0 || len % 4 || stride % 8 || stride < len) return 0;
+    for (int l = 0; l < w->layers; ++l) {
+        const tt_layer_weights& lw = w->layer[l];
+        if (lw.qkv_w8 || lw.o_w8 || lw.ffn1_w8 || lw.ffn2_w8) return 0;
+    }
+    if ((long long)n_seq * stride > 0x7FFFFF00LL) return 0;
+    const int H = w->hidden, Mc = (int)(((long long)n_seq * len + 255) / 256 * 256);
+    return tt_gemm_qkv_splits(Mc, 3 * H, 2 * H, 2 * H, 8 * H) ? Mc : 0;
+}
+
+__global__ __launch_bounds__(256) void compact_prologue_kernel(int32_t* cstart, int32_t* fstart, int32_t* clen, uint16_t* vt,
+                                                               int n_seq, int len, int stride, int H) {
+    const int s = blockIdx.x;
+    if (s >= n_seq) return;
+    if (threadIdx.x == 0) { cstart[s] = s * len; fstart[s] = s * stride; clen[s] = len; }
+    const int halves = (stride - len) >> 2;
+    for (int i = threadIdx.x; i < halves * H; i += 256) {
+        const int r = len + (i / H) * 4, f = i % H;
+        *reinterpret_cast<uint2*>(vt + (size_t)((s * stride + r) >> 3) * (8 * (size_t)H) + (size_t)f * 8 + (r & 7)) = make_uint2(0u, 0u);
+    }
+}
+
 }
 
 extern "C" {
@@ -75,15 +106,16 @@
 static int forward_impl(const tt_encoder_weights* w, const int32_t* ids, const int32_t* pos,
                         const int32_t* type_ids, const int32_t* seq_start, const int32_t* seq_len, int n_seq,
                         int n_rows, int max_len, void* hidden_out, void* cls_out, void* workspace,
-                        size_t workspace_bytes, void* stream, const int32_t* key_len = nullptr) {
+                        size_t workspace_bytes, void* stream, const int32_t* key_len = nullptr, const CompactRows* cr = nullptr) {
     if (int rc = check_weights(w)) return rc;
     TT_CHECK_ARG(key_len == nullptr || cls_out == nullptr, "key_len: the full forward only");
+    TT_CHECK_ARG(cr == nullptr || (cls_out != nullptr && hidden_out == nullptr && key_len == nullptr), "compact rows: the CLS forward only");
     TT_CHECK_ARG(n_rows > 0 && (n_rows % 128 == 0 || (n_rows < 256 && n_rows % 64 == 0)),
                  "n_rows=%d must be a positive multiple of 128 (or 64 / 192)", n_rows);
     TT_CHECK_ARG(n_seq > 0 && max_len > 0, "n_seq=%d max_len=%d", n_seq, max_len);
-    TT_CHECK_ARG(ids && pos && seq_start && seq_len && (hidden_out || cls_out), "null pointer");
+    TT_CHECK_ARG(ids && pos && (cr || (seq_start && seq_len)) && (hidden_out || cls_out), "null pointer");
     const bool cls_tail = cls_out != nullptr && w->layers > 0;
-    const EncWs e = enc_plan(w, n_rows, cls_tail ? n_seq : 0);
+    const EncWs e = enc_plan(w, n_rows, cls_tail ? n_seq : 0, cr ? (size_t)n_seq * cr->stride : 0);
     if (int rc = tt_check_workspace("tt_encoder_forward", workspace, workspace_bytes, e.total)) return rc;
     hipStream_t st = (hipStream_t)stream;
     char* ws = (char*)workspace;
@@ -95,7 +127,22 @@
     uint16_t* vt = (uint16_t*)(ws + e.off_vt);
     uint16_t* ctx = (uint16_t*)(ws + e.off_ctx);
     uint16_t* ffn = (uint16_t*)(ws + e.off_ffn);
-    TT_CHECK_HIP(hipMemsetAsync(ctx, 0, (size_t)T * H * 2, st));
+    const int32_t* frame_start = nullptr;
+    if (cr) {
+        const size_t real = (size_t)n_seq * cr->len;
+        if ((size_t)T > real) TT_CHECK_HIP(hipMemsetAsync(ctx + real * H, 0, ((size_t)T - real) * H * 2, st));
+        int32_t* cstart = (int32_t*)(ws + e.off_cstart);
+        int32_t* fstart = (int32_t*)(ws + e.off_fstart);
+        int32_t* clen = (int32_t*)(ws + e.off_clen);
+        {
+            TtProfScope prof(TT_K_ROWOPS, st);
+            hipLaunchKernelGGL(compact_prologue_kernel, dim3(n_seq), dim3(256), 0, st, cstart, fstart, clen, vt, n_seq, cr->len, cr->stride, H);
+            TT_CHECK_LAUNCH();
+        }
+        seq_start = cstart; seq_len = clen; frame_start = fstart;
+    } else {
+        TT_CHECK_HIP(hipMemsetAsync(ctx, 0, (size_t)T * H * 2, st));
+    }
 
     EmbedParams ep{};
     ep.ids = ids; ep.pos = pos; ep.type = type_ids;
@@ -104,6 +151,7 @@
     ep.gamma = w->emb_ln_g; ep.beta = w->emb_ln_b;
     ep.T = T; ep.H = H; ep.vocab = w->vocab; ep.max_pos = w->max_pos; ep.type_vocab = w->type_vocab;
     ep.eps = w->ln_eps;
+    if (cr) { ep.src_len = cr->len; ep.src_stride = cr->stride; ep.src_rows = cr->src_rows; }
     uint16_t* x = (w->layers == 0 && hidden_out) ? (uint16_t*)hidden_out : xa;
     ep.out = x;
     uint8_t* q8 = e.fp8 ? (uint8_t*)(ws + e.off_q8) : nullptr;
@@ -182,10 +230,17 @@
             g.W = (const uint16_t*)lw.qkv_w + (size_t)H * H; g.bias = lw.qkv_b + H;
             g.C = qk + H; g.N = 2 * H; g.vt_col0 = H;
         }
-        if (int rc = tt_gemm_launch(g, TT_EPI_QKV, st)) return rc;
+        if (cr) {
+            GemmParams gv = g;
+            g.N = g.vt_col0;
+            if (int rc = tt_gemm_launch(g, TT_EPI_BIAS, st)) return rc;
+            gv.W = g.W + (size_t)g.vt_col0 * H; gv.bias = g.bias + g.vt_col0; gv.N = H; gv.vt_col0 = 0;
+            gv.vt_len = cr->len; gv.vt_stride = cr->stride; gv.vt_rows = n_seq * cr->len;
+            if (int rc = tt_gemm_launch(gv, TT_EPI_VT, st)) return rc;
+        } else if (int rc = tt_gemm_launch(g, TT_EPI_QKV, st)) return rc;
         AttnParams a{};
         a.qk = qk; a.ld_qk = 2 * H; a.q_col0 = 0; a.k_col0 = H; a.vt = vt; a.ldvt = 8 * H;
-        a.ld_out = H; a.seq_start = seq_start; a.seq_len = seq_len;
+        a.ld_out = H; a.seq_start = seq_start; a.seq_len = seq_len; a.frame_start = frame_start;
         a.n_seq = n_seq; a.heads = w->heads; a.head_dim = dh; a.max_len = max_len;
         a.scale = 1.0f / sqrtf((float)dh);
         if (cls_tail && l == w->layers - 1) {
@@ -254,6 +309,30 @@
                         workspace_bytes, stream);
 }
 
+size_t tt_encoder_cls_compact_workspace_bytes(const tt_encoder_weights* w, int n_seq, int len, int stride, int64_t* layout) {
+    if (layout) layout[0] = layout[1] = layout[2] = 0;
+    if (!w || check_weights(w) != TT_OK) return 0;
+    const int Mc = compact_rows(w, n_seq, len, stride);
+    if (!Mc) return 0;
+    const EncWs e = enc_plan(w, Mc, n_seq, (size_t)n_seq * stride);
+    if (layout) { layout[0] = Mc; layout[1] = (int64_t)e.off_vt; layout[2] = (int64_t)n_seq * stride * w->hidden * 2; }
+    return e.total;
+}
+
+int tt_encoder_forward_cls_compact(const tt_encoder_weights* w, const int32_t* ids, const int32_t* pos, const int32_t* type_ids,
+                                   int n_seq, int len, int stride, int n_rows, void* cls_out, void* workspace, size_t workspace_bytes,
+                                   void* stream) {
+    TT_CHECK_ARG(cls_out != nullptr, "null cls_out");
+    if (int rc = check_weights(w)) return rc;
+    const int Mc = compact_rows(w, n_seq, len, stride);
+    TT_CHECK_ARG(Mc > 0, "compact rows: n_seq=%d len=%d stride=%d keeps the aligned rows (tt_encoder_cls_compact_workspace_bytes is 0)",
+                 n_seq, len, stride);
+    TT_CHECK_ARG((long long)n_rows >= (long long)(n_seq - 1) * stride + len, "n_rows=%d holds no %d sequences of stride %d", n_rows, n_seq, stride);
+    const CompactRows cr{len, stride, n_rows};
+    return forward_impl(w, ids, pos, type_ids, nullptr, nullptr, n_seq, Mc, len, nullptr, cls_out, workspace, workspace_bytes, stream,
+                        nullptr, &cr);
+}
+
 int tt_embed_pool(const void* hidden_bf16, int ld, const int32_t* rows, int n_seq, int hidden, float* out_f32,
                   void* out_bf16, void* stream) {
     TT_CHECK_ARG(n_seq >= 0, "n_seq=%d", n_seq);
@@ -406,6 +485,28 @@
     return tt_attention_launch(a, (hipStream_t)stream);
 }
 
+int tt_attention_varlen_framed(const void* qk, int ld_qk, int q_col0, int k_col0, const void* vt, int ldvt, void* out, int ld_out,
+                               const int32_t* seq_start, const int32_t* frame_start, const int32_t* seq_len, int n_seq, int heads,
+                               int head_dim, int max_len, void* stream) {
+    TT_CHECK_ARG(qk && vt && out && seq_start && frame_start && seq_len, "null pointer");
+    AttnParams a{};
+    a.qk = (const uint16_t*)qk; a.ld_qk = ld_qk; a.q_col0 = q_col0; a.k_col0 = k_col0;
+    a.vt = (const uint16_t*)vt; a.ldvt = ldvt; a.out = (uint16_t*)out; a.ld_out = ld_out;
+    a.seq_start = seq_start; a.frame_start = frame_start; a.seq_len = seq_len; a.n_seq = n_seq; a.heads = heads; a.head_dim = head_dim;
+    a.max_len = max_len; a.scale = 1.0f / sqrtf((float)head_dim);
+    return tt_attention_launch(a, (hipStream_t)stream);
+}
+
+int tt_gemm_vt(const void* a, const void* w, const float* bias, void* vt, int m, int n, int k, int rows, int len, int stride,
+               void* stream) {
+    TT_CHECK_ARG(a && w && bias && vt, "null pointer");
+    GemmParams g = gemm_16((const uint16_t*)a, w, bias, m, n, k);
+    g.C = (uint16_t*)vt;
+    g.vt = (uint16_t*)vt; g.ldvt = 8 * n; g.vt_col0 = 0;
+    g.vt_len = len; g.vt_stride = stride; g.vt_rows = rows;
+    return tt_gemm_launch(g, TT_EPI_VT, (hipStream_t)stream);
+}
+
 int tt_attention_cls_varlen(const void* qk, int ld_qk, int q_col0, int k_col0, const void* vt, int ldvt, void* out,
                             int ld_out, const int32_t* seq_start, const int32_t* seq_len, int n_seq, int heads,
                             int head_dim, int max_len, void* stream) {
diff --git a/tensor-truth_amd/csrc/f16_names.h b/tensor-truth_amd/csrc/f16_names.h
--- a/tensor-truth_amd/csrc/f16_names.h
+++ b/tensor-truth_amd/csrc/f16_names.h
@@ -3,6 +3,7 @@
 #define tt_scan_gemm_launch tt_scan_gemm_launch_f16
 #define tt_scan_gemm_sample_launch tt_scan_gemm_sample_launch_f16
 #define tt_gemm_skinny_enabled tt_gemm_skinny_enabled_f16
+#define tt_gemm_qkv_splits tt_gemm_qkv_splits_f16
 #define tt_attention_launch tt_attention_launch_f16
 #define tt_attention_cls_launch tt_attention_cls_launch_f16
 #define tt_attention_keylimit_launch tt_attention_keylimit_launch_f16
@@ -20,6 +21,10 @@
 #define tt_encoder_forward tt_encoder_forward_f16
 #define tt_encoder_forward_cls tt_encoder_forward_cls_f16
 #define tt_encoder_forward_keylen tt_encoder_forward_keylen_f16
+#define tt_encoder_cls_compact_workspace_bytes tt_encoder_cls_compact_workspace_bytes_f16
+#define tt_encoder_forward_cls_compact tt_encoder_forward_cls_compact_f16
+#define tt_attention_varlen_framed tt_attention_varlen_framed_f16
+#define tt_gemm_vt tt_gemm_vt_f16
 #define tt_embed_pool tt_embed_pool_f16
 #define tt_embed_pool_mean tt_embed_pool_mean_f16
 #define tt_rerank_head tt_rerank_head_f16
diff --git a/tensor-truth_amd/csrc/gemm.hip b/tensor-truth_amd/csrc/gemm.hip
--- a/tensor-truth_amd/csrc/gemm.hip
+++ b/tensor-truth_amd/csrc/gemm.hip
@@ -146,18 +146,28 @@
     }
 }
 
-template <int NT, int MT, bool FP8 = false, bool X3 = false>
+template <int NT, int MT, bool FP8 = false, bool X3 = false, bool FRAME = false>
 __device__ __forceinline__ void gemm_epilogue_vt(const GemmParams& p, f32x4 (&acc)[NT][MT], int mw, int nw, int lane) {
     static_assert(NT % 2 == 0, "n-tiles are processed in pairs");
+    static_assert(!FRAME || (!FP8 && !X3), "the frame scatter is written for plain 16-bit operands");
     const int g = lane >> 4;
     const bool odd = (g & 1) != 0;
+    int fs0 = 0, fr0 = 0;
+    if constexpr (FRAME) {
+        const int m0 = mw + (g & ~1) * 4;
+        fs0 = m0 / p.vt_len;
+        fr0 = m0 - fs0 * p.vt_len;
+    }
 #pragma unroll
     for (int i = 0; i < NT; i += 2) {
+        int fs = fs0, fr = fr0;
         const int n = nw + (odd ? i + 1 : i) * 16 + (lane & 15);
         const float b = p.bias[n];
         float sw = 1.f;
         if constexpr (FP8) sw = p.w_scale[n];
         uint16_t* col = p.vt + (size_t)(n - p.vt_col0) * 8;
+        uint16_t* fat = nullptr;
+        if constexpr (FRAME) fat = col + (size_t)(fs * (p.vt_stride >> 3) + (fr >> 3)) * p.ldvt + (fr & 7);
 #pragma unroll
         for (int j = 0; j < MT; ++j) {
             float v[8];
@@ -180,6 +190,35 @@
             uint4 o;
             o.x = pack_sel<X3>(v[0], v[1]); o.y = pack_sel<X3>(v[2], v[3]);
             o.z = pack_sel<X3>(v[4], v[5]); o.w = pack_sel<X3>(v[6], v[7]);
+            if constexpr (FRAME) {
+                if (fr + 16 < p.vt_len && m < p.vt_rows) {
+                    if ((fr & 7) == 0) {
+                        *reinterpret_cast<uint4*>(fat) = o;
+                    } else {
+                        *reinterpret_cast<uint2*>(fat) = make_uint2(o.x, o.y);
+                        *reinterpret_cast<uint2*>(fat + p.ldvt - 4) = make_uint2(o.z, o.w);
+                    }
+                    fr += 16;
+                    fat += 2 * (size_t)p.ldvt;
+                    continue;
+                }
+                const int g8 = p.vt_stride >> 3;
+                if (m < p.vt_rows) {
+                    const bool wrap = fr + 4 >= p.vt_len;
+                    if (!wrap && (fr & 7) == 0) {
+                        *reinterpret_cast<uint4*>(fat) = o;
+                    } else {
+                        *reinterpret_cast<uint2*>(fat) = make_uint2(o.x, o.y);
+                        const int s1 = wrap ? fs + 1 : fs, r1 = wrap ? 0 : fr + 4;
+                        if (m + 4 < p.vt_rows)
+                            *reinterpret_cast<uint2*>(col + (size_t)(s1 * g8 + (r1 >> 3)) * p.ldvt + (r1 & 7)) = make_uint2(o.z, o.w);
+                    }
+                }
+                fr += 16;
+                while (fr >= p.vt_len) { fr -= p.vt_len; ++fs; }
+                fat = col + (size_t)(fs * g8 + (fr >> 3)) * p.ldvt + (fr & 7);
+                continue;
+            }
             *reinterpret_cast<uint4*>(col + (size_t)(m >> 3) * p.ldvt) = o;
             if constexpr (X3) {
                 uint4 l;
@@ -920,9 +959,10 @@
     }
 }
 
-template <int EPI, bool FP8 = false, bool X3 = false, bool XC = false, bool RP = false>
+template <int EPI, bool FP8 = false, bool X3 = false, bool XC = false, bool RP = false, bool VF = false>
 __global__ __launch_bounds__(kThreads3, 2) void gemm_kernel_v3(GemmParams p) {
     static_assert(!(FP8 && X3), "split-bf16 operands are bf16");
+    static_assert(!VF || (EPI == TT_EPI_VT && !FP8 && !X3 && !XC), "the frame scatter: the 16-bit V^T epilogue");
     static_assert(!XC || (!FP8 && !X3 && kF16), "f16c operands: the fp16 instantiation, no other operand mode");
     constexpr int ES = FP8 ? 1 : 2;
     extern __shared__ __attribute__((aligned(16))) char smem[];
@@ -1216,7 +1256,7 @@
         for (int qm = 0; qm < 2; ++qm)
 #pragma unroll
             for (int qn = 0; qn < 2; ++qn)
-                gemm_epilogue_vt<2, 4, FP8, X3>(p, acc[qm][qn], m0 + qm * 128 + wm * 64, n0 + wn * 64 + qn * 32, lane);
+                gemm_epilogue_vt<2, 4, FP8, X3, VF>(p, acc[qm][qn], m0 + qm * 128 + wm * 64, n0 + wn * 64 + qn * 32, lane);
     } else if constexpr (X3) {
         epilogue_x3<EPI, RP>(p, acc, smem, kBiasOff, m0, n0, wm, wn, lane);
     } else if constexpr (XC && EPI == TT_EPI_RESIDUAL) {
@@ -1930,6 +1970,9 @@
             break;
         case GemmKernel::OneTile256:
             q.nt_store = sw.nt_store;
+            if constexpr (EPI == TT_EPI_VT)
+                if (p.vt_len > 0)
+                    return run_kernel<v3::gemm_kernel_v3<EPI, false, false, false, false, true>>(TT_K_GEMM, dim3(pl.gx), v3::kThreads3, v3::kLds3, st, q);
             return run_kernel<v3::gemm_kernel_v3<EPI>>(TT_K_GEMM, dim3(pl.gx), v3::kThreads3, v3::kLds3, st, q);
         case GemmKernel::Staged128:
             if constexpr (EPI != TT_EPI_VT) return run_kernel<gemm_staged_kernel<EPI, false>>(TT_K_GEMM, dim3(pl.gx), kStagedThreads, kStagedLds, st, q);
@@ -1946,6 +1989,7 @@
 }
 
 bool tt_gemm_skinny_enabled() { return gemm_switches().skinny; }
+bool tt_gemm_qkv_splits(int M, int N, int vt_col0, int ldc, int ldvt) { return gemm_qkv_splits(M, N, vt_col0, ldc, ldvt, gemm_switches()); }
 
 int tt_gemm_launch(const GemmParams& p, int epilogue, hipStream_t st) {
     if (p.M <= 0 || p.N <= 0) return TT_OK;
@@ -2007,6 +2051,17 @@
             return launch_16<TT_EPI_RESIDUAL>(p, pl, st);
         case TT_EPI_TANH: return launch_16<TT_EPI_TANH>(p, pl, st);
         case TT_EPI_RELU: return launch_16<TT_EPI_RELU>(p, pl, st);
+        case TT_EPI_VT:
+            if (!p.vt || p.vt_col0 || p.ldvt % 8 || p.M % 256 || p.N % 256 || pl.kernel != GemmKernel::OneTile256) {
+                tt_set_error("gemm: the V^T launch needs vt, whole 256x256 tiles and ldvt a multiple of 8");
+                return TT_E_INVALID;
+            }
+            if (p.vt_len < 0 || (p.vt_len > 0 && (p.vt_len % 4 || p.vt_stride % 8 || p.vt_stride < p.vt_len || p.vt_rows % p.vt_len ||
+                                                  p.vt_rows < 0 || p.vt_rows > p.M || p.ldvt < 8 * p.N))) {
+                tt_set_error("gemm: V^T frame len=%d stride=%d rows=%d (M=%d)", p.vt_len, p.vt_stride, p.vt_rows, p.M);
+                return TT_E_INVALID;
+            }
+            return launch_16<TT_EPI_VT>(p, pl, st);
         case TT_EPI_QKV: {
             if (!p.vt || (skinny && p.vt_col0 % 16)) { tt_set_error("gemm: qkv epilogue without vt"); return TT_E_INVALID; }
             if (!skinny && gemm_qkv_splits(p.M, p.N, p.vt_col0, p.ldc, p.ldvt, gemm_switches())) {
diff --git a/tensor-truth_amd/csrc/rowops.hip b/tensor-truth_amd/csrc/rowops.hip
--- a/tensor-truth_amd/csrc/rowops.hip
+++ b/tensor-truth_amd/csrc/rowops.hip
@@ -150,7 +150,13 @@
     const int lane = threadIdx.x & 63;
     const int row = blockIdx.x * (kRowThreads / 64) + (threadIdx.x >> 6);
     if (row >= p.T) return;
-    int id = p.ids[row], ps = p.pos[row], ty = p.type ? p.type[row] : 0;
+    int src = row;
+    if (p.src_len > 0) {
+        const int s = row / p.src_len;
+        src = s * p.src_stride + (row - s * p.src_len);
+        src = src < p.src_rows ? src : p.src_rows - 1;
+    }
+    int id = p.ids[src], ps = p.pos[src], ty = p.type ? p.type[src] : 0;
     id = id < 0 ? 0 : (id >= p.vocab ? p.vocab - 1 : id);
     ps = ps < 0 ? 0 : (ps >= p.max_pos ? p.max_pos - 1 : ps);
     ty = ty < 0 ? 0 : (ty >= p.type_vocab ? p.type_vocab - 1 : ty);
diff --git a/tensor-truth_amd/encoder.py b/tensor-truth_amd/encoder.py
--- a/tensor-truth_amd/encoder.py
+++ b/tensor-truth_amd/encoder.py
@@ -98,16 +98,21 @@
     score: Optional[str] = None
     pooled_head: Optional[str] = None
     pool_dense: Optional[str] = None
+    cls_compact: Optional[str] = None
+    cls_compact_workspace: Optional[str] = None
 
 
 BF16_PATH = EncoderPath(forward="tt_encoder_forward", workspace="tt_encoder_workspace_bytes",
                         cls_forward="tt_encoder_forward_cls", cls_workspace="tt_encoder_cls_workspace_bytes",
                         pool="tt_embed_pool", pool_mean="tt_embed_pool_mean", head="tt_rerank_head",
-                        scratch="enc", head_scratch="head", hidden=torch.bfloat16)
+                        scratch="enc", head_scratch="head", hidden=torch.bfloat16, cls_compact="tt_encoder_forward_cls_compact",
+                        cls_compact_workspace="tt_encoder_cls_compact_workspace_bytes")
 FP16_PATH = EncoderPath(forward="tt_encoder_forward_f16", workspace="tt_encoder_workspace_bytes_f16",
                         cls_forward="tt_encoder_forward_cls_f16", cls_workspace="tt_encoder_cls_workspace_bytes_f16",
                         pool="tt_embed_pool_f16", pool_mean="tt_embed_pool_mean_f16", head="tt_rerank_head_f16",
-                        scratch="enc", head_scratch="head", hidden=torch.float16, pool_writes_bf16=False)
+                        scratch="enc", head_scratch="head", hidden=torch.float16, pool_writes_bf16=False,
+                        cls_compact="tt_encoder_forward_cls_compact_f16",
+                        cls_compact_workspace="tt_encoder_cls_compact_workspace_bytes_f16")
 DECODER_BF16_PATH = EncoderPath(forward="tt_decoder_forward", workspace="tt_decoder_workspace_bytes", cls_forward=None,
                                 cls_workspace=None, pool="tt_embed_pool", pool_mean="tt_embed_pool_mean", head=None,
                                 scratch="enc", head_scratch="head", hidden=torch.bfloat16, pool_last="tt_embed_pool_last",
@@ -439,6 +444,9 @@
 _PACK_ALIGN = max(1, int(os.environ.get("TT_PACK_ALIGN", "8")))
 
 
+_COMPACT_ROWS = os.environ.get("TT_COMPACT_ROWS", "1") != "0"
+
+
 @dataclass
 class PackedBatch:
 
@@ -554,6 +562,22 @@
     return PackedBatch(ids, pos, types, starts, lens, int(n_rows), int(length), int(n * length))
 
 
+def uniform_geometry(batch: PackedBatch) -> Optional[Tuple[int, int]]:
+    lens, starts = batch.seq_len, batch.seq_start
+    n = len(lens)
+    if n == 0:
+        return None
+    ln = int(lens[0])
+    if ln <= 0 or ln % 4 or (lens != ln).any():
+        return None
+    stride = int(starts[1]) - int(starts[0]) if n > 1 else (ln + 7) // 8 * 8
+    if stride < ln or stride % 8 or (starts.astype(np.int64) != np.arange(n, dtype=np.int64) * stride).any():
+        return None
+    if (n - 1) * stride + ln > batch.n_rows:
+        return None
+    return ln, stride
+
+
 def pooled_rows(batch: PackedBatch, pad_token_id: Optional[int] = None) -> np.ndarray:
     starts, lens = batch.seq_start.astype(np.int64), batch.seq_len.astype(np.int64)
     if pad_token_id is None:
@@ -642,6 +666,8 @@
         self.device = weights.device
         self.path = weights.path
         self.lib = _lib.load_library()
+        self.compact_rows = _COMPACT_ROWS
+        self.last_cls_rows: Optional[str] = None
         self._enqueue_lock = _ENQUEUE_LOCKS.setdefault((self.device.type, self.device.index), threading.Lock())
 
     def _upload(self, batch: PackedBatch, *more: np.ndarray):
@@ -705,14 +731,38 @@
         w.set_gemm_dtype(prev)
         return w.ffn_act_scales
 
-    def cls_hidden_packed(self, batch: PackedBatch) -> Tuple[torch.Tensor, torch.Tensor]:
+    def cls_hidden_packed(self, batch: PackedBatch, compact: bool = False) -> Tuple[torch.Tensor, torch.Tensor]:
         p = self.path
         if p.cls_forward is None or self.cfg.layers == 0:
             return self.forward_packed(batch)
         B = len(batch.seq_len)
         b_pad = (B + 63) // 64 * 64 if p.skinny and B <= 256 else (B + 255) // 256 * 256
-        cls, _, _ = self._run(p.cls_forward, p.cls_workspace, self._padded(batch), b_pad, B)
+        cls = self._cls_compact(batch, b_pad) if compact and self.compact_rows else None
+        self.last_cls_rows = "aligned" if cls is None else "compact"
+        if cls is None:
+            cls, _, _ = self._run(p.cls_forward, p.cls_workspace, self._padded(batch), b_pad, B)
         return cls, torch.arange(B, dtype=torch.int32, device=self.device)
+
+    def _cls_compact(self, batch: PackedBatch, out_rows: int) -> Optional[torch.Tensor]:
+        p, dev, w = self.path, self.device, ctypes.byref(self.w.struct)
+        if p.cls_compact is None or getattr(self.w, "gemm_dtype", "bf16") == "fp8" or not _lib.has(p.cls_compact):
+            return None
+        geo = uniform_geometry(batch)
+        if geo is None:
+            return None
+        B, (ln, stride) = len(batch.seq_len), geo
+        need = getattr(self.lib, p.cls_compact_workspace)(w, B, ln, stride, None)
+        if not need:
+            return None
+        ids, pos, types, _, _ = self._upload(batch)
+        out = torch.empty((out_rows, self.cfg.hidden), dtype=p.hidden, device=dev)
+        with self._enqueue_lock, torch.cuda.device(dev):
+            ws, base = _scratch.get(p.scratch, dev, need)
+            rc = getattr(self.lib, p.cls_compact)(w, ids.data_ptr(), pos.data_ptr(), types.data_ptr() if types is not None else None,
+                                                  B, ln, stride, batch.n_rows, out.data_ptr(), base, need,
+                                                  torch.cuda.current_stream(dev).cuda_stream)
+        _lib.check(rc, p.cls_compact)
+        return out
 
     def rows_hidden_packed(self, batch: PackedBatch, rows: np.ndarray) -> torch.Tensor:
         p, dev, w = self.path, self.device, ctypes.byref(self.w.struct)
@@ -817,7 +867,7 @@
                                                       torch.cuda.current_stream(dev).cuda_stream)
             _lib.check(rc, p.pooled_head)
             return (scores, logits) if want_logits else scores
-        hidden, cls_rows = self.cls_hidden_packed(batch)
+        hidden, cls_rows = self.cls_hidden_packed(batch, compact=True)
         n_pad = (B + 127) // 128 * 128
         need = 2 * ((n_pad * H * hidden.element_size() + 255) // 256 * 256)
         with self._enqueue_lock, torch.cuda.device(dev):
```

Result: no change. 117.1, median of 6 (+0.8%).
